# zgcr/SimpleAICV_pytorch_training_examples

Measured on NVIDIA H100. Metric: images/sec (ResNet-50 224x224 training step, whole job), higher is better.
Workload: dtype bf16

## Files before the change

### include/saicv_b200.h

```cpp
#ifndef SAICV_B200_H_
#define SAICV_B200_H_
#include <stdint.h>

#ifdef __cplusplus
extern "C" {
#endif

#define SAICV_EPI_BIAS 1
#define SAICV_EPI_RELU 2
#define SAICV_EPI_GELU 4
#define SAICV_EPI_DIRECT 8
#define SAICV_EPI_RESID 16
#define SAICV_EPI_ADD_BF16 32
#define SAICV_EPI_MUL_DRELU 512

int saicv_version(void);
const char* saicv_last_error(void);
int saicv_sm_count(void);
long long saicv_launch_count(void);

int saicv_linear_fwd(const void* x, const void* w, const float* bias, const float* resid,
                     const float* row_scale, int rows_per_scale, float* stats_partial, void* y,
                     int M, int N, int K, int flags, int out_f32, void* stream);
int saicv_gemm_stats_rows(long long out_rows, int out_cols);
int saicv_linear_dgrad(const void* dy, const void* w, const float* resid, const void* gelu_pre,
                       void* dx, int M, int N, int K, int flags, int out_f32, void* stream);
int saicv_linear_wgrad(const void* dy, const void* x, float* dw_partial, int M, int N, int K,
                       int splits, void* stream);
int saicv_wgrad_splits(int out_rows, int out_cols, long long reduce_len);

typedef struct {
  int n, h, w, c;
  int k, r, s;
  int stride, pad;
} saicv_conv_shape;
int saicv_conv_fprop(const void* x, const void* w, float* stats_partial, void* y,
                     const saicv_conv_shape* cs, int flags, void* stream);
int saicv_conv_dgrad(const void* dy, const void* w, const void* add, const uint32_t* mask_bits, void* dx,
                     const saicv_conv_shape* cs, void* stream);
int saicv_conv_wgrad(const void* dy, const void* x, float* dw_partial, const saicv_conv_shape* cs,
                     int splits, void* stream);

int saicv_prep_conv_weight(const float* w, void* w_bf16, int k, int c, int r, int s, int kpad,
                           int order, int kp, int cp, void* stream);
int saicv_finish_conv_wgrad(const float* partial, float* grad, int splits, int k, int c, int r,
                            int s, int kpad, int accumulate, int order, int kp, int cp, void* stream);
int saicv_reduce_partials(const float* partial, float* out, int splits, long long n,
                          int accumulate, void* stream);
int saicv_cast_bf16(const float* src, void* dst, long long n, void* stream);
int saicv_nchw_to_nhwc_bf16(const float* x, void* y, int n, int c, int h, int w, void* stream);
int saicv_stem_kpad(int c, int r, int s);
int saicv_stem_im2col(const float* x, void* cols, int n, int c, int h, int w, int r, int s,
                      int stride, int pad, int kpad, void* stream);
int saicv_zero_upsample2(const void* dy, void* u, int n, int p, int q, int h, int w, int c,
                         void* stream);
int saicv_add_strided2(void* dx, const void* dd, int n, int p, int q, int h, int w, int c,
                       void* stream);

#define SAICV_BN_PARTIAL_ROWS 264
int saicv_bn_stats(const void* y, float* partials, long long rows, int c, void* stream);
int saicv_bn_finalize(const float* partials, int partial_rows, const float* gamma, const float* beta,
                      float* running_mean, float* running_var, float* scale_shift, float* saved,
                      long long rows, int c, float eps, float momentum, void* stream);
int saicv_bn_apply(const void* y, const float* scale_shift, const void* res,
                   const float* res_scale_shift, void* out, uint32_t* mask_bits, long long rows, int c,
                   int act, void* stream);
int saicv_bn_bwd_reduce(const void* dout, const void* out, const uint32_t* bits, const void* y,
                        const float* saved, const float* scale_shift, float* partials, float* sums,
                        long long rows, int c, int act, void* stream);
int saicv_bn_bwd_apply(const void* dout, const void* out, const uint32_t* bits, const void* y,
                       const float* saved, const float* gamma, const float* scale_shift, float* sums,
                       void* dy, void* dres, float* dgamma, float* dbeta, long long rows, int c, int act,
                       int accumulate, void* stream);
int saicv_bn_bwd_reduce2(const void* g, const uint32_t* bits, const void* y_a, const void* y_b,
                         const float* saved_a, const float* saved_b, float* partials, float* sums,
                         long long rows, int c, void* stream);
int saicv_bn_bwd_apply2(const void* g, const uint32_t* bits, const void* y_a, const void* y_b,
                        const float* saved_a, const float* saved_b, const float* gamma_a,
                        const float* gamma_b, const float* sums, void* dy_a, void* dy_b,
                        float* dgamma_a, float* dbeta_a, float* dgamma_b, float* dbeta_b,
                        long long rows, int c, int accumulate_a, int accumulate_b, void* stream);
int saicv_add_bf16(void* a, const void* b, long long n, void* stream);

int saicv_maxpool3x3s2_fwd(const void* x, void* y, uint8_t* argmax, int n, int h, int w, int c,
                           void* stream);
int saicv_maxpool3x3s2_bwd(const void* dy, const uint8_t* argmax, void* dx, int n, int h, int w,
                           int c, void* stream);
int saicv_maxpool_fwd(const void* x, void* y, uint8_t* argmax, int n, int h, int w, int c, int k,
                      int stride, int pad, int pad_hi, int oob_zero, void* stream);
int saicv_maxpool_bwd(const void* dy, const uint8_t* argmax, void* dx, int n, int h, int w, int c,
                      int k, int stride, int pad, int pad_hi, void* stream);
int saicv_avgpool_fwd(const void* x, void* y, int n, int hw, int c, void* stream);
int saicv_avgpool_bwd(const void* dy, void* dx, int n, int hw, int c, void* stream);
int saicv_colsum(const void* x, float* partials, float* out, long long rows, int c, int accumulate,
                 int is_f32, void* stream);

int saicv_layernorm_fwd(const float* x, const float* gamma, const float* beta, void* y,
                        float* stats, long long rows, int c, float eps, void* stream);
int saicv_layernorm_bwd(const void* dy, const float* x, const float* gamma, const float* stats,
                        const float* dres, float* dx, void* dx_bf16, const float* bf16_row_scale,
                        int rows_per_scale, float* partials ,
                        float* dgamma, float* dbeta, long long rows, int c, int accumulate, void* stream);
int saicv_gelu_fwd(const void* u, void* h, long long n, void* stream);
int saicv_gelu_bwd(const void* dh, const void* u, void* du, long long n, void* stream);
int saicv_vit_assemble_tokens(const float* patch, const float* cls, const float* pos, float* x,
                              int b, int np, int c, void* stream);
int saicv_vit_assemble_tokens_bwd(const float* dx, float* dpos, float* dcls, void* dpatch, int b,
                                  int np, int c, int accumulate, void* stream);
int saicv_token_pool_fwd(const float* x, float* pooled, int b, int l, int c, int mean_pool,
                         void* stream);
int saicv_token_pool_bwd(const float* dpooled, float* dx, void* dx_bf16, const float* bf16_row_scale,
                         int b, int l, int c, int mean_pool, void* stream);
int saicv_dwconv_fwd(const void* x, const float* w, const float* bias, void* y, int n, int h, int wd,
                     int c, int k, int dil, int relu, int flip, void* stream);
int saicv_dwconv_dgrad_masked(const void* dy, const float* w, const void* mask, void* dx, int n, int h,
                              int wd, int c, int k, void* stream);
int saicv_avgpool_stream_fwd(const void* x, int x_f32, void* y, int n, int hw, int c, void* stream);
int saicv_avgpool_stream_bwd(const void* dy, void* dx, int dx_f32, int n, int hw, int c, void* stream);
int saicv_dwconv_wgrad_blocks(long long npix);
int saicv_dwconv_wgrad(const void* dy, const void* x, float* partial, float* dw, int n, int h, int wd,
                       int c, int k, int dil, int accumulate, void* stream);
int saicv_mul_bf16(const void* a, const void* b, void* out, long long n, void* stream);
int saicv_gate_bwd(const void* dg, const void* c1, const void* dlk, const void* p1, void* out,
                   long long n, void* stream);
int saicv_ls_residual_fwd(const void* x, int x_f32, const void* branch, const void* shortcut,
                          const float* ls, const float* row_scale, int rows_per_scale, float* out,
                          long long rows, int c, void* stream);
int saicv_ls_residual_bwd(const float* dxn, const void* branch, const void* shortcut, const float* ls,
                          const float* row_scale, int rows_per_scale, void* dy, float* partial,
                          float* dls, long long rows, int c, int accumulate, void* stream);
int saicv_bn_generic_partial_rows(long long rows, int c);
int saicv_bn_stats_generic(const void* x, int x_f32, float* partial, long long rows, int c, void* stream);
int saicv_bn_apply_generic(const void* x, int x_f32, const float* scale_shift, void* out, int out_f32,
                           long long rows, int c, void* stream);
int saicv_bn_bwd_generic(const void* x, int x_f32, const void* g, int g_f32, const float* saved,
                         const float* gamma, const float* dres, float* partial, float* sums, void* dx,
                         int dx_f32, float* dgamma, float* dbeta, long long rows, int c, int accumulate,
                         void* stream);
int saicv_im2col_nhwc(const void* x, void* cols, int n, int h, int w, int c, int k, int stride, int pad,
                      void* stream);
int saicv_col2im_nhwc(const void* dcols, void* dx, int n, int h, int w, int c, int k, int stride, int pad,
                      void* stream);

int saicv_window_partition(const void* x, void* windows, int b, int h, int w, int c, int ws, void* stream);
int saicv_window_unpartition(const void* windows, void* x, int b, int h, int w, int c, int ws, void* stream);
int saicv_add_pos_embed(float* x, const float* pos, int b, long long per_batch, void* stream);
int saicv_relpos_pack_q(const void* qkv, void* qc, int bw, int heads, int hd, int l, void* stream);
int saicv_relpos_table(const float* rel_pos_h, const float* rel_pos_w, void* rtab, int sh, int sw, int nip, int hd,
                       void* stream);
int saicv_relpos_gather(const void* qkv, const void* t, void* qe, void* ke, int bw, int heads, int hd, int sh, int sw,
                        int dqk, int nip, float scale, void* stream);
int saicv_relpos_shift(const void* dqe, void* ef, int bw, int heads, int hd, int sh, int sw, int dqk, int nip,
                       void* stream);
int saicv_relpos_dq_combine(const void* dqe, const float* dqx, void* dqkv, int bw, int heads, int hd, int l, int dqk,
                            float scale, void* stream);

typedef struct {
  const void* q; const void* k; const void* v;
  void* out;
  float* lse;
  long long q_strides[3], k_strides[3], v_strides[3], o_strides[3];
  const unsigned int* key_mask_bits;
  int mask_words;
  int b, h, lq, lk, dqk, dv;
  float scale;
  float dropout_p;
  unsigned long long dropout_seed;
  const unsigned long long* dropout_seed_base;
} saicv_attn_args;
int saicv_attn_fwd(const saicv_attn_args* a, void* stream);
typedef struct {
  saicv_attn_args fwd;
  const void* dout;
  float* delta;
  void* dq; void* dk; void* dv;
  long long dq_strides[3], dk_strides[3], dv_strides[3];
  int dk_cols;
} saicv_attn_bwd_args;
int saicv_attn_bwd(const saicv_attn_bwd_args* a, void* stream);
int saicv_attention_fwd(const void* qkv, void* out, float* lse, int b, int l, int h, int d,
                        float scale, void* stream);
int saicv_attention_bwd(const void* qkv, const void* out, const void* dout, const float* lse,
                        float* delta, void* dqkv, int b, int l, int h, int d, float scale, void* stream);

int saicv_postln_fwd(const float* z, const float* gamma, const float* beta, float eps, float* y, void* yb,
                     const float* pos, long long pos_rows, void* ypb, float* stats, long long rows, int c,
                     void* stream);
int saicv_postln_bwd(const float* dy, const float* z, const float* gamma, const float* stats, const float* dres,
                     float* dz, void* dzb, float* partials, float* dgamma, float* dbeta, long long rows, int c,
                     int accumulate, void* stream);
int saicv_add_pos_cast(const float* x, const float* pos, long long pos_rows, void* xb, void* xpb, long long rows,
                       int c, void* stream);
int saicv_dropout(const void* in, int in_f32, const float* resid, const float* row_scale, long long elems_per_scale,
                  void* out, int out_f32, long long n, float p, unsigned long long seed,
                  const unsigned long long* seed_base, void* stream);
int saicv_heads_pack(const void* src, int ld, int col0, const float* extra, float extra_const, void* dst, int b,
                     int l, int h, int hd, int dp, float scale, void* stream);
int saicv_heads_unpack(const void* src, void* dst, int ld, int col0, int b, int l, int h, int hd, int dp, float scale,
                       void* stream);

int saicv_sam_loss_partial_floats(int b, int m, long long n);
int saicv_sam_loss_sums(const void* logits, int logits_bf16, const float* targets, float* partials, float* sums, int b,
                        int m, long long n, float alpha, float gamma, float mask_threshold, void* stream);
int saicv_sam_loss_bwd(const void* logits, int logits_bf16, const float* targets, const float* coef, void* dlogits,
                       int dl_bf16, int b, int m, long long n, float alpha, float gamma, void* stream);

#define SAICV_OPT_CHUNK 8192
#define SAICV_OPT_RING 8
typedef struct {
  float* p;
  const float* g;
  float* s1;
  float* s2;
  void* shadow;
  long long numel;
  int group;
  int rs;
  int c, cp, kpad;
  int pad_;
} saicv_opt_tensor;
int saicv_opt_chunk(void);
int saicv_multi_tensor_sgd(const void* tensors, const int* chunk_tensor, const int* chunk_index, int n_chunks,
                           const float* hyper, int n_groups, int* step, const float* clip, void* stream);
int saicv_multi_tensor_adamw(const void* tensors, const int* chunk_tensor, const int* chunk_index, int n_chunks,
                             const float* hyper, int n_groups, int* step, const float* clip, void* stream);
int saicv_multi_tensor_clip_coef(const void* tensors, const int* chunk_tensor, const int* chunk_index, int n_chunks,
                                 float max_norm, float* partial, float* clip, void* stream);

int saicv_u8_nhwc_to_nchw_norm(const void* in, float* out, int n, int h, int w, const float* mean3, const float* std3,
                               void* stream);

int saicv_token_gather_fwd(const float* src, long long src_rows, const int* idx, const float* fill, const float* pos,
                           const int* pos_idx, float* out, int b, int r, int c, void* stream);
int saicv_token_fill_slabs(long long rows);
int saicv_token_gather_bwd(const float* dout, const int* idx, void* dsrc, int dsrc_bf16, long long src_rows,
                           float* fill_partial, int b, int r, int c, void* stream);

#ifdef __cplusplus
}
#endif
#endif
```

### simpleaicv_pytorch_training_examples_b200/_lib.py

```python
import ctypes
import os

_HERE = os.path.dirname(os.path.abspath(__file__))
LIB_PATH = os.path.join(_HERE, 'libsaicv_b200.so')
BN_PARTIAL_ROWS = 264

c_void_p = ctypes.c_void_p
c_int = ctypes.c_int
c_ll = ctypes.c_longlong
c_float = ctypes.c_float


class ConvShape(ctypes.Structure):
    _fields_ = [('n', c_int), ('h', c_int), ('w', c_int), ('c', c_int),
                ('k', c_int), ('r', c_int), ('s', c_int), ('stride', c_int),
                ('pad', c_int)]


class AttnArgs(ctypes.Structure):
    _fields_ = [('q', c_void_p), ('k', c_void_p), ('v', c_void_p), ('out', c_void_p), ('lse', c_void_p),
                ('q_strides', c_ll * 3), ('k_strides', c_ll * 3), ('v_strides', c_ll * 3), ('o_strides', c_ll * 3),
                ('key_mask_bits', c_void_p), ('mask_words', c_int),
                ('b', c_int), ('h', c_int), ('lq', c_int), ('lk', c_int), ('dqk', c_int), ('dv', c_int),
                ('scale', c_float), ('dropout_p', c_float), ('dropout_seed', ctypes.c_ulonglong),
                ('dropout_seed_base', c_void_p)]


class AttnBwdArgs(ctypes.Structure):
    _fields_ = [('fwd', AttnArgs), ('dout', c_void_p), ('delta', c_void_p),
                ('dq', c_void_p), ('dk', c_void_p), ('dv', c_void_p),
                ('dq_strides', c_ll * 3), ('dk_strides', c_ll * 3), ('dv_strides', c_ll * 3), ('dk_cols', c_int)]


SIGNATURES = {
    'saicv_version': [],
    'saicv_sm_count': [],
    'saicv_linear_fwd': [c_void_p, c_void_p, c_void_p, c_void_p, c_void_p, c_int, c_void_p, c_void_p, c_int, c_int, c_int, c_int, c_int, c_void_p],
    'saicv_gemm_stats_rows': [c_ll, c_int],
    'saicv_linear_dgrad': [c_void_p, c_void_p, c_void_p, c_void_p, c_void_p, c_int, c_int, c_int, c_int, c_int, c_void_p],
    'saicv_linear_wgrad': [c_void_p, c_void_p, c_void_p, c_int, c_int, c_int, c_int, c_void_p],
    'saicv_wgrad_splits': [c_int, c_int, c_ll],
    'saicv_conv_fprop': [c_void_p, c_void_p, c_void_p, c_void_p, ctypes.POINTER(ConvShape), c_int, c_void_p],
    'saicv_conv_dgrad': [c_void_p, c_void_p, c_void_p, c_void_p, c_void_p, ctypes.POINTER(ConvShape), c_void_p],
    'saicv_conv_wgrad': [c_void_p, c_void_p, c_void_p, ctypes.POINTER(ConvShape), c_int, c_void_p],
    'saicv_prep_conv_weight': [c_void_p, c_void_p, c_int, c_int, c_int, c_int, c_int, c_int, c_int, c_int, c_void_p],
    'saicv_finish_conv_wgrad': [c_void_p, c_void_p, c_int, c_int, c_int, c_int, c_int, c_int, c_int, c_int, c_int, c_int, c_void_p],
    'saicv_reduce_partials': [c_void_p, c_void_p, c_int, c_ll, c_int, c_void_p],
    'saicv_cast_bf16': [c_void_p, c_void_p, c_ll, c_void_p],
    'saicv_nchw_to_nhwc_bf16': [c_void_p, c_void_p, c_int, c_int, c_int, c_int, c_void_p],
    'saicv_stem_kpad': [c_int, c_int, c_int],
    'saicv_stem_im2col': [c_void_p, c_void_p, c_int, c_int, c_int, c_int, c_int, c_int, c_int, c_int, c_int, c_void_p],
    'saicv_zero_upsample2': [c_void_p, c_void_p, c_int, c_int, c_int, c_int, c_int, c_int, c_void_p],
    'saicv_add_strided2': [c_void_p, c_void_p, c_int, c_int, c_int, c_int, c_int, c_int, c_void_p],
    'saicv_bn_stats': [c_void_p, c_void_p, c_ll, c_int, c_void_p],
    'saicv_bn_finalize': [c_void_p, c_int, c_void_p, c_void_p, c_void_p, c_void_p, c_void_p, c_void_p, c_ll, c_int, c_float, c_float, c_void_p],
    'saicv_bn_apply': [c_void_p, c_void_p, c_void_p, c_void_p, c_void_p, c_void_p, c_ll, c_int, c_int, c_void_p],
    'saicv_bn_bwd_reduce': [c_void_p, c_void_p, c_void_p, c_void_p, c_void_p, c_void_p, c_void_p, c_void_p, c_ll, c_int, c_int, c_void_p],
    'saicv_bn_bwd_apply': [c_void_p, c_void_p, c_void_p, c_void_p, c_void_p, c_void_p, c_void_p, c_void_p, c_void_p, c_void_p, c_void_p, c_void_p, c_ll, c_int, c_int, c_int, c_void_p],
    'saicv_bn_bwd_reduce2': [c_void_p, c_void_p, c_void_p, c_void_p, c_void_p, c_void_p, c_void_p, c_void_p, c_ll, c_int, c_void_p],
    'saicv_bn_bwd_apply2': [c_void_p] * 15 + [c_ll, c_int, c_int, c_int, c_void_p],
    'saicv_add_bf16': [c_void_p, c_void_p, c_ll, c_void_p],
    'saicv_maxpool3x3s2_fwd': [c_void_p, c_void_p, c_void_p, c_int, c_int, c_int, c_int, c_void_p],
    'saicv_maxpool3x3s2_bwd': [c_void_p, c_void_p, c_void_p, c_int, c_int, c_int, c_int, c_void_p],
    'saicv_maxpool_fwd': [c_void_p, c_void_p, c_void_p, c_int, c_int, c_int, c_int, c_int, c_int, c_int, c_int, c_int, c_void_p],
    'saicv_maxpool_bwd': [c_void_p, c_void_p, c_void_p, c_int, c_int, c_int, c_int, c_int, c_int, c_int, c_int, c_void_p],
    'saicv_avgpool_fwd': [c_void_p, c_void_p, c_int, c_int, c_int, c_void_p],
    'saicv_avgpool_bwd': [c_void_p, c_void_p, c_int, c_int, c_int, c_void_p],
    'saicv_colsum': [c_void_p, c_void_p, c_void_p, c_ll, c_int, c_int, c_int, c_void_p],
    'saicv_layernorm_fwd': [c_void_p, c_void_p, c_void_p, c_void_p, c_void_p, c_ll, c_int, c_float, c_void_p],
    'saicv_layernorm_bwd': [c_void_p, c_void_p, c_void_p, c_void_p, c_void_p, c_void_p, c_void_p, c_void_p, c_int, c_void_p, c_void_p, c_void_p, c_ll, c_int, c_int, c_void_p],
    'saicv_gelu_fwd': [c_void_p, c_void_p, c_ll, c_void_p],
    'saicv_gelu_bwd': [c_void_p, c_void_p, c_void_p, c_ll, c_void_p],
    'saicv_vit_assemble_tokens': [c_void_p, c_void_p, c_void_p, c_void_p, c_int, c_int, c_int, c_void_p],
    'saicv_vit_assemble_tokens_bwd': [c_void_p, c_void_p, c_void_p, c_void_p, c_int, c_int, c_int, c_int, c_void_p],
    'saicv_token_pool_fwd': [c_void_p, c_void_p, c_int, c_int, c_int, c_int, c_void_p],
    'saicv_token_pool_bwd': [c_void_p, c_void_p, c_void_p, c_void_p, c_int, c_int, c_int, c_int, c_void_p],
    'saicv_attention_fwd': [c_void_p, c_void_p, c_void_p, c_int, c_int, c_int, c_int, c_float, c_void_p],
    'saicv_attention_bwd': [c_void_p, c_void_p, c_void_p, c_void_p, c_void_p, c_void_p, c_int, c_int, c_int, c_int, c_float, c_void_p],
    'saicv_attn_fwd': [ctypes.POINTER(AttnArgs), c_void_p],
    'saicv_attn_bwd': [ctypes.POINTER(AttnBwdArgs), c_void_p],
    'saicv_window_partition': [c_void_p, c_void_p, c_int, c_int, c_int, c_int, c_int, c_void_p],
    'saicv_window_unpartition': [c_void_p, c_void_p, c_int, c_int, c_int, c_int, c_int, c_void_p],
    'saicv_add_pos_embed': [c_void_p, c_void_p, c_int, c_ll, c_void_p],
    'saicv_relpos_pack_q': [c_void_p, c_void_p, c_int, c_int, c_int, c_int, c_void_p],
    'saicv_relpos_table': [c_void_p, c_void_p, c_void_p, c_int, c_int, c_int, c_int, c_void_p],
    'saicv_relpos_gather': [c_void_p, c_void_p, c_void_p, c_void_p, c_int, c_int, c_int, c_int, c_int, c_int, c_int, c_float, c_void_p],
    'saicv_relpos_shift': [c_void_p, c_void_p, c_int, c_int, c_int, c_int, c_int, c_int, c_int, c_void_p],
    'saicv_relpos_dq_combine': [c_void_p, c_void_p, c_void_p, c_int, c_int, c_int, c_int, c_int, c_float, c_void_p],
    'saicv_sam_loss_partial_floats': [c_int, c_int, c_ll],
    'saicv_sam_loss_sums': [c_void_p, c_int, c_void_p, c_void_p, c_void_p, c_int, c_int, c_ll, c_float, c_float, c_float, c_void_p],
    'saicv_sam_loss_bwd': [c_void_p, c_int, c_void_p, c_void_p, c_void_p, c_int, c_int, c_int, c_ll, c_float, c_float, c_void_p],
    'saicv_u8_nhwc_to_nchw_norm': [c_void_p, c_void_p, c_int, c_int, c_int, ctypes.POINTER(c_float), ctypes.POINTER(c_float), c_void_p],
    'saicv_token_gather_fwd': [c_void_p, c_ll, c_void_p, c_void_p, c_void_p, c_void_p, c_void_p, c_int, c_int, c_int, c_void_p],
    'saicv_token_fill_slabs': [c_ll],
    'saicv_token_gather_bwd': [c_void_p, c_void_p, c_void_p, c_int, c_ll, c_void_p, c_int, c_int, c_int, c_void_p],
    'saicv_opt_chunk': [],
    'saicv_multi_tensor_sgd': [c_void_p, c_void_p, c_void_p, c_int, c_void_p, c_int, c_void_p, c_void_p, c_void_p],
    'saicv_multi_tensor_adamw': [c_void_p, c_void_p, c_void_p, c_int, c_void_p, c_int, c_void_p, c_void_p, c_void_p],
    'saicv_multi_tensor_clip_coef': [c_void_p, c_void_p, c_void_p, c_int, c_float, c_void_p, c_void_p, c_void_p],
    'saicv_postln_fwd': [c_void_p, c_void_p, c_void_p, c_float, c_void_p, c_void_p, c_void_p, c_ll, c_void_p, c_void_p, c_ll, c_int, c_void_p],
    'saicv_postln_bwd': [c_void_p, c_void_p, c_void_p, c_void_p, c_void_p, c_void_p, c_void_p, c_void_p, c_void_p, c_void_p, c_ll, c_int, c_int, c_void_p],
    'saicv_add_pos_cast': [c_void_p, c_void_p, c_ll, c_void_p, c_void_p, c_ll, c_int, c_void_p],
    'saicv_dropout': [c_void_p, c_int, c_void_p, c_void_p, c_ll, c_void_p, c_int, c_ll, c_float, ctypes.c_ulonglong, c_void_p, c_void_p],
    'saicv_heads_pack': [c_void_p, c_int, c_int, c_void_p, c_float, c_void_p, c_int, c_int, c_int, c_int, c_int, c_float, c_void_p],
    'saicv_heads_unpack': [c_void_p, c_void_p, c_int, c_int, c_int, c_int, c_int, c_int, c_int, c_float, c_void_p],
    'saicv_dwconv_fwd': [c_void_p, c_void_p, c_void_p, c_void_p, c_int, c_int, c_int, c_int, c_int, c_int, c_int, c_int, c_void_p],
    'saicv_dwconv_dgrad_masked': [c_void_p, c_void_p, c_void_p, c_void_p, c_int, c_int, c_int, c_int, c_int, c_void_p],
    'saicv_avgpool_stream_fwd': [c_void_p, c_int, c_void_p, c_int, c_int, c_int, c_void_p],
    'saicv_avgpool_stream_bwd': [c_void_p, c_void_p, c_int, c_int, c_int, c_int, c_void_p],
    'saicv_dwconv_wgrad_blocks': [c_ll],
    'saicv_dwconv_wgrad': [c_void_p, c_void_p, c_void_p, c_void_p, c_int, c_int, c_int, c_int, c_int, c_int, c_int, c_void_p],
    'saicv_mul_bf16': [c_void_p, c_void_p, c_void_p, c_ll, c_void_p],
    'saicv_gate_bwd': [c_void_p, c_void_p, c_void_p, c_void_p, c_void_p, c_ll, c_void_p],
    'saicv_ls_residual_fwd': [c_void_p, c_int, c_void_p, c_void_p, c_void_p, c_void_p, c_int, c_void_p, c_ll, c_int, c_void_p],
    'saicv_ls_residual_bwd': [c_void_p, c_void_p, c_void_p, c_void_p, c_void_p, c_int, c_void_p, c_void_p, c_void_p, c_ll, c_int, c_int, c_void_p],
    'saicv_bn_generic_partial_rows': [c_ll, c_int],
    'saicv_bn_stats_generic': [c_void_p, c_int, c_void_p, c_ll, c_int, c_void_p],
    'saicv_bn_apply_generic': [c_void_p, c_int, c_void_p, c_void_p, c_int, c_ll, c_int, c_void_p],
    'saicv_bn_bwd_generic': [c_void_p, c_int, c_void_p, c_int, c_void_p, c_void_p, c_void_p, c_void_p, c_void_p, c_void_p, c_int, c_void_p, c_void_p, c_ll, c_int, c_int, c_void_p],
    'saicv_im2col_nhwc': [c_void_p, c_void_p, c_int, c_int, c_int, c_int, c_int, c_int, c_int, c_void_p],
    'saicv_col2im_nhwc': [c_void_p, c_void_p, c_int, c_int, c_int, c_int, c_int, c_int, c_int, c_void_p],
}

_lib = None


def load():
    global _lib
    if _lib is not None:
        return _lib
    if not os.path.exists(LIB_PATH):
        raise RuntimeError(
            f'{LIB_PATH} not found: build it with `python -c "import __graft_entry__ as g; g.build()"` '
            '(there is no CPU or library fallback for the hot path)')
    lib = ctypes.CDLL(LIB_PATH)
    lib.saicv_last_error.restype = ctypes.c_char_p
    lib.saicv_last_error.argtypes = []
    lib.saicv_launch_count.restype = c_ll
    lib.saicv_launch_count.argtypes = []
    for name, argtypes in SIGNATURES.items():
        fn = getattr(lib, name)
        fn.argtypes = argtypes
        fn.restype = c_int
    _lib = lib
    return lib


def launch_count():
    return int(load().saicv_launch_count())


def call(name, *args):
    lib = load()
    rc = getattr(lib, name)(*args)
    if rc != 0:
        raise RuntimeError(f'{name} failed ({rc}): {lib.saicv_last_error().decode()}')
    return rc
```

### simpleaicv_pytorch_training_examples_b200/csrc/capi_elementwise.cu

```cuda
#include <cuda_bf16.h>
#include <cuda_runtime.h>

#include <atomic>
#include <cstdarg>
#include <cstdio>

#include "../../include/saicv_b200.h"
#include "host_util.h"
#include "vec8.cuh"

namespace saicv {

static thread_local char g_err[512] = "";
int set_error(const char* fmt, ...) {
  va_list ap;
  va_start(ap, fmt);
  vsnprintf(g_err, sizeof(g_err), fmt, ap);
  va_end(ap);
  return 1;
}
static std::atomic<long long> g_launches{0};
void count_launch(int n) { g_launches.fetch_add(n, std::memory_order_relaxed); }
int check_launch(const char* what) {
  cudaError_t e = cudaGetLastError();
// ... 323 lines not shown
  const float inv_n = 1.0f / (float)rows;
  const float mean = s0 * inv_n;
  float var = s1 * inv_n - mean * mean;
  var = fmaxf(var, 0.f);
  const float rstd = rsqrtf(var + eps);
  const float sc = gamma[c] * rstd;
  ss[c] = sc;
  ss[C + c] = beta[c] - mean * sc;
  saved[c] = mean;
  saved[C + c] = rstd;
  if (rmean) {
    const float unbiased = rows > 1 ? var * ((float)rows / (float)(rows - 1)) : var;
    rmean[c] = (1.f - momentum) * rmean[c] + momentum * mean;
    rvar[c] = (1.f - momentum) * rvar[c] + momentum * unbiased;
  }
}

template <bool HAS_RES, bool RES_BN>
__global__ void __launch_bounds__(kThreads, 2)
bn_apply_kernel(const void* __restrict__ y, const float* __restrict__ ss, const void* __restrict__ res,
                const float* __restrict__ rss, void* __restrict__ out, uint8_t* __restrict__ mask, long long rows, int C,
                SlabGeom gm, int act) {
  const int vpr = gm.vpr;
  const int tx = threadIdx.x % gm.tx_count;
  const int ty = threadIdx.x / gm.tx_count;
  if (tx >= vpr) return;
  float sc[8], sh[8], rsc[8], rsh[8];
#pragma unroll
  for (int i = 0; i < 8; ++i) {
    sc[i] = ss[tx * 8 + i];
    sh[i] = ss[C + tx * 8 + i];
    rsc[i] = RES_BN ? rss[tx * 8 + i] : 1.f;
    rsh[i] = RES_BN ? rss[C + tx * 8 + i] : 0.f;
  }
  const long long r0 = (long long)blockIdx.x * gm.rows_per_block;
  long long r1 = r0 + gm.rows_per_block;
  if (r1 > rows) r1 = rows;
  for (long long r = r0 + ty; r < r1; r += (long long)gm.ty_count * UNROLL) {
    V8 vy[UNROLL], vr[UNROLL];
    bool ok[UNROLL];
#pragma unroll
    for (int u = 0; u < UNROLL; ++u) {
      const long long rr = r + (long long)u * gm.ty_count;
      ok[u] = rr < r1;
      if (ok[u]) {
        vy[u] = ldg8(y, rr * vpr + tx);
        if (HAS_RES) vr[u] = ldg8(res, rr * vpr + tx);
      }
    }
#pragma unroll
    for (int u = 0; u < UNROLL; ++u) {
      if (!ok[u]) continue;
      float f[8];
      unpack8(vy[u], f);
#pragma unroll
      for (int i = 0; i < 8; ++i) f[i] = f[i] * sc[i] + sh[i];
      const bool res_after = (act & 8) != 0;
      if (res_after) {
#pragma unroll
        for (int i = 0; i < 8; ++i) f[i] = act_apply(f[i], act & 7);
      }
      if (HAS_RES) {
        float rv[8];
        unpack8(vr[u], rv);
#pragma unroll
        for (int i = 0; i < 8; ++i) f[i] += RES_BN ? rv[i] * rsc[i] + rsh[i] : rv[i];
      }
      if (!res_after) {
#pragma unroll
        for (int i = 0; i < 8; ++i) f[i] = act_apply(f[i], act);
      }
      const long long vi = (r + (long long)u * gm.ty_count) * vpr + tx;
      const V8 o = pack8(f);
      stg8(out, vi, o);
      if (mask) {
        float fo[8];
        unpack8(o, fo);
        uint32_t m = 0;
#pragma unroll
        for (int i = 0; i < 8; ++i) m |= (fo[i] > 0.f ? 1u : 0u) << i;
        mask[vi] = (uint8_t)m;
      }
    }
  }
}

__device__ __forceinline__ void bwd_apply_coefs(const float* __restrict__ saved, const float* __restrict__ gamma,
                                                const float* __restrict__ sums, int tx, int C, float inv_rows,
                                                float (&A)[8], float (&B)[8], float (&K)[8]) {
#pragma unroll
  for (int i = 0; i < 8; ++i) {
    const int c = tx * 8 + i;
    const float mean = saved[c], rstd = saved[C + c];
    const float k1 = gamma[c] * rstd;
    const float k2 = sums[c] * inv_rows, k3 = sums[C + c] * inv_rows;
    A[i] = k1;
    B[i] = -k1 * k3 * rstd;
    K[i] = -k1 * k2 + k1 * k3 * rstd * mean;
  }
}

template <bool HAS_OUT, bool HAS_DRES>
__global__ void __launch_bounds__(kThreads, 2)
bn_bwd_apply_kernel(const void* __restrict__ dout, const void* __restrict__ out, const uint8_t* __restrict__ bits,
                    const void* __restrict__ y, const float* __restrict__ saved, const float* __restrict__ gamma,
                    const float* __restrict__ sums, const float* __restrict__ ss, void* __restrict__ dy,
                    void* __restrict__ dres, long long rows, int C, SlabGeom gm, int act, float inv_rows) {
  const int vpr = gm.vpr;
  const int tx = threadIdx.x % gm.tx_count;
  const int ty = threadIdx.x / gm.tx_count;
  if (tx >= vpr) return;
  float A[8], B[8], K[8], sc[8], sh[8];
  const bool use_bits = !HAS_OUT && act != 0 && bits != nullptr;
  const bool recompute_mask = !HAS_OUT && act != 0 && bits == nullptr;
  bwd_apply_coefs(saved, gamma, sums, tx, C, inv_rows, A, B, K);
#pragma unroll
  for (int i = 0; i < 8; ++i) {
    sc[i] = recompute_mask ? ss[tx * 8 + i] : 0.f;
    sh[i] = recompute_mask ? ss[C + tx * 8 + i] : 0.f;
  }
  const long long r0 = (long long)blockIdx.x * gm.rows_per_block;
  long long r1 = r0 + gm.rows_per_block;
  if (r1 > rows) r1 = rows;
  for (long long r = r0 + ty; r < r1; r += (long long)gm.ty_count * UNROLL) {
    V8 vg[UNROLL], vo[UNROLL], vy[UNROLL];
    uint32_t mb[UNROLL];
    bool ok[UNROLL];
#pragma unroll
    for (int u = 0; u < UNROLL; ++u) {
      const long long rr = r + (long long)u * gm.ty_count;
      ok[u] = rr < r1;
      if (ok[u]) {
        const long long vi = rr * vpr + tx;
        vg[u] = ldg8(dout, vi);
        vy[u] = ldg8(y, vi);
        if (HAS_OUT) vo[u] = ldg8(out, vi);
        else if (use_bits) mb[u] = __ldg(bits + vi);
      }
    }
#pragma unroll
    for (int u = 0; u < UNROLL; ++u) {
      if (!ok[u]) continue;
      const long long vi = (r + (long long)u * gm.ty_count) * vpr + tx;
      float g[8], fy[8];
      unpack8(vg[u], g);
      unpack8(vy[u], fy);
      if (HAS_OUT) {
        float fo[8];
        unpack8(vo[u], fo);
#pragma unroll
        for (int i = 0; i < 8; ++i) g[i] *= act_grad(fo[i], act);
      } else if (use_bits) {
#pragma unroll
        for (int i = 0; i < 8; ++i) g[i] *= mask_bit(mb[u], i);
      } else if (act != 0) {
#pragma unroll
        for (int i = 0; i < 8; ++i) g[i] *= act_grad(fy[i] * sc[i] + sh[i], act);
      }
      if (HAS_DRES) stg8(dres, vi, pack8(g));
      float d[8];
#pragma unroll
      for (int i = 0; i < 8; ++i) d[i] = A[i] * g[i] + B[i] * fy[i] + K[i];
      stg8(dy, vi, pack8(d));
    }
  }
}

__global__ void __launch_bounds__(kThreads, 2)
bn_bwd_apply2_kernel(const void* __restrict__ g, const uint8_t* __restrict__ bits, const void* __restrict__ ya,
                     const void* __restrict__ yb, const float* __restrict__ saved_a, const float* __restrict__ saved_b,
                     const float* __restrict__ gamma_a, const float* __restrict__ gamma_b, const float* __restrict__ sums,
                     void* __restrict__ dya, void* __restrict__ dyb, long long rows, int C, SlabGeom gm, float inv_rows) {
  const int vpr = gm.vpr;
  const int tx = threadIdx.x % gm.tx_count;
  const int ty = threadIdx.x / gm.tx_count;
  if (tx >= vpr) return;
  float Aa[8], Ba[8], Ka[8], Ab[8], Bb[8], Kb[8];
  bwd_apply_coefs(saved_a, gamma_a, sums, tx, C, inv_rows, Aa, Ba, Ka);
  bwd_apply_coefs(saved_b, gamma_b, sums + 2 * C, tx, C, inv_rows, Ab, Bb, Kb);
  const long long r0 = (long long)blockIdx.x * gm.rows_per_block;
  long long r1 = r0 + gm.rows_per_block;
  if (r1 > rows) r1 = rows;
  for (long long r = r0 + ty; r < r1; r += (long long)gm.ty_count * UNROLL) {
    V8 vg[UNROLL], va[UNROLL], vb[UNROLL];
    uint32_t mk[UNROLL];
    bool ok[UNROLL];
#pragma unroll
    for (int u = 0; u < UNROLL; ++u) {
      const long long rr = r + (long long)u * gm.ty_count;
      ok[u] = rr < r1;
      if (ok[u]) {
        const long long vi = rr * vpr + tx;
        vg[u] = ldg8(g, vi);
        va[u] = ldg8(ya, vi);
        vb[u] = ldg8(yb, vi);
        if (bits) mk[u] = __ldg(bits + vi);
      }
    }
#pragma unroll
    for (int u = 0; u < UNROLL; ++u) {
      if (!ok[u]) continue;
      const long long vi = (r + (long long)u * gm.ty_count) * vpr + tx;
      float fg[8], fa[8], fb[8], d[8];
      unpack8(vg[u], fg);
      unpack8(va[u], fa);
      unpack8(vb[u], fb);
      if (bits) {
#pragma unroll
        for (int i = 0; i < 8; ++i) fg[i] *= mask_bit(mk[u], i);
      }
#pragma unroll
      for (int i = 0; i < 8; ++i) d[i] = Aa[i] * fg[i] + Ba[i] * fa[i] + Ka[i];
      stg8(dya, vi, pack8(d));
#pragma unroll
      for (int i = 0; i < 8; ++i) d[i] = Ab[i] * fg[i] + Bb[i] * fb[i] + Kb[i];
      stg8(dyb, vi, pack8(d));
    }
  }
}

__global__ void bn_param_grad_kernel(const float* __restrict__ sums, float* __restrict__ dgamma,
                                     float* __restrict__ dbeta, int C, int accumulate) {
  const int c = blockIdx.x * blockDim.x + threadIdx.x;
  if (c >= C) return;
  if (accumulate) {
    dbeta[c] += sums[c];
    dgamma[c] += sums[C + c];
  } else {
    dbeta[c] = sums[c];
    dgamma[c] = sums[C + c];
  }
}

__global__ void add_bf16_kernel(void* __restrict__ a, const void* __restrict__ b, long long nvec) {
  for (long long vi = (long long)blockIdx.x * blockDim.x + threadIdx.x; vi < nvec;
       vi += (long long)gridDim.x * blockDim.x) {
    float fa[8], fb[8];
    unpack8(ldg8(a, vi), fa);
    unpack8(ldg8(b, vi), fb);
#pragma unroll
    for (int i = 0; i < 8; ++i) fa[i] += fb[i];
    stg8(a, vi, pack8(fa));
  }
}

__global__ void cast_bf16_kernel(const float* __restrict__ src, __nv_bfloat16* __restrict__ dst, long long n) {
  for (long long i = (long long)blockIdx.x * blockDim.x + threadIdx.x; i < n;
       i += (long long)gridDim.x * blockDim.x)
    dst[i] = __float2bfloat16_rn(src[i]);
}
__global__ void cast_bf16_vec_kernel(const float4* __restrict__ src, uint4* __restrict__ dst, long long n8) {
  for (long long i = (long long)blockIdx.x * blockDim.x + threadIdx.x; i < n8; i += (long long)gridDim.x * blockDim.x) {
    const float4 a = __ldg(src + 2 * i), b = __ldg(src + 2 * i + 1);
    const float f[8] = {a.x, a.y, a.z, a.w, b.x, b.y, b.z, b.w};
    dst[i] = pack8(f).q;
  }
}

__global__ void reduce_partials_kernel(const float* __restrict__ partial, float* __restrict__ out, int splits,
                                       long long n, int accumulate) {
  for (long long i = (long long)blockIdx.x * blockDim.x + threadIdx.x; i < n;
       i += (long long)gridDim.x * blockDim.x) {
    float s = accumulate ? out[i] : 0.f;
    for (int k = 0; k < splits; ++k) s += partial[(long long)k * n + i];
    out[i] = s;
  }
}
__global__ void reduce_partials_vec_kernel(const float4* __restrict__ partial, float4* __restrict__ out, int splits, long long n4,
                                           int accumulate) {
  for (long long i = (long long)blockIdx.x * blockDim.x + threadIdx.x; i < n4; i += (long long)gridDim.x * blockDim.x) {
    float4 s = accumulate ? out[i] : make_float4(0.f, 0.f, 0.f, 0.f);
#pragma unroll 4
    for (int k = 0; k < splits; ++k) {
      const float4 v = __ldg(partial + (long long)k * n4 + i);
      s.x += v.x; s.y += v.y; s.z += v.z; s.w += v.w;
    }
    out[i] = s;
  }
}

__global__ void prep_conv_weight_kernel(const float* __restrict__ w, __nv_bfloat16* __restrict__ o, int K, int C,
                                        int R, int S, int kpad, int order, int Kp, int Cp) {
  const long long total = (long long)Kp * kpad;
  for (long long i = (long long)blockIdx.x * blockDim.x + threadIdx.x; i < total;
       i += (long long)gridDim.x * blockDim.x) {
    const int k = (int)(i / kpad), j = (int)(i % kpad);
    float v = 0.f;
    if (k < K) {
      if (order == 1) {
        const int S8 = (S + 7) & ~7;
        const int cr = j / S8, sx = j % S8;
        if (cr < C * R && sx < S) v = w[(long long)k * C * R * S + (long long)cr * S + sx];
      } else if (j < R * S * Cp) {
        const int tap = j / Cp, c = j % Cp;
        if (c < C) v = w[((long long)k * C + c) * (R * S) + tap];
      }
    }
    o[i] = __float2bfloat16_rn(v);
  }
}

__global__ void finish_conv_wgrad_kernel(const float* __restrict__ partial, float* __restrict__ grad, int splits,
                                         int K, int C, int R, int S, int kpad, int accumulate, int order, int Kp,
                                         int Cp) {
  const long long total = (long long)K * C * R * S;
  for (long long i = (long long)blockIdx.x * blockDim.x + threadIdx.x; i < total;
       i += (long long)gridDim.x * blockDim.x) {
    const int tap = (int)(i % (R * S));
    const long long kc = i / (R * S);
    const int c = (int)(kc % C), k = (int)(kc / C);
    const int S8 = (S + 7) & ~7;
    const long long src = order == 1 ? (long long)k * kpad + (long long)(c * R + tap / S) * S8 + tap % S
                                     : (long long)k * kpad + (long long)tap * Cp + c;
    float s = accumulate ? grad[i] : 0.f;
    for (int sp = 0; sp < splits; ++sp) s += partial[(long long)sp * Kp * kpad + src];
    grad[i] = s;
  }
}

__global__ void nchw_to_nhwc_kernel(const float* __restrict__ x, __nv_bfloat16* __restrict__ y, int N, int C, int H,
                                    int W) {
  const long long total = (long long)N * H * W;
  for (long long i = (long long)blockIdx.x * blockDim.x + threadIdx.x; i < total;
       i += (long long)gridDim.x * blockDim.x) {
    const long long hw = i % ((long long)H * W);
    const long long n = i / ((long long)H * W);
    for (int c = 0; c < C; ++c) y[i * C + c] = __float2bfloat16_rn(x[(n * C + c) * (long long)H * W + hw]);
  }
}

__global__ void __launch_bounds__(kThreads)
stem_im2col_kernel(const float* __restrict__ x, void* __restrict__ cols, int N, int C, int H, int W, int R, int S,
                   int stride, int pad, int P, int Q, int kpad, int T) {
  extern __shared__ float sm[];
  const int Wt = (T - 1) * stride + S;
  float* patch = sm;
  const int qtiles = (Q + T - 1) / T;
  const int qt = blockIdx.x % qtiles;
  const int p = (blockIdx.x / qtiles) % P;
  const int n = blockIdx.x / (qtiles * P);
  const int q0 = qt * T;
  const int h0 = p * stride - pad, w0 = q0 * stride - pad;
  for (int i = threadIdx.x; i < C * R * Wt; i += blockDim.x) {
    const int wi = i % Wt, cr = i / Wt;
    const int r = cr % R, c = cr / R;
    const int h = h0 + r, w = w0 + wi;
    float v = 0.f;
    if (h >= 0 && h < H && w >= 0 && w < W) v = __ldg(x + (((long long)n * C + c) * H + h) * W + w);
    patch[i] = v;
  }
  __syncthreads();
  const int vpr = kpad >> 3, S8 = (S + 7) & ~7, vps = S8 >> 3;
  const int npix = min(T, Q - q0);
  const long long row0 = ((long long)n * P + p) * Q + q0;
  for (int v = threadIdx.x; v < npix * vpr; v += blockDim.x) {
    const int pix = v / vpr, kv = v - pix * vpr;
    const int cr = kv / vps, s0 = (kv - cr * vps) * 8;
    float f[8];
    if (cr < C * R) {
      const float* src = patch + cr * Wt + pix * stride + s0;
#pragma unroll
      for (int e = 0; e < 8; ++e) f[e] = (s0 + e < S) ? src[e] : 0.f;
    } else {
#pragma unroll
      for (int e = 0; e < 8; ++e) f[e] = 0.f;
    }
    stg8(cols, (row0 + pix) * vpr + kv, pack8(f));
  }
}

__global__ void zero_upsample2_kernel(const void* __restrict__ dy, void* __restrict__ u, int N, int P, int Q, int H,
                                      int W, int C) {
  const int vpr = C >> 3;
  const long long total = (long long)N * H * W * vpr;
  for (long long i = (long long)blockIdx.x * blockDim.x + threadIdx.x; i < total;
       i += (long long)gridDim.x * blockDim.x) {
    const int v = (int)(i % vpr);
    const long long pix = i / vpr;
    const int w = (int)(pix % W);
    const int h = (int)((pix / W) % H);
    const long long n = pix / ((long long)W * H);
    V8 val;
    val.q = make_uint4(0u, 0u, 0u, 0u);
    if (!(h & 1) && !(w & 1) && (h >> 1) < P && (w >> 1) < Q)
      val = ldg8(dy, ((n * P + (h >> 1)) * Q + (w >> 1)) * vpr + v);
    stg8(u, i, val);
  }
}

__global__ void add_strided2_kernel(void* __restrict__ dx, const void* __restrict__ dd, int N, int P, int Q, int H,
                                    int W, int C) {
  const int vpr = C >> 3;
  const long long total = (long long)N * P * Q * vpr;
  for (long long i = (long long)blockIdx.x * blockDim.x + threadIdx.x; i < total;
       i += (long long)gridDim.x * blockDim.x) {
    const int v = (int)(i % vpr);
    const long long pix = i / vpr;
    const int q = (int)(pix % Q);
    const int p = (int)((pix / Q) % P);
    const long long n = pix / ((long long)Q * P);
    const long long di = ((n * H + 2 * p) * W + 2 * q) * vpr + v;
    float a[8], b[8];
    unpack8(ldg8(dx, di), a);
    unpack8(ldg8(dd, i), b);
#pragma unroll
    for (int k = 0; k < 8; ++k) a[k] += b[k];
    stg8(dx, di, pack8(a));
  }
}

template <int KT>
__global__ void maxpool_fwd_kernel(const void* __restrict__ x, void* __restrict__ y, uint8_t* __restrict__ amax,
                                   int N, int H, int W, int C, int P, int Q, int Krt, int stride, int pad, int oob_zero) {
  const int K = KT > 0 ? KT : Krt;
  const int vpr = C >> 3;
  const long long total = (long long)N * P * Q * vpr;
  for (long long i = (long long)blockIdx.x * blockDim.x + threadIdx.x; i < total;
       i += (long long)gridDim.x * blockDim.x) {
    const int v = (int)(i % vpr);
    const long long pix = i / vpr;
    const int q = (int)(pix % Q);
    const int p = (int)((pix / Q) % P);
    const long long n = pix / ((long long)Q * P);
    float best[8];
    int arg[8];
#pragma unroll
    for (int k = 0; k < 8; ++k) { best[k] = -INFINITY; arg[k] = 0; }
    bool first = true;
    if (KT > 0) {
      V8 win[KT > 0 ? KT * KT : 1];
      bool ok[KT > 0 ? KT * KT : 1];
#pragma unroll
      for (int r = 0; r < KT; ++r)
#pragma unroll
        for (int s = 0; s < KT; ++s) {
          const int h = stride * p - pad + r, w = stride * q - pad + s;
          ok[r * KT + s] = h >= 0 && h < H && w >= 0 && w < W;
          win[r * KT + s].zero();
          if (ok[r * KT + s]) win[r * KT + s] = ldg8(x, ((n * H + h) * W + w) * vpr + v);
        }
#pragma unroll
      for (int t = 0; t < KT * KT; ++t) {
        if (!ok[t] && !oob_zero) continue;
        float f[8];
        unpack8(win[t], f);
        const int code = ok[t] ? t : 255;
#pragma unroll
        for (int k = 0; k < 8; ++k)
          if (first || f[k] > best[k]) { best[k] = f[k]; arg[k] = code; }
        first = false;
      }
    } else {
      for (int r = 0; r < K; ++r) {
        const int h = stride * p - pad + r;
        for (int s = 0; s < K; ++s) {
          const int w = stride * q - pad + s;
          const bool inside = h >= 0 && h < H && w >= 0 && w < W;
          if (!inside && !oob_zero) continue;
          float f[8];
          if (inside) {
            unpack8(ldg8(x, ((n * H + h) * W + w) * vpr + v), f);
          } else {
#pragma unroll
            for (int k = 0; k < 8; ++k) f[k] = 0.f;
          }
          const int code = inside ? r * K + s : 255;
#pragma unroll
          for (int k = 0; k < 8; ++k)
            if (first || f[k] > best[k]) { best[k] = f[k]; arg[k] = code; }
          first = false;
        }
      }
    }
    stg8(y, i, pack8(best));
    uint64_t packed = 0;
#pragma unroll
    for (int k = 0; k < 8; ++k) packed |= (uint64_t)(arg[k] & 0xff) << (8 * k);
    reinterpret_cast<uint64_t*>(amax)[i] = packed;
  }
}

template <bool FAST>
__global__ void maxpool_bwd_kernel(const void* __restrict__ dy, const uint8_t* __restrict__ amax,
                                   void* __restrict__ dx, int N, int H, int W, int C, int P, int Q, int K, int stride,
                                   int pad) {
  const int vpr = C >> 3;
  const long long total = (long long)N * H * W * vpr;
  for (long long i = (long long)blockIdx.x * blockDim.x + threadIdx.x; i < total;
       i += (long long)gridDim.x * blockDim.x) {
    const int v = (int)(i % vpr);
    const long long pix = i / vpr;
    const int w = (int)(pix % W);
    const int h = (int)((pix / W) % H);
    const long long n = pix / ((long long)W * H);
    float acc[8];
#pragma unroll
    for (int k = 0; k < 8; ++k) acc[k] = 0.f;
    const int hp = h + pad, wp = w + pad;
    const int p_hi = min(hp / stride, P - 1), q_hi = min(wp / stride, Q - 1);
    const int p_lo = max((hp - K + stride) / stride, 0), q_lo = max((wp - K + stride) / stride, 0);
    if (FAST) {
      uint64_t am[4];
      V8 gv[4];
      int code[4];
#pragma unroll
      for (int t = 0; t < 4; ++t) {
        const int p = hp / stride - (t >> 1), q = wp / stride - (t & 1);
        const int r = hp - stride * p, s2 = wp - stride * q;
        const bool ok = p >= 0 && p < P && q >= 0 && q < Q && r < K && s2 < K;
        code[t] = ok ? r * K + s2 : -1;
        am[t] = 0;
        gv[t].zero();
        if (ok) {
          const long long oi = ((n * P + p) * Q + q) * vpr + v;
          am[t] = __ldg(reinterpret_cast<const uint64_t*>(amax) + oi);
          gv[t] = ldg8(dy, oi);
        }
      }
#pragma unroll
      for (int t = 0; t < 4; ++t) {
        float g[8];
        unpack8(gv[t], g);
#pragma unroll
        for (int k = 0; k < 8; ++k)
          if ((int)((am[t] >> (8 * k)) & 0xff) == code[t]) acc[k] += g[k];
      }
      stg8(dx, i, pack8(acc));
      continue;
    }
    for (int p = p_lo; p <= p_hi; ++p) {
      const int r = hp - stride * p;
      if (r < 0 || r >= K) continue;
      for (int q = q_lo; q <= q_hi; ++q) {
        const int s = wp - stride * q;
        if (s < 0 || s >= K) continue;
        const long long oi = ((n * P + p) * Q + q) * vpr + v;
        const uint64_t packed = reinterpret_cast<const uint64_t*>(amax)[oi];
        float g[8];
        unpack8(ldg8(dy, oi), g);
#pragma unroll
        for (int k = 0; k < 8; ++k)
          if ((int)((packed >> (8 * k)) & 0xff) == r * K + s) acc[k] += g[k];
      }
    }
    stg8(dx, i, pack8(acc));
  }
}

__global__ void avgpool_fwd_kernel(const void* __restrict__ x, void* __restrict__ y, int N, int HW, int C) {
  const int vpr = C >> 3;
  const long long total = (long long)N * vpr;
  const float inv = 1.f / (float)HW;
  for (long long i = (long long)blockIdx.x * blockDim.x + threadIdx.x; i < total;
       i += (long long)gridDim.x * blockDim.x) {
    const int v = (int)(i % vpr);
    const long long n = i / vpr;
    float acc[8];
#pragma unroll
    for (int k = 0; k < 8; ++k) acc[k] = 0.f;
    for (int t = 0; t < HW; ++t) {
      float f[8];
      unpack8(ldg8(x, (n * HW + t) * vpr + v), f);
#pragma unroll
      for (int k = 0; k < 8; ++k) acc[k] += f[k];
    }
#pragma unroll
    for (int k = 0; k < 8; ++k) acc[k] *= inv;
    stg8(y, i, pack8(acc));
  }
}

__global__ void avgpool_bwd_kernel(const void* __restrict__ dy, void* __restrict__ dx, int N, int HW, int C) {
  const int vpr = C >> 3;
  const long long total = (long long)N * HW * vpr;
  const float inv = 1.f / (float)HW;
  for (long long i = (long long)blockIdx.x * blockDim.x + threadIdx.x; i < total;
       i += (long long)gridDim.x * blockDim.x) {
    const int v = (int)(i % vpr);
    const long long n = i / ((long long)HW * vpr);
    float f[8];
    unpack8(ldg8(dy, n * vpr + v), f);
#pragma unroll
    for (int k = 0; k < 8; ++k) f[k] *= inv;
    stg8(dx, i, pack8(f));
  }
}

}
}

using namespace saicv;

#define ST ((cudaStream_t)stream)

extern "C" {

int saicv_version(void) { return 100; }
long long saicv_launch_count(void) { return saicv::launch_count(); }
const char* saicv_last_error(void) { return saicv::last_error(); }

int saicv_bn_stats(const void* y, float* partials, long long rows, int c, void* stream) {
  int nblk;
  return launch_colreduce<0>(y, nullptr, nullptr, nullptr, nullptr, partials, rows, c, 0, &nblk, ST);
}

int saicv_bn_finalize(const float* partials, int partial_rows_, const float* gamma, const float* beta,
                      float* running_mean, float* running_var, float* scale_shift, float* saved, long long rows,
                      int c, float eps, float momentum, void* stream) {
  const int nrows = partial_rows_ > 0 ? partial_rows_ : partial_rows(rows, c);
  bn_finalize_kernel<<<(c + 7) / 8, 256, 0, ST>>>(partials, nrows, gamma, beta, running_mean,
                                                    running_var, scale_shift, saved, rows, c, eps, momentum);
  return check_launch("bn_finalize_kernel");
}

int saicv_bn_apply(const void* y, const float* scale_shift, const void* res, const float* res_scale_shift,
                   void* out, uint32_t* mask_bits, long long rows, int c, int act, void* stream) {
  if (mask_bits && (c % 32 || (act & 7) != 1))
    return set_error("saicv_bn_apply: mask_bits needs c %% 32 == 0 and a ReLU (c=%d act=%d)", c, act);
  SlabGeom g;
  int blocks;
  if (!slab_geom(rows, c, UNROLL, &g, &blocks)) return 1;
  uint8_t* mask = reinterpret_cast<uint8_t*>(mask_bits);
  if (res == nullptr)
    bn_apply_kernel<false, false><<<blocks, kThreads, 0, ST>>>(y, scale_shift, res, res_scale_shift, out, mask, rows, c, g, act);
  else if (res_scale_shift == nullptr)
    bn_apply_kernel<true, false><<<blocks, kThreads, 0, ST>>>(y, scale_shift, res, res_scale_shift, out, mask, rows, c, g, act);
  else
    bn_apply_kernel<true, true><<<blocks, kThreads, 0, ST>>>(y, scale_shift, res, res_scale_shift, out, mask, rows, c, g, act);
  return check_launch("bn_apply_kernel");
}

static int check_mask_source(const char* fn, const void* out, const uint32_t* bits, const float* scale_shift, int c,
                             int act) {
  if (act != 0 && out == nullptr && bits == nullptr && scale_shift == nullptr)
    return set_error("%s: need the activated output, mask bits or scale_shift to form the activation mask", fn);
  if ((act & 7) == 3 && out != nullptr) return set_error("%s: SiLU needs the recompute path (out == NULL, scale_shift given)", fn);
  if (bits != nullptr && (act != 1 || c % 32)) return set_error("%s: mask bits need act == 1 (ReLU) and c %% 32 == 0 (c=%d)", fn, c);
  return 0;
}

int saicv_bn_bwd_reduce(const void* dout, const void* out, const uint32_t* bits, const void* y, const float* saved,
                        const float* scale_shift, float* partials, float* sums, long long rows, int c, int act,
                        void* stream) {
  if (int e = check_mask_source("saicv_bn_bwd_reduce", out, bits, scale_shift, c, act)) return e;
  int nblk;
  if (int e = launch_colreduce<1>(dout, out, y, saved, scale_shift, partials, rows, c, act, &nblk, ST, bits)) return e;
  return fold(partials, sums, nblk, 2 * c, 0, ST);
}

int saicv_bn_bwd_apply(const void* dout, const void* out, const uint32_t* bits, const void* y, const float* saved,
                       const float* gamma, const float* scale_shift, float* sums, void* dy, void* dres, float* dgamma,
                       float* dbeta, long long rows, int c, int act, int accumulate, void* stream) {
  if (int e = check_mask_source("saicv_bn_bwd_apply", out, bits, scale_shift, c, act)) return e;
  SlabGeom g;
  int blocks;
  if (!slab_geom(rows, c, UNROLL, &g, &blocks)) return 1;
  const float inv_rows = 1.0f / (float)rows;
  const uint8_t* mask = reinterpret_cast<const uint8_t*>(bits);
#define BWD_APPLY(HO, HD) \
  bn_bwd_apply_kernel<HO, HD><<<blocks, kThreads, 0, ST>>>(dout, out, mask, y, saved, gamma, sums, scale_shift, dy, dres, rows, c, g, act, inv_rows)
  if (out != nullptr && act != 0) {
    if (dres) BWD_APPLY(true, true); else BWD_APPLY(true, false);
  } else {
    if (dres) BWD_APPLY(false, true); else BWD_APPLY(false, false);
  }
#undef BWD_APPLY
  if (int e = check_launch("bn_bwd_apply_kernel")) return e;
  bn_param_grad_kernel<<<(c + 127) / 128, 128, 0, ST>>>(sums, dgamma, dbeta, c, accumulate);
  return check_launch("bn_param_grad_kernel");
}

int saicv_bn_bwd_reduce2(const void* g, const uint32_t* bits, const void* y_a, const void* y_b, const float* saved_a,
                         const float* saved_b, float* partials, float* sums, long long rows, int c, void* stream) {
  if (bits != nullptr && c % 32) return set_error("saicv_bn_bwd_reduce2: mask bits need c %% 32 == 0 (c=%d)", c);
  SlabGeom gm;
  int nblk;
  if (!slab_geom(rows, c, 4, &gm, &nblk, kMaxPartials)) return 1;
  colreduce2_kernel<<<nblk, kThreads, 0, ST>>>(g, reinterpret_cast<const uint8_t*>(bits), y_a, y_b, saved_a, saved_b,
                                               partials, rows, c, gm);
  if (int e = check_launch("colreduce2_kernel")) return e;
  return fold(partials, sums, nblk, 4 * c, 0, ST);
}

int saicv_bn_bwd_apply2(const void* g, const uint32_t* bits, const void* y_a, const void* y_b, const float* saved_a,
                        const float* saved_b, const float* gamma_a, const float* gamma_b, const float* sums, void* dy_a,
                        void* dy_b, float* dgamma_a, float* dbeta_a, float* dgamma_b, float* dbeta_b, long long rows,
                        int c, int accumulate_a, int accumulate_b, void* stream) {
  if (bits != nullptr && c % 32) return set_error("saicv_bn_bwd_apply2: mask bits need c %% 32 == 0 (c=%d)", c);
  SlabGeom gm;
  int blocks;
  if (!slab_geom(rows, c, UNROLL, &gm, &blocks)) return 1;
  bn_bwd_apply2_kernel<<<blocks, kThreads, 0, ST>>>(g, reinterpret_cast<const uint8_t*>(bits), y_a, y_b, saved_a,
                                                    saved_b, gamma_a, gamma_b, sums, dy_a, dy_b, rows, c, gm,
                                                    1.0f / (float)rows);
  if (int e = check_launch("bn_bwd_apply2_kernel")) return e;
  bn_param_grad_kernel<<<(c + 127) / 128, 128, 0, ST>>>(sums, dgamma_a, dbeta_a, c, accumulate_a);
  if (int e = check_launch("bn_param_grad_kernel")) return e;
  bn_param_grad_kernel<<<(c + 127) / 128, 128, 0, ST>>>(sums + 2 * c, dgamma_b, dbeta_b, c, accumulate_b);
  return check_launch("bn_param_grad_kernel");
}

int saicv_add_bf16(void* a, const void* b, long long n, void* stream) {
  if (n % 8) return set_error("saicv_add_bf16: n %% 8 != 0");
  add_bf16_kernel<<<grid_for(n / 8), kThreads, 0, ST>>>(a, b, n / 8);
  return check_launch("add_bf16_kernel");
}

int saicv_cast_bf16(const float* src, void* dst, long long n, void* stream) {
  if (n % 8 == 0 && ((uintptr_t)src & 15) == 0 && ((uintptr_t)dst & 15) == 0) {
    cast_bf16_vec_kernel<<<grid_for(n / 8), kThreads, 0, ST>>>(reinterpret_cast<const float4*>(src), reinterpret_cast<uint4*>(dst), n / 8);
    return check_launch("cast_bf16_vec_kernel");
  }
  cast_bf16_kernel<<<grid_for(n), kThreads, 0, ST>>>(src, reinterpret_cast<__nv_bfloat16*>(dst), n);
  return check_launch("cast_bf16_kernel");
}

int saicv_reduce_partials(const float* partial, float* out, int splits, long long n, int accumulate,
                          void* stream) {
  if (n % 4 == 0 && ((uintptr_t)partial & 15) == 0 && ((uintptr_t)out & 15) == 0) {
    reduce_partials_vec_kernel<<<grid_for(n / 4), kThreads, 0, ST>>>(reinterpret_cast<const float4*>(partial), reinterpret_cast<float4*>(out),
                                                                    splits, n / 4, accumulate);
    return check_launch("reduce_partials_vec_kernel");
  }
  reduce_partials_kernel<<<grid_for(n), kThreads, 0, ST>>>(partial, out, splits, n, accumulate);
  return check_launch("reduce_partials_kernel");
}

int saicv_prep_conv_weight(const float* w, void* w_bf16, int k, int c, int r, int s, int kpad, int order,
                           int kp, int cp, void* stream) {
  if (kp <= 0) kp = k;
  if (cp <= 0) cp = c;
  if (kpad % 8 || kpad < r * s * (order == 1 ? c : cp) || kp < k || cp < c)
    return set_error("saicv_prep_conv_weight: bad padding (kpad %d kp %d cp %d)", kpad, kp, cp);
  prep_conv_weight_kernel<<<grid_for((long long)kp * kpad), kThreads, 0, ST>>>(
      w, reinterpret_cast<__nv_bfloat16*>(w_bf16), k, c, r, s, kpad, order, kp, cp);
  return check_launch("prep_conv_weight_kernel");
}

int saicv_finish_conv_wgrad(const float* partial, float* grad, int splits, int k, int c, int r, int s, int kpad,
                            int accumulate, int order, int kp, int cp, void* stream) {
  if (kp <= 0) kp = k;
  if (cp <= 0) cp = c;
  finish_conv_wgrad_kernel<<<grid_for((long long)k * c * r * s), kThreads, 0, ST>>>(partial, grad, splits, k, c, r,
                                                                                     s, kpad, accumulate, order, kp, cp);
  return check_launch("finish_conv_wgrad_kernel");
}

int saicv_nchw_to_nhwc_bf16(const float* x, void* y, int n, int c, int h, int w, void* stream) {
  nchw_to_nhwc_kernel<<<grid_for((long long)n * h * w), kThreads, 0, ST>>>(x, reinterpret_cast<__nv_bfloat16*>(y),
                                                                           n, c, h, w);
  return check_launch("nchw_to_nhwc_kernel");
}

int saicv_stem_kpad(int c, int r, int s) { return (c * r * ((s + 7) / 8 * 8) + 63) / 64 * 64; }

int saicv_stem_im2col(const float* x, void* cols, int n, int c, int h, int w, int r, int s, int stride, int pad,
                      int kpad, void* stream) {
  if (kpad % 8 || kpad < r * c * ((s + 7) / 8 * 8))
    return set_error("saicv_stem_im2col: kpad %d must be a multiple of 8 >= c*r*roundup(s, 8) = %d (saicv_stem_kpad)", kpad, r * c * ((s + 7) / 8 * 8));
  const int P = (h + 2 * pad - r) / stride + 1, Q = (w + 2 * pad - s) / stride + 1;
  int T = 32;
  while (T > 1 && ((size_t)c * r * ((T - 1) * stride + s) * 4) > 40 * 1024) T >>= 1;
  const size_t smem = (size_t)c * r * ((T - 1) * stride + s) * 4;
  if (smem > 48 * 1024) return set_error("saicv_stem_im2col: patch of %zu bytes does not fit in shared memory", smem);
  const long long blocks = (long long)n * P * ((Q + T - 1) / T);
  stem_im2col_kernel<<<(unsigned)blocks, kThreads, smem, ST>>>(x, cols, n, c, h, w, r, s, stride, pad, P, Q, kpad, T);
  return check_launch("stem_im2col_kernel");
}

int saicv_zero_upsample2(const void* dy, void* u, int n, int p, int q, int h, int w, int c, void* stream) {
  if (c % 8) return set_error("saicv_zero_upsample2: C %% 8 != 0");
  zero_upsample2_kernel<<<grid_for((long long)n * h * w * (c / 8)), kThreads, 0, ST>>>(dy, u, n, p, q, h, w, c);
  return check_launch("zero_upsample2_kernel");
}

int saicv_add_strided2(void* dx, const void* dd, int n, int p, int q, int h, int w, int c, void* stream) {
  if (c % 8) return set_error("saicv_add_strided2: C %% 8 != 0");
  add_strided2_kernel<<<grid_for((long long)n * p * q * (c / 8)), kThreads, 0, ST>>>(dx, dd, n, p, q, h, w, c);
  return check_launch("add_strided2_kernel");
}

int saicv_maxpool_fwd(const void* x, void* y, uint8_t* argmax, int n, int h, int w, int c, int k, int stride, int pad,
                      int pad_hi, int oob_zero, void* stream) {
  if (c % 8) return set_error("saicv_maxpool_fwd: C %% 8 != 0");
  if (k < 1 || k > 15 || stride < 1) return set_error("saicv_maxpool_fwd: unsupported window %d / stride %d", k, stride);
  const int P = (h + pad + pad_hi - k) / stride + 1, Q = (w + pad + pad_hi - k) / stride + 1;
  const int grid = grid_for((long long)n * P * Q * (c / 8));
  if (k == 3) maxpool_fwd_kernel<3><<<grid, kThreads, 0, ST>>>(x, y, argmax, n, h, w, c, P, Q, k, stride, pad, oob_zero);
  else if (k == 2) maxpool_fwd_kernel<2><<<grid, kThreads, 0, ST>>>(x, y, argmax, n, h, w, c, P, Q, k, stride, pad, oob_zero);
  else maxpool_fwd_kernel<0><<<grid, kThreads, 0, ST>>>(x, y, argmax, n, h, w, c, P, Q, k, stride, pad, oob_zero);
  return check_launch("maxpool_fwd_kernel");
}

int saicv_maxpool_bwd(const void* dy, const uint8_t* argmax, void* dx, int n, int h, int w, int c, int k, int stride,
                      int pad, int pad_hi, void* stream) {
  if (c % 8) return set_error("saicv_maxpool_bwd: C %% 8 != 0");
  const int P = (h + pad + pad_hi - k) / stride + 1, Q = (w + pad + pad_hi - k) / stride + 1;
  const int grid = grid_for((long long)n * h * w * (c / 8));
  if (k <= 2 * stride && k >= stride) maxpool_bwd_kernel<true><<<grid, kThreads, 0, ST>>>(dy, argmax, dx, n, h, w, c, P, Q, k, stride, pad);
  else maxpool_bwd_kernel<false><<<grid, kThreads, 0, ST>>>(dy, argmax, dx, n, h, w, c, P, Q, k, stride, pad);
  return check_launch("maxpool_bwd_kernel");
}

int saicv_maxpool3x3s2_fwd(const void* x, void* y, uint8_t* argmax, int n, int h, int w, int c, void* stream) {
  return saicv_maxpool_fwd(x, y, argmax, n, h, w, c, 3, 2, 1, 1, 0, stream);
}

int saicv_maxpool3x3s2_bwd(const void* dy, const uint8_t* argmax, void* dx, int n, int h, int w, int c,
                           void* stream) {
  return saicv_maxpool_bwd(dy, argmax, dx, n, h, w, c, 3, 2, 1, 1, stream);
}

int saicv_avgpool_fwd(const void* x, void* y, int n, int hw, int c, void* stream) {
  if (c % 8) return set_error("saicv_avgpool_fwd: C %% 8 != 0");
  avgpool_fwd_kernel<<<grid_for((long long)n * (c / 8), 128), 128, 0, ST>>>(x, y, n, hw, c);
  return check_launch("avgpool_fwd_kernel");
}

int saicv_avgpool_bwd(const void* dy, void* dx, int n, int hw, int c, void* stream) {
  if (c % 8) return set_error("saicv_avgpool_bwd: C %% 8 != 0");
  avgpool_bwd_kernel<<<grid_for((long long)n * hw * (c / 8)), kThreads, 0, ST>>>(dy, dx, n, hw, c);
  return check_launch("avgpool_bwd_kernel");
}

int saicv_colsum(const void* x, float* partials, float* out, long long rows, int c, int accumulate, int is_f32,
                 void* stream) {
  if (is_f32) {
    colsum_f32_kernel<<<(c + 127) / 128, 128, 0, ST>>>(reinterpret_cast<const float*>(x), out, rows, c, accumulate);
    return check_launch("colsum_f32_kernel");
  }
  if (c % 8) return set_error("saicv_colsum: C %% 8 != 0");
  for (int c0 = 0; c0 < c; c0 += 2048) {
    const int cw = c - c0 < 2048 ? c - c0 : 2048;
    SlabGeom g;
    int nblk;
    if (!slab_geom(rows, cw, 8, &g, &nblk, kMaxPartials)) return 1;
    g.ldv = c / 8;
    colreduce_kernel<2, 8><<<nblk, kThreads, 0, ST>>>(reinterpret_cast<const __nv_bfloat16*>(x) + c0, nullptr, nullptr,
                                                   nullptr, nullptr, nullptr, partials, rows, cw, g, 0);
    if (int e = check_launch("colreduce_kernel")) return e;
    if (int e = fold(partials, out + c0, nblk, cw, accumulate, ST)) return e;
  }
  return 0;
}

}
```

### simpleaicv_pytorch_training_examples_b200/csrc/capi_gemm.cu

```cuda
#include <cudaTypedefs.h>

#include <cstdarg>
#include <cstdio>
#include <cstdlib>
#include <cstring>
#include <mutex>

#include "../../include/saicv_b200.h"
#include "gemm_sm90.cuh"
#include "host_util.h"

using namespace saicv;

namespace {

PFN_cuTensorMapEncodeTiled_v12000 g_encode_tiled = nullptr;
PFN_cuTensorMapEncodeIm2col_v12000 g_encode_im2col = nullptr;
int g_sm_count = 0;
int g_driver_version = 0;
std::once_flag g_once;
bool g_init_ok = false;

void init_driver() {
  cudaDriverEntryPointQueryResult qres;
  void* fn = nullptr;
  if (cudaGetDriverEntryPoint("cuTensorMapEncodeTiled", &fn, cudaEnableDefault, &qres) != cudaSuccess ||
      qres != cudaDriverEntryPointSuccess || fn == nullptr) {
    set_error("cuTensorMapEncodeTiled not available (no CUDA driver?)");
    return;
  }
  g_encode_tiled = reinterpret_cast<PFN_cuTensorMapEncodeTiled_v12000>(fn);
  fn = nullptr;
  if (cudaGetDriverEntryPoint("cuTensorMapEncodeIm2col", &fn, cudaEnableDefault, &qres) != cudaSuccess ||
      qres != cudaDriverEntryPointSuccess || fn == nullptr) {
    set_error("cuTensorMapEncodeIm2col not available");
    return;
  }
  g_encode_im2col = reinterpret_cast<PFN_cuTensorMapEncodeIm2col_v12000>(fn);
  int dev = 0;
  if (cudaGetDevice(&dev) != cudaSuccess) { set_error("cudaGetDevice failed"); return; }
  cudaDeviceProp prop;
  if (cudaGetDeviceProperties(&prop, dev) != cudaSuccess) { set_error("cudaGetDeviceProperties failed"); return; }
  if (prop.major != 9) {
    set_error("libsaicv_b200 requires an sm_90 (H100) device, found sm_%d%d", prop.major, prop.minor);
    return;
  }
  g_sm_count = prop.multiProcessorCount;
  cudaDriverGetVersion(&g_driver_version);
  g_init_ok = true;
}

bool ensure_init() {
  std::call_once(g_once, init_driver);
  return g_init_ok;
}

bool encode_2d(CUtensorMap* m, const void* ptr, CUtensorMapDataType dt, int esz, uint64_t cols,
               uint64_t rows, uint64_t row_stride_elems, uint32_t box_cols, uint32_t box_rows) {
  cuuint64_t dims[2] = {cols, rows};
  cuuint64_t strides[1] = {row_stride_elems * (uint64_t)esz};
  cuuint32_t box[2] = {box_cols, box_rows};
  cuuint32_t estr[2] = {1, 1};
  CUresult r = g_encode_tiled(m, dt, 2, const_cast<void*>(ptr), dims, strides, box, estr,
                              CU_TENSOR_MAP_INTERLEAVE_NONE, CU_TENSOR_MAP_SWIZZLE_128B,
                              CU_TENSOR_MAP_L2_PROMOTION_L2_256B, CU_TENSOR_MAP_FLOAT_OOB_FILL_NONE);
  if (r != CUDA_SUCCESS) {
    set_error("cuTensorMapEncodeTiled(2d) failed: %d (cols=%llu rows=%llu stride=%llu box=%u,%u ptr=%p)",
              (int)r, (unsigned long long)cols, (unsigned long long)rows,
              (unsigned long long)row_stride_elems, box_cols, box_rows, ptr);
    return false;
  }
  return true;
}

bool encode_out(CUtensorMap* m, const void* ptr, bool f32, uint64_t cols, uint64_t rows,
                uint64_t ldd, uint64_t splits, uint64_t split_stride) {
  const int esz = f32 ? 4 : 2;
  cuuint64_t dims[3] = {cols, rows, splits};
  cuuint64_t strides[2] = {ldd * esz, (splits > 1 ? split_stride : ldd * rows) * esz};
  cuuint32_t box[3] = {f32 ? 32u : 64u, 128u, 1u};
  cuuint32_t estr[3] = {1, 1, 1};
  CUresult r = g_encode_tiled(m, f32 ? CU_TENSOR_MAP_DATA_TYPE_FLOAT32 : CU_TENSOR_MAP_DATA_TYPE_BFLOAT16, 3,
                              const_cast<void*>(ptr), dims, strides, box, estr,
                              CU_TENSOR_MAP_INTERLEAVE_NONE, CU_TENSOR_MAP_SWIZZLE_128B,
                              CU_TENSOR_MAP_L2_PROMOTION_L2_256B, CU_TENSOR_MAP_FLOAT_OOB_FILL_NONE);
  if (r != CUDA_SUCCESS) {
    set_error("cuTensorMapEncodeTiled(out) failed: %d (cols=%llu rows=%llu ldd=%llu splits=%llu)", (int)r,
              (unsigned long long)cols, (unsigned long long)rows, (unsigned long long)ldd,
              (unsigned long long)splits);
    return false;
  }
  return true;
}

bool encode_im2col(CUtensorMap* m, const void* ptr, int n, int h, int w, int c, int lc_h, int lc_w,
                   int uc_h, int uc_w, int stride, uint32_t pixels_per_col) {
  cuuint64_t dims[4] = {(uint64_t)c, (uint64_t)w, (uint64_t)h, (uint64_t)n};
  cuuint64_t strides[3] = {(uint64_t)c * 2, (uint64_t)w * c * 2, (uint64_t)h * w * c * 2};
  int lower[2] = {lc_w, lc_h};
  int upper[2] = {uc_w, uc_h};
  cuuint32_t estr[4] = {1, (cuuint32_t)stride, (cuuint32_t)stride, 1};
  CUresult r = g_encode_im2col(m, CU_TENSOR_MAP_DATA_TYPE_BFLOAT16, 4, const_cast<void*>(ptr), dims, strides,
                               lower, upper, 64, pixels_per_col, estr, CU_TENSOR_MAP_INTERLEAVE_NONE,
                               CU_TENSOR_MAP_SWIZZLE_128B, CU_TENSOR_MAP_L2_PROMOTION_L2_256B,
                               CU_TENSOR_MAP_FLOAT_OOB_FILL_NONE);
  if (r != CUDA_SUCCESS) {
    set_error("cuTensorMapEncodeIm2col failed: %d (n=%d h=%d w=%d c=%d lc=%d,%d uc=%d,%d stride=%d ppc=%u)",
              (int)r, n, h, w, c, lc_h, lc_w, uc_h, uc_w, stride, pixels_per_col);
    return false;
  }
  if (g_driver_version <= 13010 && (uint64_t)n * h * w * c * 2 < 131072)
    reinterpret_cast<uint64_t*>(m)[1] &= ~(1ull << 21);
  return true;
}

bool aligned16(const void* p) { return (reinterpret_cast<uintptr_t>(p) & 15) == 0; }

void tune_override(int* bn, int* stages, int* nb) {
  const char* e = getenv("SAICV_GEMM_TUNE");
  if (!e || !*e) return;
  int a = 0, b = 0, c = 0;
  sscanf(e, "%d:%d:%d", &a, &b, &c);
  if (bn && (a == 64 || a == 128)) *bn = a;
  if (stages && b > 0) *stages = b;
  if (nb && c > 0) *nb = c;
}

template <int BN>
void pick_smem_split(const GemmParams& p, int stat_bytes, int* stages_out, int* nb_out) {
  using Cfg = GemmCfg<BN>;
  const int budget = kSmemBudget - stat_bytes;
  const bool has_aux = p.aux_tma != 0;
  const int kb = p.kb_per_split;
  const int min_stages = has_aux ? (kb <= 4 ? 2 : (kb <= 16 && p.out_f32) ? 3 : 4) : (kb >= 4 ? 4 : 3);
  int nb = has_aux ? 3 : 2;
  while (nb > 1 && (budget - 2 * nb * kStoreBufBytes) / Cfg::kStageBytes < min_stages) --nb;
  int stages = (budget - 2 * nb * kStoreBufBytes) / Cfg::kStageBytes;
  tune_override(nullptr, &stages, &nb);
  if (nb > kMaxStoreBufs) nb = kMaxStoreBufs;
  const int fit = (budget - 2 * nb * kStoreBufBytes) / Cfg::kStageBytes;
  if (stages > fit) stages = fit;
  if (stages > Cfg::kStages) stages = Cfg::kStages;
  *stages_out = stages;
  *nb_out = nb;
}

template <int BN, int VAR>
int launch(const CUtensorMap& a, const CUtensorMap& b, const CUtensorMap& d, const CUtensorMap& r, const GemmParams& p,
           cudaStream_t st) {
  using Cfg = GemmCfg<BN>;
  static bool attr_set = false;
  if (!attr_set) {
    cudaError_t e = cudaFuncSetAttribute(gemm_sm90_kernel<BN, VAR>, cudaFuncAttributeMaxDynamicSharedMemorySize,
                                         Cfg::kSmemBytes);
    if (e != cudaSuccess) return set_error("cudaFuncSetAttribute(smem=%d): %s", Cfg::kSmemBytes, cudaGetErrorString(e));
    attr_set = true;
  }
  const int num_m = (p.M + BM - 1) / BM, num_n = (p.N + BN - 1) / BN;
  const long long total = (long long)num_m * num_n * p.splits;
  const int grid = (int)(total < g_sm_count ? total : g_sm_count);
  const int stat_bytes = (p.epi_flags & EPI_STATS) ? ((8 * p.N + 15) & ~15) : 0;
  int stages = 0, nb = 1;
  pick_smem_split<BN>(p, stat_bytes, &stages, &nb);
  if (stages < 2) return set_error("gemm_sm90_kernel<%d>: %d bytes of statistics do not fit in shared memory", BN, stat_bytes);
  const_cast<GemmParams&>(p).num_stages = stages;
  const_cast<GemmParams&>(p).store_bufs = nb;
  gemm_sm90_kernel<BN, VAR><<<grid, GemmVariant<VAR>::kThreads, Cfg::kSmemBytes, st>>>(a, b, d, r, p);
  cudaError_t e = cudaGetLastError();
  if (e != cudaSuccess) return set_error("gemm_sm90_kernel<%d> launch: %s", BN, cudaGetErrorString(e));
  count_launch(1);
  return 0;
}

int pick_bn(int N) {
  const int cand[2] = {128, 64};
  int best = 128;
  long long best_cost = -1;
  for (int i = 0; i < 2; ++i) {
    const long long cost = (long long)((N + cand[i] - 1) / cand[i]) * cand[i];
    if (best_cost < 0 || cost < best_cost) { best_cost = cost; best = cand[i]; }
  }
  tune_override(&best, nullptr, nullptr);
  return best;
}

int dispatch(int bn, const CUtensorMap& a, const CUtensorMap& b, const CUtensorMap& d, GemmParams& p,
             cudaStream_t st, const void* aux = nullptr, bool aux_f32 = false) {
  CUtensorMap r = d;
  p.aux_tma = 0;
  const bool both = (p.epi_flags & EPI_RESID) && (p.epi_flags & (EPI_RESID_BF16 | EPI_MUL_DGELU | EPI_MUL_DRELU));
  if (aux && !both && !(p.epi_flags & EPI_DIRECT) && p.splits == 1 && aux_f32 == (p.out_f32 != 0) && aligned16(aux) &&
      !getenv("SAICV_GEMM_NO_AUX_TMA")) {
    if (!encode_out(&r, aux, aux_f32, p.N, p.M, p.ldd, 1, 0)) return 2;
    p.aux_tma = 1;
  }
  int var = VAR_FULL;
  if (!getenv("SAICV_GEMM_FULL_VARIANT")) {
    if (p.aux_tma && !(p.epi_flags & ~GemmVariant<VAR_AUX>::kMask)) var = VAR_AUX;
    else if (!p.aux_tma && !p.out_f32 && !(p.epi_flags & ~GemmVariant<VAR_PLAIN_BF16>::kMask))
      var = ((p.epi_flags & EPI_STATS) && !getenv("SAICV_GEMM_INLINE_STATS")) ? VAR_STATS_BF16 : VAR_PLAIN_BF16;
    else if (!p.aux_tma && p.out_f32 && !(p.epi_flags & ~GemmVariant<VAR_PLAIN_F32>::kMask)) var = VAR_PLAIN_F32;
  }
  if ((p.epi_flags & EPI_MASK_BITS) && var != VAR_AUX)
    return set_error("EPI_MASK_BITS needs the TMA aux-operand epilogue (VAR_AUX): bf16 `add` operand, one split, no overrides");
#define SAICV_LAUNCH_BN(BN_)                                                         \
  switch (var) {                                                                     \
    case VAR_PLAIN_BF16: return launch<BN_, VAR_PLAIN_BF16>(a, b, d, r, p, st);      \
    case VAR_STATS_BF16: return launch<BN_, VAR_STATS_BF16>(a, b, d, r, p, st);      \
    case VAR_PLAIN_F32: return launch<BN_, VAR_PLAIN_F32>(a, b, d, r, p, st);        \
    case VAR_AUX: return launch<BN_, VAR_AUX>(a, b, d, r, p, st);                    \
    default: return launch<BN_, VAR_FULL>(a, b, d, r, p, st);                        \
  }
  switch (bn) {
    case 64: SAICV_LAUNCH_BN(64)
    default: SAICV_LAUNCH_BN(128)
  }
#undef SAICV_LAUNCH_BN
}

}

extern "C" {

int saicv_sm_count(void) { return ensure_init() ? g_sm_count : 0; }

int saicv_gemm_stats_rows(long long out_rows, int out_cols) {
  const int bn = pick_bn(out_cols);
  const long long tiles = ((out_rows + BM - 1) / BM) * ((out_cols + bn - 1) / bn);
  const int sms = ensure_init() ? g_sm_count : 132;
  return (int)(tiles < sms ? tiles : sms);
}

int saicv_wgrad_splits(int out_rows, int out_cols, long long reduce_len) {
  const int bn = pick_bn(out_cols);
  const long long tiles = (long long)((out_rows + BM - 1) / BM) * ((out_cols + bn - 1) / bn);
  const long long num_kb = (reduce_len + BK - 1) / BK;
  const int sms = g_sm_count > 0 ? g_sm_count : 132;
  long long want = (2LL * sms + tiles - 1) / tiles;
  long long max_by_k = num_kb / 8 > 0 ? num_kb / 8 : 1;
  long long s = want < max_by_k ? want : max_by_k;
  if (s < 1) s = 1;
  if (s > 64) s = 64;
  long long per = (num_kb + s - 1) / s;
  s = (num_kb + per - 1) / per;
  return (int)s;
}

int saicv_linear_fwd(const void* x, const void* w, const float* bias, const float* resid,
                     const float* row_scale, int rows_per_scale, float* stats_partial, void* y, int M, int N,
                     int K, int flags, int out_f32, void* stream) {
  if (!ensure_init()) return 1;
  if (!aligned16(x) || !aligned16(w) || !aligned16(y) || (K % 8) || (N % (out_f32 ? 4 : 8)))
    return set_error("saicv_linear_fwd: unaligned operand (M=%d N=%d K=%d)", M, N, K);
  const int bn = pick_bn(N);
  CUtensorMap ta, tb, td;
  if (!encode_2d(&ta, x, CU_TENSOR_MAP_DATA_TYPE_BFLOAT16, 2, K, M, K, 64, 128)) return 2;
  if (!encode_2d(&tb, w, CU_TENSOR_MAP_DATA_TYPE_BFLOAT16, 2, K, N, K, 64, bn)) return 2;
  if (!encode_out(&td, y, out_f32, N, M, N, 1, 0)) return 2;
  GemmParams p{};
  p.M = M; p.N = N; p.num_kb = (K + BK - 1) / BK; p.kb_per_split = p.num_kb; p.splits = 1;
  p.a_mode = A_K2D; p.b_mode = B_K2D;
  p.g.P = p.g.Q = 1; p.g.cchunks = 1; p.g.S = 1; p.g.R = 1;
  p.epi_flags = (flags & (EPI_RELU | EPI_GELU | EPI_DIRECT)) | (bias ? EPI_BIAS : 0) | (resid ? EPI_RESID : 0) |
                (row_scale ? EPI_ROW_SCALE : 0);
  if (row_scale && rows_per_scale <= 0) return set_error("saicv_linear_fwd: rows_per_scale must be > 0");
  p.row_scale = row_scale; p.rows_per_scale = rows_per_scale;
  if (stats_partial) {
    if (bias || resid || out_f32 || (flags & EPI_DIRECT))
      return set_error("saicv_linear_fwd: stats_partial needs a plain bf16 output through the TMA-store epilogue (no bias / residual)");
    p.epi_flags |= EPI_STATS; p.stats_partial = stats_partial;
  }
  p.out_f32 = out_f32; p.bias = bias; p.resid = resid; p.out = y; p.ldd = N; p.split_stride = 0;
  return dispatch(bn, ta, tb, td, p, (cudaStream_t)stream, resid, true);
}

int saicv_linear_dgrad(const void* dy, const void* w, const float* resid, const void* gelu_pre, void* dx,
                       int M, int N, int K, int flags, int out_f32, void* stream) {
  if (!ensure_init()) return 1;
  if (!aligned16(dy) || !aligned16(w) || !aligned16(dx) || (K % 8) || (N % 8))
    return set_error("saicv_linear_dgrad: unaligned operand (M=%d N=%d K=%d)", M, N, K);
  const int bn = pick_bn(K);
  CUtensorMap ta, tb, td;
  if (!encode_2d(&ta, dy, CU_TENSOR_MAP_DATA_TYPE_BFLOAT16, 2, N, M, N, 64, 128)) return 2;
  if (!encode_2d(&tb, w, CU_TENSOR_MAP_DATA_TYPE_BFLOAT16, 2, K, N, K, 64, 64)) return 2;
  if (!encode_out(&td, dx, out_f32, K, M, K, 1, 0)) return 2;
  GemmParams p{};
  p.M = M; p.N = K; p.num_kb = (N + BK - 1) / BK; p.kb_per_split = p.num_kb; p.splits = 1;
  p.a_mode = A_K2D; p.b_mode = B_MN2D;
  p.g.P = p.g.Q = 1; p.g.cchunks = 1; p.g.S = 1; p.g.R = 1;
  const int aux_mode = !gelu_pre ? 0 : (flags & EPI_MUL_DRELU) ? EPI_MUL_DRELU : (flags & EPI_RESID_BF16) ? EPI_RESID_BF16 : EPI_MUL_DGELU;
  p.epi_flags = (flags & EPI_DIRECT) | (resid ? EPI_RESID : 0) | aux_mode;
  if (gelu_pre && !aligned16(gelu_pre)) return set_error("saicv_linear_dgrad: unaligned aux operand");
  p.out_f32 = out_f32; p.resid = resid; p.resid_bf16 = gelu_pre; p.out = dx; p.ldd = K;
  return dispatch(bn, ta, tb, td, p, (cudaStream_t)stream, resid ? (const void*)resid : gelu_pre, resid != nullptr);
}

int saicv_linear_wgrad(const void* dy, const void* x, float* dw_partial, int M, int N, int K,
                       int splits, void* stream) {
  if (!ensure_init()) return 1;
  if (!aligned16(dy) || !aligned16(x) || !aligned16(dw_partial) || (K % 8) || (N % 8))
    return set_error("saicv_linear_wgrad: unaligned operand (M=%d N=%d K=%d)", M, N, K);
  const int bn = pick_bn(K);
  CUtensorMap ta, tb, td;
  if (!encode_2d(&ta, dy, CU_TENSOR_MAP_DATA_TYPE_BFLOAT16, 2, N, M, N, 64, 64)) return 2;
  if (!encode_2d(&tb, x, CU_TENSOR_MAP_DATA_TYPE_BFLOAT16, 2, K, M, K, 64, 64)) return 2;
  if (!encode_out(&td, dw_partial, true, K, N, K, splits, (uint64_t)N * K)) return 2;
  GemmParams p{};
  p.M = N; p.N = K; p.num_kb = (M + BK - 1) / BK;
  p.kb_per_split = (p.num_kb + splits - 1) / splits;
  p.splits = (p.num_kb + p.kb_per_split - 1) / p.kb_per_split;
  if (p.splits != splits) return set_error("saicv_linear_wgrad: splits=%d leaves an empty split (use saicv_wgrad_splits)", splits);
  p.a_mode = A_MN2D; p.b_mode = B_MN2D;
  p.g.P = p.g.Q = 1; p.g.cchunks = 1; p.g.S = 1; p.g.R = 1;
  p.epi_flags = 0; p.out_f32 = 1; p.out = dw_partial; p.ldd = K; p.split_stride = (long long)N * K;
  return dispatch(bn, ta, tb, td, p, (cudaStream_t)stream);
}

static int conv_out(int in, int pad, int r, int stride) { return (in + 2 * pad - r) / stride + 1; }

int saicv_conv_fprop(const void* x, const void* w, float* stats_partial, void* y, const saicv_conv_shape* cs,
                     int flags, void* stream) {
  if (!ensure_init()) return 1;
  if (cs->c % 64 || cs->k % 8 || !aligned16(x) || !aligned16(w) || !aligned16(y))
    return set_error("saicv_conv_fprop: needs c%%64==0, k%%8==0 and 16B-aligned pointers (c=%d k=%d)", cs->c, cs->k);
  const int P = conv_out(cs->h, cs->pad, cs->r, cs->stride), Q = conv_out(cs->w, cs->pad, cs->s, cs->stride);
  const long long M = (long long)cs->n * P * Q;
  const int Kred = cs->r * cs->s * cs->c;
  const int bn = pick_bn(cs->k);
  CUtensorMap ta, tb, td;
  if (!encode_im2col(&ta, x, cs->n, cs->h, cs->w, cs->c, -cs->pad, -cs->pad, cs->pad - (cs->r - 1),
                     cs->pad - (cs->s - 1), cs->stride, 128))
    return 2;
  if (!encode_2d(&tb, w, CU_TENSOR_MAP_DATA_TYPE_BFLOAT16, 2, Kred, cs->k, Kred, 64, bn)) return 2;
  if (!encode_out(&td, y, false, cs->k, M, cs->k, 1, 0)) return 2;
  GemmParams p{};
  p.M = (int)M; p.N = cs->k; p.num_kb = Kred / BK; p.kb_per_split = p.num_kb; p.splits = 1;
  p.a_mode = A_IM2COL; p.b_mode = B_K2D; p.b_cin = cs->c;
  p.g.P = P; p.g.Q = Q; p.g.stride = cs->stride; p.g.lc_h = -cs->pad; p.g.lc_w = -cs->pad;
  p.g.R = cs->r; p.g.S = cs->s; p.g.cchunks = cs->c / 64; p.g.n_img = cs->n;
  p.epi_flags = flags & (EPI_RELU | EPI_DIRECT); p.out_f32 = 0; p.out = y; p.ldd = cs->k;
  if (stats_partial) {
    if (flags & EPI_DIRECT) return set_error("saicv_conv_fprop: stats_partial is not available with SAICV_EPI_DIRECT");
    p.epi_flags |= EPI_STATS; p.stats_partial = stats_partial;
  }
  return dispatch(bn, ta, tb, td, p, (cudaStream_t)stream);
}

int saicv_conv_dgrad(const void* dy, const void* w, const void* add, const uint32_t* mask_bits, void* dx,
                     const saicv_conv_shape* cs, void* stream) {
  if (!ensure_init()) return 1;
  if (cs->c % 64 || cs->k % 64 || !aligned16(dy) || !aligned16(w) || !aligned16(dx))
    return set_error("saicv_conv_dgrad: needs c%%64==0 and k%%64==0 (c=%d k=%d)", cs->c, cs->k);
  if (cs->stride != 1) return set_error("saicv_conv_dgrad: stride must be 1 (zero-upsample dy for strided convs)");
  const long long M = (long long)cs->n * cs->h * cs->w;
  const int Kw = cs->r * cs->s * cs->c;
  const int bn = pick_bn(cs->c);
  const int lc_h = cs->pad - (cs->r - 1), lc_w = cs->pad - (cs->s - 1);
  CUtensorMap ta, tb, td;
  if (!encode_im2col(&ta, dy, cs->n, cs->h, cs->w, cs->k, lc_h, lc_w, lc_h, lc_w, 1, 128)) return 2;
  if (!encode_2d(&tb, w, CU_TENSOR_MAP_DATA_TYPE_BFLOAT16, 2, Kw, cs->k, Kw, 64, 64)) return 2;
  if (!encode_out(&td, dx, false, cs->c, M, cs->c, 1, 0)) return 2;
  GemmParams p{};
  p.M = (int)M; p.N = cs->c; p.num_kb = cs->r * cs->s * (cs->k / 64); p.kb_per_split = p.num_kb; p.splits = 1;
  p.a_mode = A_IM2COL; p.b_mode = B_MN2D; p.flip_taps = 1; p.b_cin = cs->c;
  p.g.P = cs->h; p.g.Q = cs->w; p.g.stride = 1; p.g.lc_h = lc_h; p.g.lc_w = lc_w;
  p.g.R = cs->r; p.g.S = cs->s; p.g.cchunks = cs->k / 64; p.g.n_img = cs->n;
  p.epi_flags = (add ? EPI_RESID_BF16 : 0) | (mask_bits ? EPI_MASK_BITS : 0);
  p.resid_bf16 = add; p.mask_bits = mask_bits; p.out_f32 = 0; p.out = dx; p.ldd = cs->c;
  if (add && !aligned16(add)) return set_error("saicv_conv_dgrad: unaligned `add`");
  if (mask_bits && !add) return set_error("saicv_conv_dgrad: mask_bits is applied in the epilogue of the fused `add` only");
  return dispatch(bn, ta, tb, td, p, (cudaStream_t)stream, add, false);
}

int saicv_conv_wgrad(const void* dy, const void* x, float* dw_partial, const saicv_conv_shape* cs,
                     int splits, void* stream) {
  if (!ensure_init()) return 1;
  if (cs->c % 64 || cs->k % 8 || !aligned16(dy) || !aligned16(x) || !aligned16(dw_partial))
    return set_error("saicv_conv_wgrad: needs c%%64==0, k%%8==0 (c=%d k=%d)", cs->c, cs->k);
  const int P = conv_out(cs->h, cs->pad, cs->r, cs->stride), Q = conv_out(cs->w, cs->pad, cs->s, cs->stride);
  const long long Mpix = (long long)cs->n * P * Q;
  const int Ncols = cs->r * cs->s * cs->c;
  const int bn = pick_bn(Ncols);
  CUtensorMap ta, tb, td;
  if (!encode_2d(&ta, dy, CU_TENSOR_MAP_DATA_TYPE_BFLOAT16, 2, cs->k, Mpix, cs->k, 64, 64)) return 2;
  if (!encode_im2col(&tb, x, cs->n, cs->h, cs->w, cs->c, -cs->pad, -cs->pad, cs->pad - (cs->r - 1),
                     cs->pad - (cs->s - 1), cs->stride, 64))
    return 2;
  if (!encode_out(&td, dw_partial, true, Ncols, cs->k, Ncols, splits, (uint64_t)cs->k * Ncols)) return 2;
  GemmParams p{};
  p.M = cs->k; p.N = Ncols; p.num_kb = (int)((Mpix + BK - 1) / BK);
  p.kb_per_split = (p.num_kb + splits - 1) / splits;
  p.splits = (p.num_kb + p.kb_per_split - 1) / p.kb_per_split;
  if (p.splits != splits) return set_error("saicv_conv_wgrad: splits=%d leaves an empty split (use saicv_wgrad_splits)", splits);
  p.a_mode = A_MN2D; p.b_mode = B_IM2COL;
  p.g.P = P; p.g.Q = Q; p.g.stride = cs->stride; p.g.lc_h = -cs->pad; p.g.lc_w = -cs->pad;
  p.g.R = cs->r; p.g.S = cs->s; p.g.cchunks = cs->c / 64; p.g.n_img = cs->n;
  p.epi_flags = 0; p.out_f32 = 1; p.out = dw_partial; p.ldd = Ncols; p.split_stride = (long long)cs->k * Ncols;
  return dispatch(bn, ta, tb, td, p, (cudaStream_t)stream);
}

}
```

### simpleaicv_pytorch_training_examples_b200/csrc/gemm_sm90.cuh

```cuda
#pragma once
#include "gelu_math.cuh"
#include "ptx.cuh"

namespace saicv {

enum : int { A_K2D = 0, A_IM2COL = 1, A_MN2D = 2 };
enum : int { B_K2D = 0, B_MN2D = 2, B_IM2COL = 3 };
enum : int { EPI_BIAS = 1, EPI_RELU = 2, EPI_GELU = 4, EPI_DIRECT = 8, EPI_RESID = 16, EPI_RESID_BF16 = 32,
              EPI_MUL_DGELU = 64, EPI_ROW_SCALE = 128, EPI_STATS = 256, EPI_MUL_DRELU = 512, EPI_MASK_BITS = 1024 };

constexpr int BM = 128;
constexpr int BK = 64;
constexpr int kGemmThreads = 384;
constexpr int kStoreBufBytes = 16384;
constexpr int kMaxStoreBufs = 3;
constexpr int kSmemTotal = 232448;
constexpr int kXposeStride = 33;
constexpr int kXposeBytes = 8 * 32 * kXposeStride * 4;
constexpr int kSmemBudget = kSmemTotal - 1024  - 512  - kXposeBytes;

template <int BN>
struct GemmCfg {
  static constexpr int kStageBytes = BM * BK * 2 + BN * BK * 2;
  static constexpr int kStagesRaw = (kSmemBudget - 2 * kStoreBufBytes) / kStageBytes;
  static constexpr int kStages = kStagesRaw > 8 ? 8 : kStagesRaw;
  static constexpr int kSmemBytes = kSmemTotal;
  static_assert(BN == 64 || BN == 128, "a consumer warpgroup owns 64 columns: BN is 64 (one warpgroup) or 128 (two)");
  static constexpr int kConsumerWGs = BN / 64;
};

struct ConvGeom {
  int P, Q;
  int stride;
  int lc_h, lc_w;
  int R, S;
  int cchunks;
  int n_img;
};

struct GemmParams {
  int M, N;
  int num_kb;
  int kb_per_split;
  int splits;
  int a_mode, b_mode;
  int flip_taps;
  int b_cin;
  ConvGeom g;
  int epi_flags;
  int out_f32;
  const float* bias;
  const float* resid;
  const void* resid_bf16;
  const float* row_scale;
  int rows_per_scale;
  void* out;
  long long ldd;
  long long split_stride;
  int num_stages;
  int store_bufs;
  int aux_tma;
  float* stats_partial;
  const uint32_t* mask_bits;
};

enum : int { VAR_FULL = 0, VAR_PLAIN_BF16 = 1, VAR_PLAIN_F32 = 2, VAR_AUX = 3, VAR_STATS_BF16 = 4 };
template <int VAR>
struct GemmVariant {
  static constexpr int kMask = VAR == VAR_FULL ? (0x7fffffff & ~EPI_MASK_BITS)
                               : (VAR == VAR_PLAIN_BF16 || VAR == VAR_STATS_BF16) ? (EPI_BIAS | EPI_RELU | EPI_STATS)
                               : VAR == VAR_PLAIN_F32 ? EPI_BIAS
                               : (EPI_BIAS | EPI_ROW_SCALE | EPI_RESID | EPI_RESID_BF16 | EPI_MUL_DGELU | EPI_MUL_DRELU |
                                  EPI_MASK_BITS);
  static constexpr int kOut = (VAR == VAR_PLAIN_BF16 || VAR == VAR_STATS_BF16) ? 1 : VAR == VAR_PLAIN_F32 ? 2 : 0;
  static constexpr int kAux = VAR == VAR_FULL ? 0 : VAR == VAR_AUX ? 2 : 1;
  static constexpr bool kStatsWarps = VAR == VAR_STATS_BF16;
  static constexpr int kThreads = kStatsWarps ? kGemmThreads + 128 : kGemmThreads;
};

template <int BN, int TA, int TB>
__device__ __forceinline__ void gemm_mainloop(float (&acc)[2][32], const uint8_t* sA, const uint8_t* sB, uint64_t* full_bar,
                                              uint64_t* empty_bar, int nstages, int& stage, uint32_t& phase, int kb0, int kb1,
                                              uint32_t b_off, int lane) {
  constexpr int kABytes = BM * BK * 2, kBBytes = BN * BK * 2;
  constexpr uint32_t a_lbo = TA ? 8192u : 16u, b_lbo = TB ? 8192u : 16u;
  constexpr uint32_t a_kstep = TA ? 2048u : 32u, b_kstep = TB ? 2048u : 32u;
  int prev = -1;
  for (int kb = kb0; kb < kb1; ++kb) {
    mbar_wait(&full_bar[stage], phase);
    const uint32_t a_addr = smem_u32(sA + stage * kABytes);
    const uint32_t b_addr = smem_u32(sB + stage * kBBytes) + b_off;
    wgmma_fence_regs(acc[0]);
    wgmma_fence_regs(acc[1]);
    wgmma_fence();
#pragma unroll
    for (int k = 0; k < BK / 16; ++k) {
      const uint64_t db = make_smem_desc(b_addr + k * b_kstep, b_lbo, 1024);
      const int acc_in = (kb > kb0 || k > 0) ? 1 : 0;
      wgmma_m64n64<TA, TB>(acc[0], make_smem_desc(a_addr + k * a_kstep, a_lbo, 1024), db, acc_in);
      wgmma_m64n64<TA, TB>(acc[1], make_smem_desc(a_addr + 8192 + k * a_kstep, a_lbo, 1024), db, acc_in);
    }
    wgmma_commit();
    wgmma_wait<1>();
    wgmma_fence_regs(acc[0]);
    wgmma_fence_regs(acc[1]);
    if (prev >= 0) {
      __syncwarp();
      if (lane == 0) mbar_arrive(&empty_bar[prev]);
    }
    prev = stage;
    if (++stage == nstages) { stage = 0; phase ^= 1; }
  }
  wgmma_wait<0>();
  wgmma_fence_regs(acc[0]);
  wgmma_fence_regs(acc[1]);
  if (prev >= 0) {
    __syncwarp();
    if (lane == 0) mbar_arrive(&empty_bar[prev]);
  }
}

template <int BN, int VAR>
__global__ void __launch_bounds__(GemmVariant<VAR>::kThreads, 1)
gemm_sm90_kernel(const __grid_constant__ CUtensorMap tmA, const __grid_constant__ CUtensorMap tmB,
                  const __grid_constant__ CUtensorMap tmD, const __grid_constant__ CUtensorMap tmR,
                  const GemmParams p) {
  using Cfg = GemmCfg<BN>;
  constexpr int kStages = Cfg::kStages;
  constexpr int kABytes = BM * BK * 2;
  constexpr int kBBytes = BN * BK * 2;

  extern __shared__ uint8_t smem_raw[];
  uint8_t* smem = reinterpret_cast<uint8_t*>((reinterpret_cast<uintptr_t>(smem_raw) + 1023) &
                                             ~static_cast<uintptr_t>(1023));
  using V = GemmVariant<VAR>;
  const int flags = p.epi_flags & V::kMask;
  const bool out_f32 = V::kOut == 0 ? (p.out_f32 != 0) : (V::kOut == 2);
  const int nstages = p.num_stages;
  const bool do_stats = (flags & EPI_STATS) != 0;
  uint8_t* sA = smem;
  uint8_t* sB = smem + nstages * kABytes;
  uint8_t* sD = smem + nstages * Cfg::kStageBytes;
  const int NB = p.store_bufs;
  float* sStat = reinterpret_cast<float*>(sD + 2 * NB * kStoreBufBytes);
  uint64_t* full_bar = reinterpret_cast<uint64_t*>(sD + 2 * NB * kStoreBufBytes + (do_stats ? ((8 * p.N + 15) & ~15) : 0));
  uint64_t* empty_bar = full_bar + kStages;
  uint64_t* aux_bar = empty_bar + kStages;
  uint64_t* staged_bar = aux_bar + 2 * kMaxStoreBufs;
  uint64_t* sdone_bar = staged_bar + 2 * kMaxStoreBufs;
  float* sXpose = reinterpret_cast<float*>(smem + kSmemTotal - 1024 - kXposeBytes);

  const int warp = threadIdx.x >> 5;
  const int lane = threadIdx.x & 31;

  if (warp == 0 && lane == 0) {
    tma_prefetch_desc(&tmA);
    tma_prefetch_desc(&tmB);
    tma_prefetch_desc(&tmD);
    if (V::kAux != 1 && p.aux_tma) tma_prefetch_desc(&tmR);
  }
  if (warp == 1 && lane == 0) {
    for (int i = 0; i < kStages; ++i) {
      mbar_init(&full_bar[i], 1);
      mbar_init(&empty_bar[i], 4 * Cfg::kConsumerWGs);
    }
    for (int i = 0; i < 2 * kMaxStoreBufs; ++i) {
      mbar_init(&aux_bar[i], 1);
      mbar_init(&staged_bar[i], 1);
      mbar_init(&sdone_bar[i], 4);
    }
    fence_barrier_init();
  }
  __syncthreads();

  const int num_m = (p.M + BM - 1) / BM;
  const int num_n = (p.N + BN - 1) / BN;
  const int total = num_m * num_n * p.splits;

  if (warp == 0) {
    if (lane == 0) {
      int stage = 0;
      uint32_t phase = 0;
      const int PQ = p.g.P * p.g.Q;
      for (int w = blockIdx.x; w < total; w += gridDim.x) {
        const int n_blk = w % num_n;
        const int t = w / num_n;
        const int m_blk = t % num_m;
        const int split = t / num_m;
        const int m0 = m_blk * BM, n0 = n_blk * BN;
        const int kb0 = split * p.kb_per_split;
        const int kb1 = min(p.num_kb, kb0 + p.kb_per_split);
        int a_n = 0, a_h = 0, a_w = 0;
        if (p.a_mode == A_IM2COL) {
          a_n = m0 / PQ;
          const int rem = m0 - a_n * PQ;
          const int pp = rem / p.g.Q;
          a_h = pp * p.g.stride + p.g.lc_h;
          a_w = (rem - pp * p.g.Q) * p.g.stride + p.g.lc_w;
        }
        for (int kb = kb0; kb < kb1; ++kb) {
          mbar_wait(&empty_bar[stage], phase ^ 1);
          uint64_t* bar = &full_bar[stage];
          mbar_expect_tx(bar, kABytes + kBBytes);
          uint8_t* a_dst = sA + stage * kABytes;
          uint8_t* b_dst = sB + stage * kBBytes;
          int tap = 0, cc = kb, r = 0, s = 0;
          if (p.a_mode == A_IM2COL) {
            tap = kb / p.g.cchunks;
            cc = kb - tap * p.g.cchunks;
            r = tap / p.g.S;
            s = tap - r * p.g.S;
          }
          if (p.a_mode == A_K2D) {
            tma_load_2d(&tmA, bar, a_dst, kb * BK, m0);
          } else if (p.a_mode == A_IM2COL) {
            tma_load_im2col_4d(&tmA, bar, a_dst, cc * 64, a_w, a_h, a_n, (uint16_t)s, (uint16_t)r);
          } else {
            tma_load_2d(&tmA, bar, a_dst, m0, kb * BK);
            tma_load_2d(&tmA, bar, a_dst + 8192, m0 + 64, kb * BK);
          }
          if (p.b_mode == B_K2D) {
            tma_load_2d(&tmB, bar, b_dst, kb * BK, n0);
          } else if (p.b_mode == B_MN2D) {
            int col_base = 0, row = kb * BK;
            if (p.a_mode == A_IM2COL) {
              const int tapb = p.flip_taps ? (p.g.R * p.g.S - 1 - tap) : tap;
              col_base = tapb * p.b_cin;
              row = cc * 64;
            }
#pragma unroll
            for (int j = 0; j < BN / 64; ++j)
              tma_load_2d(&tmB, bar, b_dst + j * 8192, col_base + n0 + j * 64, row);
          } else {
            const int pix = kb * BK;
            const int bn_ = pix / PQ;
            const int rem = pix - bn_ * PQ;
            const int pp = rem / p.g.Q;
            const int bh = pp * p.g.stride + p.g.lc_h;
            const int bw = (rem - pp * p.g.Q) * p.g.stride + p.g.lc_w;
#pragma unroll
            for (int j = 0; j < BN / 64; ++j) {
              const int cb = n0 / 64 + j;
              const int tapj = cb / p.g.cchunks;
              const int ccj = cb - tapj * p.g.cchunks;
              const int rj = tapj / p.g.S;
              const int sj = tapj - rj * p.g.S;
              const bool valid = tapj < p.g.R * p.g.S;
              tma_load_im2col_4d(&tmB, bar, b_dst + j * 8192, ccj * 64, bw, bh,
                                 valid ? bn_ : p.g.n_img, (uint16_t)(valid ? sj : 0),
                                 (uint16_t)(valid ? rj : 0));
            }
          }
          if (++stage == nstages) { stage = 0; phase ^= 1; }
        }
      }
    }
    __syncwarp();
  } else if (warp >= 4 && warp < 12) {
    const int e = warp - 4;
    const int q = e & 3;
    const int half = e >> 2;
    const int gtid = threadIdx.x - 128 - half * 128;
    const int row_in_tile = (lane < 16 ? 0 : 48) + q * 16 + lane;
    const int rsw = row_in_tile & 7;
    const uint32_t bar_id = 1 + half;
    uint8_t* const sbase = sD + half * NB * kStoreBufBytes;
    uint64_t* const abar = aux_bar + half * kMaxStoreBufs;
    float* const xp = sXpose + e * 32 * kXposeStride;
    const bool direct = (flags & EPI_DIRECT) != 0;
    const bool aux_tma = V::kAux == 0 ? (p.aux_tma != 0) : (V::kAux == 2);
    constexpr int NCH = BN / 32;
    const int c_begin = half ? 2 : 0;
    const int c_end = half ? NCH : 2;
    const bool a_mn = (p.a_mode == A_MN2D), b_mn = (p.b_mode != B_K2D);
    int stage = 0;
    uint32_t phase = 0;
    const int spt = out_f32 ? (c_end - c_begin) : ((c_end - c_begin) >> 1);
    int bufi = 0;
    uint32_t aux_phase = 0;
    long long pf_w = blockIdx.x;
    int pf_j = 0, pf_b = 0;
    auto request_aux = [&]() {
      if (pf_w < total) {
        const int n_blk2 = (int)(pf_w % num_n);
        const int m_blk2 = (int)((pf_w / num_n) % num_m);
        const int col = n_blk2 * BN + (out_f32 ? (c_begin + pf_j) * 32 : ((c_begin >> 1) + pf_j) * 64);
        mbar_expect_tx(&abar[pf_b], kStoreBufBytes);
        tma_load_3d(&tmR, &abar[pf_b], sbase + pf_b * kStoreBufBytes, col, m_blk2 * BM, 0);
      }
      if (++pf_j == spt) { pf_j = 0; pf_w += gridDim.x; }
      if (++pf_b == NB) pf_b = 0;
    };
    if (aux_tma && gtid == 0 && spt > 0) {
      const int la = NB > 1 ? NB - 1 : 1;
      for (int i = 0; i < la; ++i) request_aux();
    }
    constexpr int kStatBarThreads = V::kStatsWarps ? 384 : 256;
    uint32_t sd_phase = 0;
    if (do_stats) {
      for (int j = threadIdx.x - 128; j < 2 * p.N; j += 256) sStat[j] = 0.f;
      named_bar_sync(3, kStatBarThreads);
    }
    for (int w = blockIdx.x; w < total; w += gridDim.x) {
      const int n_blk = w % num_n;
      const int t = w / num_n;
      const int m_blk = t % num_m;
      const int split = t / num_m;
      const int m0 = m_blk * BM, n0 = n_blk * BN;
      const long long row = m0 + row_in_tile;
      if (c_begin >= c_end) continue;
      float acc[2][32];
      {
        const int kb0 = split * p.kb_per_split;
        const int kb1 = min(p.num_kb, kb0 + p.kb_per_split);
        const uint32_t b_off = half * 8192u;
        if (a_mn) gemm_mainloop<BN, 1, 1>(acc, sA, sB, full_bar, empty_bar, nstages, stage, phase, kb0, kb1, b_off, lane);
        else if (b_mn) gemm_mainloop<BN, 0, 1>(acc, sA, sB, full_bar, empty_bar, nstages, stage, phase, kb0, kb1, b_off, lane);
        else gemm_mainloop<BN, 0, 0>(acc, sA, sB, full_bar, empty_bar, nstages, stage, phase, kb0, kb1, b_off, lane);
      }
#pragma unroll
      for (int ci = 0; ci < 2; ++ci) {
        const int c = c_begin + ci;
        const int col0 = n0 + c * 32;
        const int part = out_f32 ? 0 : ((c - c_begin) & 1);
        const bool s_begin = out_f32 || part == 0;
        const bool s_end = out_f32 || part == 1;
        uint8_t* const sbuf = sbase + bufi * kStoreBufBytes;
        uint8_t* const buf = sbuf + row_in_tile * 128;
        float bv = 0.f;
        if ((flags & EPI_BIAS) && col0 + lane < p.N) bv = __ldg(p.bias + col0 + lane);
        float4 rf[8];
        uint4 rb[4];
        const bool has_rf = (flags & EPI_RESID) && row < p.M;
        const bool has_rb = (flags & (EPI_RESID_BF16 | EPI_MUL_DGELU | EPI_MUL_DRELU)) && row < p.M;
        float rscale = 1.f;
        if ((flags & EPI_ROW_SCALE) && row < p.M) rscale = __ldg(p.row_scale + row / p.rows_per_scale);
        uint32_t mbits = 0u;
        if ((flags & EPI_MASK_BITS) && row < p.M && col0 < p.N) mbits = __ldg(p.mask_bits + row * (p.N >> 5) + (col0 >> 5));
        if (!aux_tma) {
          if (has_rf) {
            const float4* rp = reinterpret_cast<const float4*>(p.resid + row * p.ldd + col0);
#pragma unroll
            for (int j = 0; j < 8; ++j) rf[j] = (col0 + 4 * j < p.N) ? __ldg(rp + j) : make_float4(0.f, 0.f, 0.f, 0.f);
          }
          if (has_rb) {
            const uint4* rp = reinterpret_cast<const uint4*>(
                reinterpret_cast<const __nv_bfloat16*>(p.resid_bf16) + row * p.ldd + col0);
#pragma unroll
            for (int j = 0; j < 4; ++j) rb[j] = (col0 + 8 * j < p.N) ? __ldg(rp + j) : make_uint4(0, 0, 0, 0);
          }
        }
        __syncwarp();
#pragma unroll
        for (int blk = 0; blk < 2; ++blk) {
#pragma unroll
          for (int jj = 0; jj < 4; ++jj) {
            const int j = ci * 4 + jj;
            float* const dst = xp + (blk * 16 + (lane >> 2)) * kXposeStride + jj * 8 + 2 * (lane & 3);
            dst[0] = acc[blk][4 * j];
            dst[1] = acc[blk][4 * j + 1];
            dst[8 * kXposeStride] = acc[blk][4 * j + 2];
            dst[8 * kXposeStride + 1] = acc[blk][4 * j + 3];
          }
        }
        __syncwarp();
        float f[32];
#pragma unroll
        for (int j = 0; j < 32; ++j) f[j] = xp[lane * kXposeStride + j];
        if (aux_tma) {
          if (s_begin) mbar_wait(&abar[bufi], (aux_phase >> bufi) & 1u);
          if (out_f32) {
#pragma unroll
            for (int j = 0; j < 8; ++j) rf[j] = *reinterpret_cast<const float4*>(buf + ((j ^ rsw) << 4));
          } else {
#pragma unroll
            for (int j = 0; j < 4; ++j) rb[j] = *reinterpret_cast<const uint4*>(buf + (((part * 4 + j) ^ rsw) << 4));
          }
        }
        if (flags & EPI_BIAS) {
#pragma unroll
          for (int j = 0; j < 32; ++j) f[j] += __shfl_sync(0xffffffffu, bv, j);
        }
        if (flags & EPI_GELU) {
#pragma unroll
          for (int j = 0; j < 32; ++j) f[j] = gelu_erf(f[j]);
        }
        if (flags & EPI_RELU) {
#pragma unroll
          for (int j = 0; j < 32; ++j) f[j] = fmaxf(f[j], 0.f);
        }
        if (flags & EPI_ROW_SCALE) {
#pragma unroll
          for (int j = 0; j < 32; ++j) f[j] *= rscale;
        }
        if (flags & EPI_RESID) {
          if (aux_tma || has_rf) {
#pragma unroll
            for (int j = 0; j < 8; ++j) {
              f[4 * j] += rf[j].x; f[4 * j + 1] += rf[j].y; f[4 * j + 2] += rf[j].z; f[4 * j + 3] += rf[j].w;
            }
          }
        }
        if (flags & (EPI_RESID_BF16 | EPI_MUL_DGELU | EPI_MUL_DRELU)) {
          if (aux_tma || has_rb) {
#pragma unroll
            for (int j = 0; j < 4; ++j) {
              const uint32_t wv[4] = {rb[j].x, rb[j].y, rb[j].z, rb[j].w};
#pragma unroll
              for (int u = 0; u < 4; ++u) {
                const float2 ab = __bfloat1622float2(*reinterpret_cast<const __nv_bfloat162*>(&wv[u]));
                if (flags & EPI_MUL_DGELU) {
                  f[8 * j + 2 * u] *= gelu_erf_grad(ab.x);
                  f[8 * j + 2 * u + 1] *= gelu_erf_grad(ab.y);
                } else if (flags & EPI_MUL_DRELU) {
                  f[8 * j + 2 * u] = ab.x > 0.f ? f[8 * j + 2 * u] : 0.f;
                  f[8 * j + 2 * u + 1] = ab.y > 0.f ? f[8 * j + 2 * u + 1] : 0.f;
                } else {
                  f[8 * j + 2 * u] += ab.x;
                  f[8 * j + 2 * u + 1] += ab.y;
                }
              }
            }
          }
        }
        if (flags & EPI_MASK_BITS) {
#pragma unroll
          for (int j = 0; j < 32; ++j) f[j] *= ((mbits >> j) & 1u) ? 1.f : 0.f;
        }
        if (direct) {
          if (row < p.M) {
            if (out_f32) {
              float* o = reinterpret_cast<float*>(p.out) + split * p.split_stride + row * p.ldd + col0;
#pragma unroll
              for (int j = 0; j < 32; j += 4)
                if (col0 + j < p.N)
                  *reinterpret_cast<float4*>(o + j) = make_float4(f[j], f[j + 1], f[j + 2], f[j + 3]);
            } else {
              __nv_bfloat16* o = reinterpret_cast<__nv_bfloat16*>(p.out) + split * p.split_stride +
                                 row * p.ldd + col0;
#pragma unroll
              for (int j = 0; j < 32; j += 8)
                if (col0 + j < p.N)
                  *reinterpret_cast<uint4*>(o + j) =
                      make_uint4(pack_bf16x2(f[j], f[j + 1]), pack_bf16x2(f[j + 2], f[j + 3]),
                                 pack_bf16x2(f[j + 4], f[j + 5]), pack_bf16x2(f[j + 6], f[j + 7]));
            }
          }
        } else {
          if (s_begin && !aux_tma) {
            if (gtid == 0) {
              tma_store_wait_read_n(NB - 1);
              if (V::kStatsWarps && do_stats) {
                mbar_wait(&sdone_bar[half * kMaxStoreBufs + bufi], ((sd_phase >> bufi) & 1u) ^ 1u);
                sd_phase ^= (1u << bufi);
              }
            }
            named_bar_sync(bar_id, 128);
          }
          if (out_f32) {
#pragma unroll
            for (int j = 0; j < 8; ++j)
              *reinterpret_cast<float4*>(buf + ((j ^ rsw) << 4)) =
                  make_float4(f[4 * j], f[4 * j + 1], f[4 * j + 2], f[4 * j + 3]);
          } else {
#pragma unroll
            for (int j = 0; j < 4; ++j)
              *reinterpret_cast<uint4*>(buf + (((part * 4 + j) ^ rsw) << 4)) =
                  make_uint4(pack_bf16x2(f[8 * j], f[8 * j + 1]), pack_bf16x2(f[8 * j + 2], f[8 * j + 3]),
                             pack_bf16x2(f[8 * j + 4], f[8 * j + 5]), pack_bf16x2(f[8 * j + 6], f[8 * j + 7]));
          }
          if (s_end) {
            fence_proxy_async_smem();
            named_bar_sync(bar_id, 128);
            const int scol = out_f32 ? col0 : col0 - 32;
            if (gtid == 0) {
              if (scol < p.N) {
                asm volatile(
                    "cp.async.bulk.tensor.3d.global.shared::cta.bulk_group [%0, {%2, %3, %4}], [%1];" ::"l"(
                        reinterpret_cast<uint64_t>(&tmD)),
                    "r"(smem_u32(sbuf)), "r"(scol), "r"(m0), "r"(split)
                    : "memory");
              }
              tma_store_commit();
              if (aux_tma) {
                tma_store_wait_read_n(NB > 1 ? 1 : 0);
                request_aux();
              }
            }
            if (V::kStatsWarps && do_stats) {
              if (gtid == 0) mbar_arrive(&staged_bar[half * kMaxStoreBufs + bufi]);
            } else if (do_stats) {
              const int wq = gtid >> 5;
              const int piece = lane & 3;
              const int chunk = wq * 2 + (piece >> 1);
              const int r0 = lane >> 2;
              const uint8_t* const sp = sbuf + r0 * 128 + ((chunk ^ r0) << 4) + (piece & 1) * 8;
              float sx[4] = {0.f, 0.f, 0.f, 0.f}, sq[4] = {0.f, 0.f, 0.f, 0.f};
#pragma unroll
              for (int i = 0; i < 16; ++i) {
                const uint2 w2 = *reinterpret_cast<const uint2*>(sp + i * 1024);
                const float a0 = __uint_as_float(w2.x << 16), a1 = __uint_as_float(w2.x & 0xffff0000u);
                const float b0 = __uint_as_float(w2.y << 16), b1 = __uint_as_float(w2.y & 0xffff0000u);
                sx[0] += a0; sq[0] = fmaf(a0, a0, sq[0]);
                sx[1] += a1; sq[1] = fmaf(a1, a1, sq[1]);
                sx[2] += b0; sq[2] = fmaf(b0, b0, sq[2]);
                sx[3] += b1; sq[3] = fmaf(b1, b1, sq[3]);
              }
#pragma unroll
              for (int o = 4; o < 32; o <<= 1) {
#pragma unroll
                for (int j = 0; j < 4; ++j) {
                  sx[j] += __shfl_xor_sync(0xffffffffu, sx[j], o);
                  sq[j] += __shfl_xor_sync(0xffffffffu, sq[j], o);
                }
              }
              const int gcol = scol + wq * 16 + piece * 4;
              if (lane < 4 && gcol < p.N) {
#pragma unroll
                for (int j = 0; j < 4; ++j) {
                  sStat[gcol + j] += sx[j];
                  sStat[p.N + gcol + j] += sq[j];
                }
              }
            }
            aux_phase ^= (1u << bufi);
            if (++bufi == NB) bufi = 0;
          }
        }
      }
    }
    if (gtid == 0) tma_store_wait<0>();
    if (do_stats) {
      named_bar_sync(3, kStatBarThreads);
      float* dst = p.stats_partial + (long long)blockIdx.x * 2 * p.N;
      for (int j = threadIdx.x - 128; j < 2 * p.N; j += 256) dst[j] = sStat[j];
    }
  } else if (V::kStatsWarps && warp >= 12) {
    if (do_stats) {
      const int wq = warp - 12;
      const int piece = lane & 3;
      const int chunk = wq * 2 + (piece >> 1);
      const int r0 = lane >> 2;
      const int soff = r0 * 128 + ((chunk ^ r0) << 4) + (piece & 1) * 8;
      constexpr int NCH = BN / 32;
      constexpr int split_at = 2 * ((BN / 64 + 1) / 2);
      constexpr int spt_h[2] = {split_at / 2, (NCH - split_at) / 2};
      int sb[2] = {0, 0};
      uint32_t st_phase[2] = {0u, 0u};
      named_bar_sync(3, 384);
      for (int w = blockIdx.x; w < total; w += gridDim.x) {
        const int n0 = (w % num_n) * BN;
#pragma unroll 1
        for (int j = 0; j < spt_h[0]; ++j) {
#pragma unroll 1
          for (int h = 0; h < 2; ++h) {
            if (j >= spt_h[h]) continue;
            const int b = sb[h];
            mbar_wait(&staged_bar[h * kMaxStoreBufs + b], (st_phase[h] >> b) & 1u);
            const uint8_t* const sp = sD + (h * NB + b) * kStoreBufBytes + soff;
            float sx[4] = {0.f, 0.f, 0.f, 0.f}, sq[4] = {0.f, 0.f, 0.f, 0.f};
#pragma unroll
            for (int i = 0; i < 16; ++i) {
              const uint2 w2 = *reinterpret_cast<const uint2*>(sp + i * 1024);
              const float a0 = __uint_as_float(w2.x << 16), a1 = __uint_as_float(w2.x & 0xffff0000u);
              const float b0 = __uint_as_float(w2.y << 16), b1 = __uint_as_float(w2.y & 0xffff0000u);
              sx[0] += a0; sq[0] = fmaf(a0, a0, sq[0]);
              sx[1] += a1; sq[1] = fmaf(a1, a1, sq[1]);
              sx[2] += b0; sq[2] = fmaf(b0, b0, sq[2]);
              sx[3] += b1; sq[3] = fmaf(b1, b1, sq[3]);
            }
            __syncwarp();
            if (lane == 0) mbar_arrive(&sdone_bar[h * kMaxStoreBufs + b]);
#pragma unroll
            for (int o = 4; o < 32; o <<= 1) {
#pragma unroll
              for (int k = 0; k < 4; ++k) {
                sx[k] += __shfl_xor_sync(0xffffffffu, sx[k], o);
                sq[k] += __shfl_xor_sync(0xffffffffu, sq[k], o);
              }
            }
            const int gcol = n0 + ((h ? split_at : 0) / 2 + j) * 64 + wq * 16 + piece * 4;
            if (lane < 4 && gcol < p.N) {
#pragma unroll
              for (int k = 0; k < 4; ++k) {
                sStat[gcol + k] += sx[k];
                sStat[p.N + gcol + k] += sq[k];
              }
            }
            st_phase[h] ^= (1u << b);
            sb[h] = (b + 1 == NB) ? 0 : b + 1;
          }
        }
      }
      named_bar_sync(3, 384);
    }
  }
}

}
```

### simpleaicv_pytorch_training_examples_b200/engine/convnet.py

```python
import torch

from .. import ops
from .operands import CONV, STEM, Linear, Operand, rows_wgrad

ACT_NONE, ACT_RELU, ACT_LEAKY, ACT_SILU = 0, 1, 2, 3
FUSE_BN_STATS = True


def _round_up(v, m):
    return (v + m - 1) // m * m


class GradSink:

    def __init__(self):
        self.views = {}
        self.on_ready = None
        self.on_backward_end = None

    def buffer_for(self, param):
        v = self.views.get(id(param))
        if v is None:
            v = torch.empty_like(param, dtype=torch.float32)
            self.views[id(param)] = v
        return v

    def begin(self, param):
        buf = self.buffer_for(param)
        if param.grad is None:
            return buf, False
        if param.grad.data_ptr() != buf.data_ptr():
            buf.copy_(param.grad)
        return buf, True

    def done(self, param, buf):
        param.grad = buf
        if self.on_ready is not None:
            self.on_ready(param)


_NBT_BATCH = None


def _flush_nbt():
    global _NBT_BATCH
    pending, _NBT_BATCH = _NBT_BATCH, None
    if pending:
        torch._foreach_add_(pending, 1)


class ConvBN:

    def __init__(self, block, act, res_after_act=False):
        self.conv = block.layer[0]
        self.bn = block.layer[1]
        self.act = act
        self.res_after_act = res_after_act
        k, c, r, s = self.conv.weight.shape
        self.k, self.c, self.r, self.s = k, c, r, s
        self.stride = self.conv.stride[0]
        self.pad = self.conv.padding[0]
        assert self.conv.groups == 1 and self.conv.bias is None and r == s
        assert self.conv.stride[0] == self.conv.stride[1] and self.conv.padding[0] == self.conv.padding[1]
        self.is_stem = (c % 8) != 0
        self.kp = _round_up(k, 64)
        self.cp = c if self.is_stem else _round_up(c, 64)
        self.padded = self.kp != k
        self.op = Operand(self.conv.weight, STEM if self.is_stem else CONV, kp=self.kp, cp=self.cp)
        self.kpad = self.op.kpad
        self.sums = None

    @property
    def w_bf16(self):
        return self.op.w

    def prep(self):
        bn = self.bn
        dev = self.op.refresh().device
        if self.sums is None or self.sums.device != dev:
            self.sums = torch.zeros(2, self.kp, device=dev)
            if self.padded:
                self.gamma_p = torch.ones(self.kp, device=dev)
                self.beta_p = torch.zeros(self.kp, device=dev)
                self.rm_p = torch.zeros(self.kp, device=dev)
                self.rv_p = torch.ones(self.kp, device=dev)
                self.dg_p = torch.empty(self.kp, device=dev)
                self.db_p = torch.empty(self.kp, device=dev)
        if self.padded:
            self.gamma_p[:self.k].copy_(bn.weight.detach())
            self.beta_p[:self.k].copy_(bn.bias.detach())

    def _gamma(self):
        return self.gamma_p if self.padded else self.bn.weight.detach()

    def _beta(self):
        return self.beta_p if self.padded else self.bn.bias.detach()

    def out_hw(self, h, w):
        return (ops.conv_out_size(h, self.pad, self.r, self.stride),
                ops.conv_out_size(w, self.pad, self.s, self.stride))

    def conv_fwd(self, a_in, tape, want_stats=False):
        if self.is_stem:
            n, _, h, w = a_in.shape
        else:
            n, h, w, cin = a_in.shape
            assert cin == self.cp, f'expected {self.cp} (padded) input channels, got {cin}'
        P, Q = self.out_hw(h, w)
        rows = n * P * Q
        stats = ops.partial_ws(a_in.device, 2 * self.kp) if want_stats else None
        tape['stats'] = (stats, ops.gemm_stats_rows(rows, self.kp)) if want_stats else None
        if self.is_stem:
            cols = ops.stem_im2col(a_in, self.r, self.s, self.stride, self.pad, self.kpad)
            y = ops.linear_fwd(cols, self.op.w, stats=stats).view(n, P, Q, self.kp)
            tape['cols'] = cols
        else:
            cs = ops.make_conv_shape(n, h, w, self.cp, self.kp, self.r, self.s, self.stride, self.pad)
            y = ops.conv_fprop(a_in, self.op.w, cs, stats=stats)
            tape['a_in'] = a_in
            tape['cs'] = cs
        tape['in_hw'] = (h, w)
        tape['y'] = y
        return y

    def bn_prepare(self, y, training, tape):
        bn = self.bn
        rows = y.numel() // self.kp
        track = bn.track_running_stats
        ss = tape['ss'] = torch.empty(2, self.kp, device=y.device)
        saved = tape['saved'] = torch.empty(2, self.kp, device=y.device)
        if training or not track:
            momentum = bn.momentum if bn.momentum is not None else 0.1
            fused = tape.get('stats') if tape is not None else None
            if fused is not None:
                partials, prow = fused
            else:
                partials, prow = ops.bn_stats(y), 0
            if self.padded and track:
                self.rm_p[:self.k].copy_(bn.running_mean)
                self.rv_p[:self.k].copy_(bn.running_var)
            rm = (self.rm_p if self.padded else bn.running_mean) if track else None
            rv = (self.rv_p if self.padded else bn.running_var) if track else None
            ops.bn_finalize(partials, self._gamma(), self._beta(), rm, rv, ss, saved, rows, bn.eps, momentum,
                            partial_rows=prow)
            if self.padded and track:
                bn.running_mean.copy_(self.rm_p[:self.k])
                bn.running_var.copy_(self.rv_p[:self.k])
            if track and bn.num_batches_tracked is not None:
                if _NBT_BATCH is not None:
                    _NBT_BATCH.append(bn.num_batches_tracked)
                else:
                    bn.num_batches_tracked.add_(1)
        else:
            scale = bn.weight.detach() * torch.rsqrt(bn.running_var + bn.eps)
            ss.zero_()
            ss[0, :self.k].copy_(scale)
            ss[1, :self.k].copy_(bn.bias.detach() - bn.running_mean * scale)

    def forward(self, a_in, tape, training, res=None, res_ss=None, want_mask=False):
        y = self.conv_fwd(a_in, tape, want_stats=training and FUSE_BN_STATS)
        self.bn_prepare(y, training, tape)
        out = torch.empty_like(y)
        act = self.act | (8 if (self.res_after_act and res is not None) else 0)
        bits = tape['bits'] = ops.mask_bits_like(y) if want_mask else None
        ops.bn_apply(y, tape['ss'], out, act, res=res, res_scale_shift=res_ss, mask_bits=bits)
        tape['out'] = out
        return out

    def _grad_targets(self, sink):
        gbuf, gacc = sink.begin(self.bn.weight)
        bbuf, bacc = sink.begin(self.bn.bias)
        assert gacc == bacc
        if self.padded:
            return (self.gamma_p, self.dg_p, self.db_p, False), (gbuf, bbuf, gacc)
        return (self.bn.weight.detach(), gbuf, bbuf, gacc), (gbuf, bbuf, gacc)

    def _grad_done(self, sink, bufs):
        gbuf, bbuf, acc = bufs
        if self.padded:
            if acc:
                gbuf.add_(self.dg_p[:self.k])
                bbuf.add_(self.db_p[:self.k])
            else:
                gbuf.copy_(self.dg_p[:self.k])
                bbuf.copy_(self.db_p[:self.k])
        sink.done(self.bn.weight, gbuf)
        sink.done(self.bn.bias, bbuf)

    def bn_bwd(self, dout, tape, sink, bits=None, want_dres=False, act=None):
        act = self.act if act is None else act
        y = tape['y']
        ss = tape['ss'] if (act != ACT_NONE and bits is None) else None
        saved = tape['saved']
        ops.bn_bwd_reduce(dout, None, y, saved, self.sums, act, scale_shift=ss, bits=bits)
        dy = torch.empty_like(y)
        dres = torch.empty_like(y) if want_dres else None
        (gamma, dg, db, acc), bufs = self._grad_targets(sink)
        ops.bn_bwd_apply(dout, None, y, saved, gamma, self.sums, dy, dres, dg, db, act, accumulate=acc,
                         scale_shift=ss, bits=bits)
        self._grad_done(sink, bufs)
        return dy, dres

    def bn_bwd_pair(self, other, g, tape, other_tape, sink, bits):
        y, yo = tape['y'], other_tape['y']
        sums = torch.empty(4, self.kp, device=y.device)
        ops.bn_bwd_reduce2(g, bits, y, yo, tape['saved'], other_tape['saved'], sums)
        dy, dyo = torch.empty_like(y), torch.empty_like(yo)
        (ga, dga, dba, acca), bufs_a = self._grad_targets(sink)
        (gb, dgb, dbb, accb), bufs_b = other._grad_targets(sink)
        ops.bn_bwd_apply2(g, bits, y, yo, tape['saved'], other_tape['saved'], ga, gb, sums, dy, dyo, dga, dba, dgb, dbb,
                          accumulate_a=acca, accumulate_b=accb)
        self._grad_done(sink, bufs_a)
        other._grad_done(sink, bufs_b)
        return dy, dyo

    def conv_bwd(self, dy, tape, sink, need_dx=True, add=None, mask_bits=None):
        w = self.conv.weight
        wbuf, wacc = sink.begin(w)
        n, P, Q, _ = dy.shape
        h, wd = tape['in_hw']
        if self.is_stem:
            part = ops.linear_wgrad(dy.view(-1, self.kp), tape['cols'])
            ops.finish_conv_wgrad(part, wbuf, self.kpad, accumulate=wacc, order=ops.ORDER_CRS, kp=self.kp)
            sink.done(w, wbuf)
            assert not need_dx, 'the stem has no data gradient'
            return None
        cs = tape['cs']
        part = ops.conv_wgrad(dy, tape['a_in'], cs)
        ops.finish_conv_wgrad(part, wbuf, self.kpad, accumulate=wacc, kp=self.kp, cp=self.cp)
        sink.done(w, wbuf)
        if not need_dx:
            return None
        if self.stride == 1:
            return ops.conv_dgrad(dy, self.op.w, cs, add=add, mask_bits=mask_bits)
        assert self.stride == 2
        if self.r == 1:
            assert add is None and mask_bits is None
            return 'strided', ops.linear_dgrad(dy.view(-1, self.kp), self.op.w).view(n, P, Q, self.cp)
        u = ops.zero_upsample2(dy, h, wd)
        cs1 = ops.make_conv_shape(n, h, wd, self.cp, self.kp, self.r, self.s, 1, self.pad)
        return ops.conv_dgrad(u, self.op.w, cs1, add=add, mask_bits=mask_bits)


class ResidualBlockRT:

    def __init__(self, block):
        names = ['conv1', 'conv2'] + (['conv3'] if hasattr(block, 'conv3') else [])
        self.units = []
        for nm in names:
            self.units.append(ConvBN(getattr(block, nm), ACT_RELU))
        self.down = ConvBN(block.downsample_conv, ACT_NONE) if block.downsample else None

    def all_units(self):
        return self.units + ([self.down] if self.down is not None else [])

    def forward(self, a_in, tape, training):
        tapes = tape.setdefault('u', [dict() for _ in self.units])
        x = a_in
        for u, t in zip(self.units[:-1], tapes[:-1]):
            x = u.forward(x, t, training)
        last, tl = self.units[-1], tapes[-1]
        if self.down is not None:
            td = tape.setdefault('d', dict())
            yd = self.down.conv_fwd(a_in, td, want_stats=training and FUSE_BN_STATS)
            self.down.bn_prepare(yd, training, td)
            out = last.forward(x, tl, training, res=yd, res_ss=td['ss'], want_mask=training)
        else:
            out = last.forward(x, tl, training, res=a_in, want_mask=training)
        return out

    @staticmethod
    def out_mask(tape):
        tapes = tape.get('u')
        return tapes[-1].get('bits') if tapes else None

    def backward(self, dout, tape, sink):
        return self.backward_chain(dout, tape, sink)[0]

    def backward_chain(self, dout, tape, sink, dout_masked=False, in_mask=None):
        tapes = tape['u']
        last, tl = self.units[-1], tapes[-1]
        bits = None if dout_masked else tl['bits']
        strided = None
        if self.down is None:
            dy, g = last.bn_bwd(dout, tl, sink, bits=bits, want_dres=not dout_masked,
                                act=ACT_NONE if dout_masked else None)
            shortcut = dout if dout_masked else g
        else:
            td = tape['d']
            dy, dyd = last.bn_bwd_pair(self.down, dout, tl, td, sink, bits)
            shortcut = self.down.conv_bwd(dyd, td, sink)
            if isinstance(shortcut, tuple):
                strided, shortcut = shortcut[1], None
        first_unit = self.units[0]
        fuse = shortcut is not None and not (first_unit.stride == 2 and first_unit.r == 1)
        mask = in_mask if fuse else None
        n_main = len(self.units) - 1
        dx = last.conv_bwd(dy, tl, sink, add=shortcut if (fuse and n_main == 0) else None,
                           mask_bits=mask if n_main == 0 else None)
        for i, (u, t) in enumerate(zip(reversed(self.units[:-1]), reversed(tapes[:-1]))):
            dy, _ = u.bn_bwd(dx, t, sink)
            dx = u.conv_bwd(dy, t, sink, add=shortcut if (fuse and i == n_main - 1) else None,
                            mask_bits=mask if i == n_main - 1 else None)
        if shortcut is not None and not fuse:
            ops.add_bf16(dx, shortcut)
        if strided is not None:
            ops.add_strided2(dx, strided)
        return dx, mask is not None


def blocks_backward(blocks, tapes, da, sink):
    masked = False
    for i in reversed(range(len(blocks))):
        b, t = blocks[i], tapes[i]
        if 'ckpt_in' in t:
            b.forward(t.pop('ckpt_in'), t, True)
        if isinstance(b, ResidualBlockRT):
            prev = blocks[i - 1] if i > 0 else None
            in_mask = prev.out_mask(tapes[i - 1]) if isinstance(prev, ResidualBlockRT) else None
            da, masked = b.backward_chain(da, t, sink, dout_masked=masked, in_mask=in_mask)
        else:
            assert not masked
            da = b.backward(da, t, sink)
        t.clear()
    return da


class PlainUnitRT:

    def __init__(self, block, act):
        self.unit = ConvBN(block, act)

    def all_units(self):
        return [self.unit]

    def forward(self, a_in, tape, training):
        return self.unit.forward(a_in, tape, training)

    def backward(self, dout, tape, sink):
        dy, _ = self.unit.bn_bwd(dout, tape, sink)
        return self.unit.conv_bwd(dy, tape, sink)


class DarkBlockRT:

    def __init__(self, block, act):
        self.u1 = ConvBN(block.conv[0], act)
        self.u2 = ConvBN(block.conv[1], act, res_after_act=True)

    def all_units(self):
        return [self.u1, self.u2]

    def forward(self, a_in, tape, training):
        t1, t2 = tape.setdefault('u', [dict(), dict()])
        return self.u2.forward(self.u1.forward(a_in, t1, training), t2, training, res=a_in)

    def backward(self, dout, tape, sink):
        t1, t2 = tape['u']
        dy, _ = self.u2.bn_bwd(dout, t2, sink)
        dx = self.u2.conv_bwd(dy, t2, sink)
        dy, _ = self.u1.bn_bwd(dx, t1, sink)
        return self.u1.conv_bwd(dy, t1, sink, add=dout)


class MaxPoolRT:

    def __init__(self, k, stride, pad=0, pad_hi=None, oob_zero=False):
        self.k, self.stride, self.pad, self.pad_hi, self.oob_zero = k, stride, pad, pad_hi, oob_zero

    def all_units(self):
        return []

    def forward(self, a_in, tape, training):
        tape['in_hw'] = (a_in.shape[1], a_in.shape[2])
        out, tape['argmax'] = ops.maxpool_fwd(a_in, self.k, self.stride, self.pad, self.pad_hi, self.oob_zero)
        return out

    def backward(self, dout, tape, sink):
        h, w = tape['in_hw']
        return ops.maxpool_bwd(dout, tape['argmax'], h, w, self.k, self.stride, self.pad, self.pad_hi)


class FcHeadRT:

    def __init__(self, fc):
        self.fc = fc
        self.lin = Linear(fc)
        self.op = self.lin.op

    def prep(self):
        self.lin.prep()

    def forward(self, a, tape):
        tape['feat_hw'] = (a.shape[1], a.shape[2])
        pooled = ops.avgpool_fwd(a)
        feat = self.fc.weight.shape[1]
        if pooled.shape[1] != feat:
            pooled = pooled[:, :feat].contiguous()
        return self.fc_forward(pooled, tape)

    def fc_forward(self, pooled, tape):
        tape['pooled'] = pooled
        ncls = self.fc.weight.shape[0]
        logits = self.lin.fwd(pooled, out_f32=True)
        if logits.shape[1] != ncls:
            logits = logits[:, :ncls].contiguous()
        return logits

    def backward(self, dlogits, tape, sink, cpad):
        dpooled = self.fc_backward(dlogits, tape, sink)
        feat = self.fc.weight.shape[1]
        if cpad != feat:
            full = torch.zeros(dpooled.shape[0], cpad, device=dpooled.device, dtype=torch.bfloat16)
            full[:, :feat] = dpooled
            dpooled = full
        h, w = tape['feat_hw']
        return ops.avgpool_bwd(dpooled, h, w)

    def fc_backward(self, dlogits, tape, sink):
        ncls = self.fc.weight.shape[0]
        npad = self.op.w.shape[0]
        dlogits = dlogits.contiguous().float()
        bbuf, bacc = sink.begin(self.fc.bias)
        ops.colsum(dlogits, bbuf, accumulate=bacc)
        sink.done(self.fc.bias, bbuf)
        dl = torch.zeros(dlogits.shape[0], npad, device=dlogits.device, dtype=torch.bfloat16)
        if npad == ncls:
            ops.cast_bf16(dlogits, dl)
        else:
            dl[:, :ncls] = dlogits.to(torch.bfloat16)
        rows_wgrad(dl, tape['pooled'], self.fc.weight, sink)
        return ops.linear_dgrad(dl, self.op.w)


class ConvHeadRT:

    def __init__(self, conv):
        self.conv = conv
        assert conv.kernel_size == (1, 1) and conv.bias is not None
        self.lin = Linear(conv)
        self.op = self.lin.op

    def prep(self):
        self.lin.prep()

    def forward(self, a, tape):
        n, h, w, c = a.shape
        tape['a_in'] = a
        y = self.lin.fwd(a.view(n * h * w, c))
        pooled = ops.avgpool_fwd(y.view(n, h, w, -1))
        return pooled[:, :self.conv.weight.shape[0]].float()

    def backward(self, dlogits, tape, sink, cpad):
        a = tape['a_in']
        n, h, w, c = a.shape
        ncls = self.conv.weight.shape[0]
        npad = self.op.w.shape[0]
        dl = torch.zeros(n, npad, device=a.device, dtype=torch.bfloat16)
        dl[:, :ncls] = dlogits.to(torch.bfloat16)
        dy = ops.avgpool_bwd(dl, h, w).view(n * h * w, npad)
        bias = self.conv.bias
        rows_wgrad(dy, a.view(n * h * w, c), self.conv.weight, sink)
        bbuf, bacc = sink.begin(bias)
        full = torch.empty(npad, device=a.device)
        ops.colsum(dy, full)
        bbuf.copy_(full[:ncls] + bbuf if bacc else full[:ncls])
        sink.done(bias, bbuf)
        return ops.linear_dgrad(dy, self.op.w).view(n, h, w, c)


class ResNetRT:

    def __init__(self, model, has_maxpool, stem=None, blocks=None, head=None, checkpoint=False):
        self.model = model
        self.has_maxpool = has_maxpool
        if stem is None:
            stem = ConvBN(model.conv1, ACT_RELU)
            blocks = []
            for layer in (model.layer1, model.layer2, model.layer3, model.layer4):
                for blk in layer:
                    blocks.append(ResidualBlockRT(blk))
        self.stem = stem
        self.blocks = blocks
        self.head = head if head is not None else FcHeadRT(model.fc)
        self.checkpoint = checkpoint
        self.sink = GradSink()
        self._units = self.units() + [self.head]

    def units(self):
        us = [self.stem]
        for b in self.blocks:
            us += b.all_units()
        return us

    def operands(self):
        return [u.op for u in self._units]

    def prep(self):
        for u in self._units:
            u.prep()

    def stem_forward(self, x, tape, training):
        a = self.stem.forward(x, tape['stem'], training)
        if self.has_maxpool:
            tape['pool_in_hw'] = (a.shape[1], a.shape[2])
            a, tape['argmax'] = ops.maxpool3x3s2_fwd(a)
        return a

    def head_forward(self, a, tape):
        tape['feat_c'] = a.shape[3]
        return self.head.forward(a, tape)

    def forward(self, x, training, keep_tape):
        assert x.is_cuda and x.dtype == torch.float32 and x.dim() == 4
        global _NBT_BATCH
        x = x.contiguous()
        self.prep()
        tape = {'stem': {}, 'blocks': [dict() for _ in self.blocks]}
        _NBT_BATCH = [] if training else None
        try:
            a = self.stem_forward(x, tape, training)
            ckpt = self.checkpoint and keep_tape
            for b, t in zip(self.blocks, tape['blocks']):
                if ckpt:
                    t['ckpt_in'] = a
                    a = b.forward(a, {}, training)
                else:
                    a = b.forward(a, t, training)
            logits = self.head_forward(a, tape)
        finally:
            _flush_nbt()
        return logits, (tape if keep_tape else None)

    def head_backward(self, dlogits, tape):
        return self.head.backward(dlogits, tape, self.sink, tape['feat_c'])

    def stem_backward(self, da, tape):
        if self.has_maxpool:
            ph, pw = tape['pool_in_hw']
            da = ops.maxpool3x3s2_bwd(da, tape['argmax'], ph, pw)
        dy, _ = self.stem.bn_bwd(da, tape['stem'], self.sink)
        self.stem.conv_bwd(dy, tape['stem'], self.sink, need_dx=False)

    def backward(self, dlogits, tape):
# ... 32 lines not shown
```

### simpleaicv_pytorch_training_examples_b200/ops.py

```python
import ctypes

import torch

from . import _lib
from ._lib import ConvShape

EPI_BIAS, EPI_RELU, EPI_GELU, EPI_DIRECT, EPI_RESID, EPI_ADD_BF16, EPI_MUL_DRELU = 1, 2, 4, 8, 16, 32, 512


def _p(t):
    if t is None:
        return None
    assert t.is_cuda and t.is_contiguous(), 'saicv ops need contiguous CUDA tensors'
    return ctypes.c_void_p(t.data_ptr())


def _stream():
    return ctypes.c_void_p(torch.cuda.current_stream().cuda_stream)


def conv_out_size(h, pad, r, stride):
    return (h + 2 * pad - r) // stride + 1


def make_conv_shape(n, h, w, c, k, r, s, stride, pad):
    return ConvShape(n, h, w, c, k, r, s, stride, pad)


def gemm_stats_rows(out_rows, out_cols):
    return _lib.load().saicv_gemm_stats_rows(out_rows, out_cols)


def linear_fwd(x, w, bias=None, resid=None, out=None, flags=0, out_f32=False, row_scale=None, rows_per_scale=0,
               stats=None):
    M, K = x.shape
    N = w.shape[0]
    assert x.dtype == torch.bfloat16 and w.dtype == torch.bfloat16 and w.shape[1] == K
    if out is None:
        out = torch.empty(M, N, device=x.device, dtype=torch.float32 if out_f32 else torch.bfloat16)
    _lib.call('saicv_linear_fwd', _p(x), _p(w), _p(bias), _p(resid), _p(row_scale), rows_per_scale, _p(stats),
              _p(out), M, N, K, flags, int(out_f32), _stream())
    return out


def linear_dgrad(dy, w, resid=None, out=None, flags=0, out_f32=False, gelu_pre=None, relu_out=None, add=None):
    M, N = dy.shape
    K = w.shape[1]
    assert dy.dtype == torch.bfloat16 and w.dtype == torch.bfloat16 and w.shape[0] == N
    assert (gelu_pre is not None) + (relu_out is not None) + (add is not None) <= 1
    if relu_out is not None:
        gelu_pre, flags = relu_out, flags | EPI_MUL_DRELU
    elif add is not None:
        gelu_pre, flags = add, flags | EPI_ADD_BF16
    if out is None:
        out = torch.empty(M, K, device=dy.device, dtype=torch.float32 if out_f32 else torch.bfloat16)
    _lib.call('saicv_linear_dgrad', _p(dy), _p(w), _p(resid), _p(gelu_pre), _p(out), M, N, K, flags,
              int(out_f32), _stream())
    return out


def wgrad_splits(out_rows, out_cols, reduce_len):
    return _lib.load().saicv_wgrad_splits(out_rows, out_cols, reduce_len)


def linear_wgrad(dy, x, partial=None):
    M, N = dy.shape
    K = x.shape[1]
    splits = wgrad_splits(N, K, M)
    if partial is None:
        partial = torch.empty(splits, N, K, device=dy.device, dtype=torch.float32)
    _lib.call('saicv_linear_wgrad', _p(dy), _p(x), _p(partial), M, N, K, splits, _stream())
    return partial


def reduce_partials(partial, out, accumulate=False):
    splits = partial.shape[0]
    n = out.numel()
    _lib.call('saicv_reduce_partials', _p(partial), _p(out), splits, n, int(accumulate), _stream())
    return out


def conv_fprop(x, w, cs, out=None, flags=0, stats=None):
    P = conv_out_size(cs.h, cs.pad, cs.r, cs.stride)
    Q = conv_out_size(cs.w, cs.pad, cs.s, cs.stride)
    if out is None:
        out = torch.empty(cs.n, P, Q, cs.k, device=x.device, dtype=torch.bfloat16)
    _lib.call('saicv_conv_fprop', _p(x), _p(w), _p(stats), _p(out), ctypes.byref(cs), flags, _stream())
    return out


def conv_dgrad(dy, w, cs, out=None, add=None, mask_bits=None):
    if out is None:
        out = torch.empty(cs.n, cs.h, cs.w, cs.c, device=dy.device, dtype=torch.bfloat16)
    _lib.call('saicv_conv_dgrad', _p(dy), _p(w), _p(add), _p(mask_bits), _p(out), ctypes.byref(cs), _stream())
    return out


def conv_wgrad(dy, x, cs, partial=None):
    P = conv_out_size(cs.h, cs.pad, cs.r, cs.stride)
    Q = conv_out_size(cs.w, cs.pad, cs.s, cs.stride)
    ncols = cs.r * cs.s * cs.c
    splits = wgrad_splits(cs.k, ncols, cs.n * P * Q)
    if partial is None:
        partial = torch.empty(splits, cs.k, ncols, device=dy.device, dtype=torch.float32)
    _lib.call('saicv_conv_wgrad', _p(dy), _p(x), _p(partial), ctypes.byref(cs), splits, _stream())
    return partial


ORDER_RSC, ORDER_CRS = 0, 1


def prep_conv_weight(w_f32, out, kpad, order=ORDER_RSC, kp=0, cp=0):
    k, c, r, s = w_f32.shape
    _lib.call('saicv_prep_conv_weight', _p(w_f32), _p(out), k, c, r, s, kpad, order, kp, cp, _stream())
    return out


def finish_conv_wgrad(partial, grad, kpad, accumulate=False, order=ORDER_RSC, kp=0, cp=0):
    k, c, r, s = grad.shape
    _lib.call('saicv_finish_conv_wgrad', _p(partial), _p(grad), partial.shape[0], k, c, r, s, kpad,
              int(accumulate), order, kp, cp, _stream())
    return grad


def cast_bf16(src, out=None):
    if out is None:
        out = torch.empty(src.shape, device=src.device, dtype=torch.bfloat16)
    _lib.call('saicv_cast_bf16', _p(src), _p(out), src.numel(), _stream())
    return out


def u8_normalize(images, mean, std, out=None):
    import ctypes
    assert images.is_cuda and images.dtype == torch.uint8 and images.dim() == 4 and images.shape[3] == 3 and images.is_contiguous()
    n, h, w, _ = images.shape
    if out is None:
        out = torch.empty(n, 3, h, w, device=images.device, dtype=torch.float32)
    m3 = (ctypes.c_float * 3)(*[float(v) for v in mean])
    s3 = (ctypes.c_float * 3)(*[float(v) for v in std])
    _lib.call('saicv_u8_nhwc_to_nchw_norm', _p(images), _p(out), n, h, w, m3, s3, _stream())
    return out


def nchw_to_nhwc_bf16(x, out=None):
    n, c, h, w = x.shape
    if out is None:
        out = torch.empty(n, h, w, c, device=x.device, dtype=torch.bfloat16)
    _lib.call('saicv_nchw_to_nhwc_bf16', _p(x), _p(out), n, c, h, w, _stream())
    return out


def stem_kpad(c, r, s):
    return (c * r * ((s + 7) // 8 * 8) + 63) // 64 * 64


def stem_im2col(x, r, s, stride, pad, kpad, out=None):
    n, c, h, w = x.shape
    P, Q = conv_out_size(h, pad, r, stride), conv_out_size(w, pad, s, stride)
    if out is None:
        out = torch.empty(n * P * Q, kpad, device=x.device, dtype=torch.bfloat16)
    _lib.call('saicv_stem_im2col', _p(x), _p(out), n, c, h, w, r, s, stride, pad, kpad, _stream())
    return out


def zero_upsample2(dy, h, w, out=None):
    n, p, q, c = dy.shape
    if out is None:
        out = torch.empty(n, h, w, c, device=dy.device, dtype=torch.bfloat16)
    _lib.call('saicv_zero_upsample2', _p(dy), _p(out), n, p, q, h, w, c, _stream())
    return out


def add_strided2(dx, dd):
    n, h, w, c = dx.shape
    _, p, q, _ = dd.shape
    _lib.call('saicv_add_strided2', _p(dx), _p(dd), n, p, q, h, w, c, _stream())
    return dx


_WS = {}


def partial_ws(device, ncols):
    key = (device, ncols)
    ws = _WS.get(key)
    if ws is None:
        ws = _WS[key] = torch.empty(_lib.BN_PARTIAL_ROWS * ncols, device=device, dtype=torch.float32)
    return ws


def bn_stats(y, partials=None):
    c = y.shape[-1]
    if partials is None:
        partials = partial_ws(y.device, 2 * c)
    _lib.call('saicv_bn_stats', _p(y), _p(partials), y.numel() // c, c, _stream())
    return partials


def bn_finalize(stats, gamma, beta, rmean, rvar, scale_shift, saved, rows, eps, momentum, partial_rows=0):
    c = gamma.numel()
    _lib.call('saicv_bn_finalize', _p(stats), partial_rows, _p(gamma), _p(beta), _p(rmean), _p(rvar),
              _p(scale_shift), _p(saved), rows, c, eps, momentum, _stream())


def mask_bits_like(y):
    c = y.shape[-1]
    return torch.empty(y.numel() // c, c // 32, device=y.device, dtype=torch.int32)


def bn_apply(y, scale_shift, out, act, res=None, res_scale_shift=None, mask_bits=None):
    c = y.shape[-1]
    _lib.call('saicv_bn_apply', _p(y), _p(scale_shift), _p(res), _p(res_scale_shift), _p(out), _p(mask_bits),
              y.numel() // c, c, act, _stream())
    return out


def bn_bwd_reduce(dout, out, y, saved, sums, act, scale_shift=None, bits=None):
    c = y.shape[-1]
    _lib.call('saicv_bn_bwd_reduce', _p(dout), _p(out), _p(bits), _p(y), _p(saved), _p(scale_shift),
              _p(partial_ws(y.device, 2 * c)), _p(sums), y.numel() // c, c, act, _stream())


def bn_bwd_apply(dout, out, y, saved, gamma, sums, dy, dres, dgamma, dbeta, act, accumulate=False,
                 scale_shift=None, bits=None):
    c = y.shape[-1]
    _lib.call('saicv_bn_bwd_apply', _p(dout), _p(out), _p(bits), _p(y), _p(saved), _p(gamma), _p(scale_shift),
              _p(sums), _p(dy), _p(dres), _p(dgamma), _p(dbeta), y.numel() // c, c, act,
              int(accumulate), _stream())


def bn_bwd_reduce2(g, bits, y_a, y_b, saved_a, saved_b, sums):
    c = y_a.shape[-1]
    _lib.call('saicv_bn_bwd_reduce2', _p(g), _p(bits), _p(y_a), _p(y_b), _p(saved_a), _p(saved_b),
              _p(partial_ws(g.device, 4 * c)), _p(sums), y_a.numel() // c, c, _stream())


def bn_bwd_apply2(g, bits, y_a, y_b, saved_a, saved_b, gamma_a, gamma_b, sums, dy_a, dy_b, dgamma_a, dbeta_a,
                  dgamma_b, dbeta_b, accumulate_a=False, accumulate_b=False):
    c = y_a.shape[-1]
    _lib.call('saicv_bn_bwd_apply2', _p(g), _p(bits), _p(y_a), _p(y_b), _p(saved_a), _p(saved_b), _p(gamma_a),
              _p(gamma_b), _p(sums), _p(dy_a), _p(dy_b), _p(dgamma_a), _p(dbeta_a), _p(dgamma_b), _p(dbeta_b),
              y_a.numel() // c, c, int(accumulate_a), int(accumulate_b), _stream())


def add_bf16(a, b):
    _lib.call('saicv_add_bf16', _p(a), _p(b), a.numel(), _stream())
    return a


def maxpool3x3s2_fwd(x, out=None, argmax=None):
    n, h, w, c = x.shape
    P, Q = conv_out_size(h, 1, 3, 2), conv_out_size(w, 1, 3, 2)
    if out is None:
        out = torch.empty(n, P, Q, c, device=x.device, dtype=torch.bfloat16)
    if argmax is None:
        argmax = torch.empty(n, P, Q, c, device=x.device, dtype=torch.uint8)
    _lib.call('saicv_maxpool3x3s2_fwd', _p(x), _p(out), _p(argmax), n, h, w, c, _stream())
    return out, argmax


def maxpool3x3s2_bwd(dy, argmax, h, w, out=None):
    n, _, _, c = dy.shape
    if out is None:
        out = torch.empty(n, h, w, c, device=dy.device, dtype=torch.bfloat16)
    _lib.call('saicv_maxpool3x3s2_bwd', _p(dy), _p(argmax), _p(out), n, h, w, c, _stream())
    return out


def maxpool_fwd(x, k, stride, pad=0, pad_hi=None, oob_zero=False):
    n, h, w, c = x.shape
    pad_hi = pad if pad_hi is None else pad_hi
    P, Q = (h + pad + pad_hi - k) // stride + 1, (w + pad + pad_hi - k) // stride + 1
    out = torch.empty(n, P, Q, c, device=x.device, dtype=torch.bfloat16)
    argmax = torch.empty(n, P, Q, c, device=x.device, dtype=torch.uint8)
    _lib.call('saicv_maxpool_fwd', _p(x), _p(out), _p(argmax), n, h, w, c, k, stride, pad, pad_hi, int(oob_zero), _stream())
    return out, argmax


def maxpool_bwd(dy, argmax, h, w, k, stride, pad=0, pad_hi=None):
    n, _, _, c = dy.shape
    pad_hi = pad if pad_hi is None else pad_hi
    out = torch.empty(n, h, w, c, device=dy.device, dtype=torch.bfloat16)
    _lib.call('saicv_maxpool_bwd', _p(dy), _p(argmax), _p(out), n, h, w, c, k, stride, pad, pad_hi, _stream())
    return out


def avgpool_fwd(x, out=None):
    n, h, w, c = x.shape
    if out is None:
        out = torch.empty(n, c, device=x.device, dtype=torch.bfloat16)
    _lib.call('saicv_avgpool_fwd', _p(x), _p(out), n, h * w, c, _stream())
    return out


def avgpool_bwd(dy, h, w, out=None):
    n, c = dy.shape
    if out is None:
        out = torch.empty(n, h, w, c, device=dy.device, dtype=torch.bfloat16)
    _lib.call('saicv_avgpool_bwd', _p(dy), _p(out), n, h * w, c, _stream())
    return out


def colsum(x, out, accumulate=False):
    c = x.shape[-1]
    is_f32 = x.dtype == torch.float32
    ws = None if is_f32 else partial_ws(x.device, c)
    _lib.call('saicv_colsum', _p(x), _p(ws), _p(out), x.numel() // c, c, int(accumulate), int(is_f32), _stream())
    return out


def token_gather_fwd(src, idx, fill, pos=None, pos_idx=None, out=None):
    b, s_rows, c = src.shape
    r = idx.shape[1]
    assert src.dtype == torch.float32 and idx.dtype == torch.int32 and idx.shape[0] == b and src.is_contiguous() and idx.is_contiguous()
    if out is None:
        out = torch.empty(b, r, c, device=src.device, dtype=torch.float32)
    _lib.call('saicv_token_gather_fwd', _p(src), s_rows, _p(idx), _p(fill), _p(pos), _p(pos_idx), _p(out), b, r, c, _stream())
    return out


def token_gather_bwd(dout, idx, src_rows, dsrc_dtype=torch.bfloat16, want_fill=True, zero=True):
    b, r, c = dout.shape
    assert dout.dtype == torch.float32 and dout.is_contiguous() and dsrc_dtype in (torch.bfloat16, torch.float32)
    dsrc = (torch.zeros if zero else torch.empty)(b, src_rows, c, device=dout.device, dtype=dsrc_dtype)
    part = dfill = None
    if want_fill:
        nslab = _lib.load().saicv_token_fill_slabs(b * r)
        part = torch.empty(nslab, c, device=dout.device, dtype=torch.float32)
    _lib.call('saicv_token_gather_bwd', _p(dout), _p(idx), _p(dsrc), int(dsrc_dtype == torch.bfloat16), src_rows, _p(part), b, r, c, _stream())
    if want_fill:
        dfill = torch.empty(c, device=dout.device, dtype=torch.float32)
        reduce_partials(part, dfill)
    return dsrc, dfill


def layernorm_fwd(x, gamma, beta, eps, out=None, stats=None):
    rows, c = x.numel() // x.shape[-1], x.shape[-1]
    assert x.dtype == torch.float32
    if out is None:
        out = torch.empty(x.shape, device=x.device, dtype=torch.bfloat16)
    if stats is None:
        stats = torch.empty(2, rows, device=x.device, dtype=torch.float32)
    _lib.call('saicv_layernorm_fwd', _p(x), _p(gamma), _p(beta), _p(out), _p(stats), rows, c, eps, _stream())
    return out, stats


def layernorm_bwd(dy, x, gamma, stats, dgamma, dbeta, dres=None, dx=None, dx_bf16=None, accumulate=False,
                  bf16_row_scale=None, rows_per_scale=0):
    rows, c = x.numel() // x.shape[-1], x.shape[-1]
    assert dy.dtype == torch.bfloat16 and x.dtype == torch.float32
    if dx is None:
        dx = torch.empty(x.shape, device=x.device, dtype=torch.float32)
    _lib.call('saicv_layernorm_bwd', _p(dy), _p(x), _p(gamma), _p(stats), _p(dres), _p(dx), _p(dx_bf16),
              _p(bf16_row_scale), rows_per_scale, _p(partial_ws(x.device, 2 * c)), _p(dgamma), _p(dbeta), rows, c,
              int(accumulate), _stream())
    return dx


def gelu_fwd(u, out=None):
    if out is None:
        out = torch.empty_like(u)
    _lib.call('saicv_gelu_fwd', _p(u), _p(out), u.numel(), _stream())
    return out


def gelu_bwd(dh, u, out=None):
    if out is None:
        out = torch.empty_like(u)
    _lib.call('saicv_gelu_bwd', _p(dh), _p(u), _p(out), u.numel(), _stream())
    return out


def vit_assemble_tokens(patch, cls, pos, b, np_, c, out=None):
    if out is None:
        out = torch.empty(b, np_ + 1, c, device=patch.device, dtype=torch.float32)
    _lib.call('saicv_vit_assemble_tokens', _p(patch), _p(cls), _p(pos), _p(out), b, np_, c, _stream())
    return out


def vit_assemble_tokens_bwd(dx, dpos, dcls, dpatch, accumulate=False):
    b, l, c = dx.shape
    _lib.call('saicv_vit_assemble_tokens_bwd', _p(dx), _p(dpos), _p(dcls), _p(dpatch), b, l - 1, c,
              int(accumulate), _stream())
    return dpatch


def token_pool_fwd(x, mean_pool, out=None):
    b, l, c = x.shape
    if out is None:
        out = torch.empty(b, c, device=x.device, dtype=torch.float32)
    _lib.call('saicv_token_pool_fwd', _p(x), _p(out), b, l, c, int(mean_pool), _stream())
    return out


def token_pool_bwd(dpooled, l, mean_pool, dx=None, dx_bf16=None, bf16_row_scale=None):
    b, c = dpooled.shape
    if dx is None:
        dx = torch.empty(b, l, c, device=dpooled.device, dtype=torch.float32)
    _lib.call('saicv_token_pool_bwd', _p(dpooled), _p(dx), _p(dx_bf16), _p(bf16_row_scale), b, l, c,
              int(mean_pool), _stream())
    return dx


def attention_fwd(qkv, b, l, h, d, scale, out=None, lse=None):
    if out is None:
        out = torch.empty(b * l, h * d, device=qkv.device, dtype=torch.bfloat16)
    if lse is None:
        lse = torch.empty(b, h, l, device=qkv.device, dtype=torch.float32)
    _lib.call('saicv_attention_fwd', _p(qkv), _p(out), _p(lse), b, l, h, d, scale, _stream())
    return out, lse


def attention_bwd(qkv, out, dout, lse, b, l, h, d, scale, dqkv=None):
    if dqkv is None:
        dqkv = torch.empty_like(qkv)
    delta = torch.empty(b, h, l, device=qkv.device, dtype=torch.float32)
    _lib.call('saicv_attention_bwd', _p(qkv), _p(out), _p(dout), _p(lse), _p(delta), _p(dqkv), b, l, h, d, scale, _stream())
    return dqkv


def _bhl_strides(t):
    assert t.dim() == 4 and t.stride(3) == 1 and t.dtype == torch.bfloat16 and t.is_cuda
    return (ctypes.c_longlong * 3)(t.stride(0), t.stride(1), t.stride(2))

# ... 299 lines not shown
```

Baseline: 5561.

## Add phase-decomposed stride-2 conv dgrad and transposed weight-gradient GEMM

```diff
diff --git a/include/saicv_b200.h b/include/saicv_b200.h
--- a/include/saicv_b200.h
+++ b/include/saicv_b200.h
@@ -28,6 +28,7 @@
 int saicv_linear_wgrad(const void* dy, const void* x, float* dw_partial, int M, int N, int K,
                        int splits, void* stream);
 int saicv_wgrad_splits(int out_rows, int out_cols, long long reduce_len);
+int saicv_wgrad_transposed(int out_rows, int out_cols);
 
 typedef struct {
   int n, h, w, c;
@@ -44,7 +45,7 @@
 int saicv_prep_conv_weight(const float* w, void* w_bf16, int k, int c, int r, int s, int kpad,
                            int order, int kp, int cp, void* stream);
 int saicv_finish_conv_wgrad(const float* partial, float* grad, int splits, int k, int c, int r,
-                            int s, int kpad, int accumulate, int order, int kp, int cp, void* stream);
+                            int s, int kpad, int accumulate, int order, int kp, int cp, int transposed, void* stream);
 int saicv_reduce_partials(const float* partial, float* out, int splits, long long n,
                           int accumulate, void* stream);
 int saicv_cast_bf16(const float* src, void* dst, long long n, void* stream);
diff --git a/simpleaicv_pytorch_training_examples_b200/_lib.py b/simpleaicv_pytorch_training_examples_b200/_lib.py
--- a/simpleaicv_pytorch_training_examples_b200/_lib.py
+++ b/simpleaicv_pytorch_training_examples_b200/_lib.py
@@ -40,11 +40,12 @@
     'saicv_linear_dgrad': [c_void_p, c_void_p, c_void_p, c_void_p, c_void_p, c_int, c_int, c_int, c_int, c_int, c_void_p],
     'saicv_linear_wgrad': [c_void_p, c_void_p, c_void_p, c_int, c_int, c_int, c_int, c_void_p],
     'saicv_wgrad_splits': [c_int, c_int, c_ll],
+    'saicv_wgrad_transposed': [c_int, c_int],
     'saicv_conv_fprop': [c_void_p, c_void_p, c_void_p, c_void_p, ctypes.POINTER(ConvShape), c_int, c_void_p],
     'saicv_conv_dgrad': [c_void_p, c_void_p, c_void_p, c_void_p, c_void_p, ctypes.POINTER(ConvShape), c_void_p],
     'saicv_conv_wgrad': [c_void_p, c_void_p, c_void_p, ctypes.POINTER(ConvShape), c_int, c_void_p],
     'saicv_prep_conv_weight': [c_void_p, c_void_p, c_int, c_int, c_int, c_int, c_int, c_int, c_int, c_int, c_void_p],
-    'saicv_finish_conv_wgrad': [c_void_p, c_void_p, c_int, c_int, c_int, c_int, c_int, c_int, c_int, c_int, c_int, c_int, c_void_p],
+    'saicv_finish_conv_wgrad': [c_void_p, c_void_p, c_int, c_int, c_int, c_int, c_int, c_int, c_int, c_int, c_int, c_int, c_int, c_void_p],
     'saicv_reduce_partials': [c_void_p, c_void_p, c_int, c_ll, c_int, c_void_p],
     'saicv_cast_bf16': [c_void_p, c_void_p, c_ll, c_void_p],
     'saicv_nchw_to_nhwc_bf16': [c_void_p, c_void_p, c_int, c_int, c_int, c_int, c_void_p],
diff --git a/simpleaicv_pytorch_training_examples_b200/csrc/capi_elementwise.cu b/simpleaicv_pytorch_training_examples_b200/csrc/capi_elementwise.cu
--- a/simpleaicv_pytorch_training_examples_b200/csrc/capi_elementwise.cu
+++ b/simpleaicv_pytorch_training_examples_b200/csrc/capi_elementwise.cu
@@ -649,7 +649,7 @@
 
 __global__ void finish_conv_wgrad_kernel(const float* __restrict__ partial, float* __restrict__ grad, int splits,
                                          int K, int C, int R, int S, int kpad, int accumulate, int order, int Kp,
-                                         int Cp) {
+                                         int Cp, int transposed) {
   const long long total = (long long)K * C * R * S;
   for (long long i = (long long)blockIdx.x * blockDim.x + threadIdx.x; i < total;
        i += (long long)gridDim.x * blockDim.x) {
@@ -657,8 +657,8 @@
     const long long kc = i / (R * S);
     const int c = (int)(kc % C), k = (int)(kc / C);
     const int S8 = (S + 7) & ~7;
-    const long long src = order == 1 ? (long long)k * kpad + (long long)(c * R + tap / S) * S8 + tap % S
-                                     : (long long)k * kpad + (long long)tap * Cp + c;
+    const long long col = order == 1 ? (long long)(c * R + tap / S) * S8 + tap % S : (long long)tap * Cp + c;
+    const long long src = transposed ? col * Kp + k : (long long)k * kpad + col;
     float s = accumulate ? grad[i] : 0.f;
     for (int sp = 0; sp < splits; ++sp) s += partial[(long long)sp * Kp * kpad + src];
     grad[i] = s;
@@ -1085,11 +1085,12 @@
 }
 
 int saicv_finish_conv_wgrad(const float* partial, float* grad, int splits, int k, int c, int r, int s, int kpad,
-                            int accumulate, int order, int kp, int cp, void* stream) {
+                            int accumulate, int order, int kp, int cp, int transposed, void* stream) {
   if (kp <= 0) kp = k;
   if (cp <= 0) cp = c;
   finish_conv_wgrad_kernel<<<grid_for((long long)k * c * r * s), kThreads, 0, ST>>>(partial, grad, splits, k, c, r,
-                                                                                     s, kpad, accumulate, order, kp, cp);
+                                                                                     s, kpad, accumulate, order, kp, cp,
+                                                                                     transposed);
   return check_launch("finish_conv_wgrad_kernel");
 }
 
diff --git a/simpleaicv_pytorch_training_examples_b200/csrc/capi_gemm.cu b/simpleaicv_pytorch_training_examples_b200/csrc/capi_gemm.cu
--- a/simpleaicv_pytorch_training_examples_b200/csrc/capi_gemm.cu
+++ b/simpleaicv_pytorch_training_examples_b200/csrc/capi_gemm.cu
@@ -88,6 +88,22 @@
     set_error("cuTensorMapEncodeTiled(out) failed: %d (cols=%llu rows=%llu ldd=%llu splits=%llu)", (int)r,
               (unsigned long long)cols, (unsigned long long)rows, (unsigned long long)ldd,
               (unsigned long long)splits);
+    return false;
+  }
+  return true;
+}
+
+bool encode_out_phases(CUtensorMap* m, void* ptr, uint64_t c, uint64_t np, uint64_t q, uint32_t rows) {
+  cuuint64_t dims[5] = {c, 2, q, 2, np};
+  cuuint64_t strides[4] = {c * 2, 2 * c * 2, 2 * q * c * 2, 4 * q * c * 2};
+  cuuint32_t box[5] = {64u, 1u, (cuuint32_t)q, 1u, rows};
+  cuuint32_t estr[5] = {1, 1, 1, 1, 1};
+  CUresult r = g_encode_tiled(m, CU_TENSOR_MAP_DATA_TYPE_BFLOAT16, 5, ptr, dims, strides, box, estr,
+                              CU_TENSOR_MAP_INTERLEAVE_NONE, CU_TENSOR_MAP_SWIZZLE_128B,
+                              CU_TENSOR_MAP_L2_PROMOTION_L2_256B, CU_TENSOR_MAP_FLOAT_OOB_FILL_NONE);
+  if (r != CUDA_SUCCESS) {
+    set_error("cuTensorMapEncodeTiled(phase out) failed: %d (c=%llu rows=%llu q=%llu box rows=%u)", (int)r,
+              (unsigned long long)c, (unsigned long long)np, (unsigned long long)q, rows);
     return false;
   }
   return true;
@@ -156,8 +172,8 @@
     if (e != cudaSuccess) return set_error("cudaFuncSetAttribute(smem=%d): %s", Cfg::kSmemBytes, cudaGetErrorString(e));
     attr_set = true;
   }
-  const int num_m = (p.M + BM - 1) / BM, num_n = (p.N + BN - 1) / BN;
-  const long long total = (long long)num_m * num_n * p.splits;
+  const int num_m = (p.M + p.tile_rows - 1) / p.tile_rows, num_n = (p.N + BN - 1) / BN;
+  const long long total = (long long)num_m * num_n * p.splits * p.phases;
   const int grid = (int)(total < g_sm_count ? total : g_sm_count);
   const int stat_bytes = (p.epi_flags & EPI_STATS) ? ((8 * p.N + 15) & ~15) : 0;
   int stages = 0, nb = 1;
@@ -188,6 +204,8 @@
              cudaStream_t st, const void* aux = nullptr, bool aux_f32 = false) {
   CUtensorMap r = d;
   p.aux_tma = 0;
+  if (p.tile_rows == 0) p.tile_rows = BM;
+  if (p.phases == 0) p.phases = 1;
   const bool both = (p.epi_flags & EPI_RESID) && (p.epi_flags & (EPI_RESID_BF16 | EPI_MUL_DGELU | EPI_MUL_DRELU));
   if (aux && !both && !(p.epi_flags & EPI_DIRECT) && p.splits == 1 && aux_f32 == (p.out_f32 != 0) && aligned16(aux) &&
       !getenv("SAICV_GEMM_NO_AUX_TMA")) {
@@ -195,7 +213,13 @@
     p.aux_tma = 1;
   }
   int var = VAR_FULL;
-  if (!getenv("SAICV_GEMM_FULL_VARIANT")) {
+  if (p.a_mode == A_IM2COL_MN && (p.epi_flags || !p.out_f32 || getenv("SAICV_GEMM_FULL_VARIANT")))
+    return set_error("the transposed conv weight gradient runs on the plain fp32 epilogue (VAR_PLAIN_F32) only");
+  if (p.phases > 1 || p.tile_rows != BM) {
+    if (p.epi_flags || p.aux_tma || p.out_f32 || p.splits != 1)
+      return set_error("the phase data gradient has a plain bf16 epilogue: no epilogue flags, aux operand or split-K");
+    var = VAR_PHASE_BF16;
+  } else if (!getenv("SAICV_GEMM_FULL_VARIANT")) {
     if (p.aux_tma && !(p.epi_flags & ~GemmVariant<VAR_AUX>::kMask)) var = VAR_AUX;
     else if (!p.aux_tma && !p.out_f32 && !(p.epi_flags & ~GemmVariant<VAR_PLAIN_BF16>::kMask))
       var = ((p.epi_flags & EPI_STATS) && !getenv("SAICV_GEMM_INLINE_STATS")) ? VAR_STATS_BF16 : VAR_PLAIN_BF16;
@@ -209,6 +233,7 @@
     case VAR_STATS_BF16: return launch<BN_, VAR_STATS_BF16>(a, b, d, r, p, st);      \
     case VAR_PLAIN_F32: return launch<BN_, VAR_PLAIN_F32>(a, b, d, r, p, st);        \
     case VAR_AUX: return launch<BN_, VAR_AUX>(a, b, d, r, p, st);                    \
+    case VAR_PHASE_BF16: return launch<BN_, VAR_PHASE_BF16>(a, b, d, r, p, st);      \
     default: return launch<BN_, VAR_FULL>(a, b, d, r, p, st);                        \
   }
   switch (bn) {
@@ -216,6 +241,41 @@
     default: SAICV_LAUNCH_BN(128)
   }
 #undef SAICV_LAUNCH_BN
+}
+
+int conv_dgrad_phases(const void* dy, const void* w, const void* add, const uint32_t* mask_bits, void* dx,
+                      const saicv_conv_shape* cs, cudaStream_t st) {
+  if (cs->r != 3 || cs->s != 3 || cs->pad != 1 || cs->h % 2 || cs->w % 2 || cs->w / 2 > BM)
+    return set_error("saicv_conv_dgrad: stride 2 needs a 3x3 pad-1 conv on even h, w with w <= %d (r=%d s=%d pad=%d "
+                     "h=%d w=%d); zero-upsample dy and pass stride 1 otherwise", 2 * BM, cs->r, cs->s, cs->pad, cs->h, cs->w);
+  if (add || mask_bits) return set_error("saicv_conv_dgrad: stride 2 takes no `add` / `mask_bits`");
+  const int P = cs->h / 2, Q = cs->w / 2;
+  const int rows = BM / Q;
+  CUtensorMap ta, tb, td;
+  if (!encode_im2col(&ta, dy, cs->n, P, Q, cs->k, 0, 0, 0, 0, 1, 128)) return 2;
+  const int Kw = 9 * cs->c;
+  if (!encode_2d(&tb, w, CU_TENSOR_MAP_DATA_TYPE_BFLOAT16, 2, Kw, cs->k, Kw, 64, 64)) return 2;
+  if (!encode_out_phases(&td, dx, cs->c, (uint64_t)cs->n * P, Q, rows)) return 2;
+  GemmParams p{};
+  p.M = cs->n * P * Q; p.N = cs->c; p.num_kb = 4 * (cs->k / 64); p.kb_per_split = p.num_kb; p.splits = 1;
+  p.a_mode = A_IM2COL; p.b_mode = B_MN2D; p.b_cin = cs->c;
+  p.g.P = P; p.g.Q = Q; p.g.stride = 1; p.g.lc_h = 0; p.g.lc_w = 0;
+  p.g.R = 3; p.g.S = 3; p.g.cchunks = cs->k / 64; p.g.n_img = cs->n;
+  p.epi_flags = 0; p.out_f32 = 0; p.out = dx; p.ldd = cs->c;
+  p.tile_rows = rows * Q;
+  p.phases = 4;
+  const int taps1[2][2] = {{1, -1}, {2, 0}};
+  const int order[4] = {3, 1, 2, 0};
+  for (int i = 0; i < 4; ++i) {
+    const int a = order[i] >> 1, b = order[i] & 1;
+    p.ph_out[i] = order[i];
+    p.ph_taps[i] = (1 + a) * (1 + b);
+    int t = 0;
+    for (int dr = 0; dr <= a; ++dr)
+      for (int ds = 0; ds <= b; ++ds)
+        p.ph_tab[i][t++] = (taps1[a][dr] * 3 + taps1[b][ds]) | (dr << 8) | (ds << 9);
+  }
+  return dispatch(pick_bn(cs->c), ta, tb, td, p, st);
 }
 
 }
@@ -229,6 +289,13 @@
   const long long tiles = ((out_rows + BM - 1) / BM) * ((out_cols + bn - 1) / bn);
   const int sms = ensure_init() ? g_sm_count : 132;
   return (int)(tiles < sms ? tiles : sms);
+}
+
+int saicv_wgrad_transposed(int out_rows, int out_cols) {
+  const int bn = pick_bn(out_cols), bnt = pick_bn(out_rows);
+  const long long cost = (long long)((out_rows + BM - 1) / BM) * BM * ((out_cols + bn - 1) / bn) * bn;
+  const long long cost_t = (long long)((out_cols + BM - 1) / BM) * BM * ((out_rows + bnt - 1) / bnt) * bnt;
+  return cost_t < cost ? 1 : 0;
 }
 
 int saicv_wgrad_splits(int out_rows, int out_cols, long long reduce_len) {
@@ -351,7 +418,9 @@
   if (!ensure_init()) return 1;
   if (cs->c % 64 || cs->k % 64 || !aligned16(dy) || !aligned16(w) || !aligned16(dx))
     return set_error("saicv_conv_dgrad: needs c%%64==0 and k%%64==0 (c=%d k=%d)", cs->c, cs->k);
-  if (cs->stride != 1) return set_error("saicv_conv_dgrad: stride must be 1 (zero-upsample dy for strided convs)");
+  if (cs->stride == 2) return conv_dgrad_phases(dy, w, add, mask_bits, dx, cs, (cudaStream_t)stream);
+  if (cs->stride != 1)
+    return set_error("saicv_conv_dgrad: stride %d (1, or 2 for 3x3 pad 1 on even sizes)", cs->stride);
   const long long M = (long long)cs->n * cs->h * cs->w;
   const int Kw = cs->r * cs->s * cs->c;
   const int bn = pick_bn(cs->c);
@@ -380,22 +449,27 @@
   const int P = conv_out(cs->h, cs->pad, cs->r, cs->stride), Q = conv_out(cs->w, cs->pad, cs->s, cs->stride);
   const long long Mpix = (long long)cs->n * P * Q;
   const int Ncols = cs->r * cs->s * cs->c;
-  const int bn = pick_bn(Ncols);
-  CUtensorMap ta, tb, td;
-  if (!encode_2d(&ta, dy, CU_TENSOR_MAP_DATA_TYPE_BFLOAT16, 2, cs->k, Mpix, cs->k, 64, 64)) return 2;
-  if (!encode_im2col(&tb, x, cs->n, cs->h, cs->w, cs->c, -cs->pad, -cs->pad, cs->pad - (cs->r - 1),
+  const bool tr = saicv_wgrad_transposed(cs->k, Ncols) != 0;
+  const int bn = pick_bn(tr ? cs->k : Ncols);
+  CUtensorMap ta, tb, td;
+  CUtensorMap& tdy = tr ? tb : ta;
+  CUtensorMap& tx = tr ? ta : tb;
+  if (!encode_2d(&tdy, dy, CU_TENSOR_MAP_DATA_TYPE_BFLOAT16, 2, cs->k, Mpix, cs->k, 64, 64)) return 2;
+  if (!encode_im2col(&tx, x, cs->n, cs->h, cs->w, cs->c, -cs->pad, -cs->pad, cs->pad - (cs->r - 1),
                      cs->pad - (cs->s - 1), cs->stride, 64))
     return 2;
-  if (!encode_out(&td, dw_partial, true, Ncols, cs->k, Ncols, splits, (uint64_t)cs->k * Ncols)) return 2;
-  GemmParams p{};
-  p.M = cs->k; p.N = Ncols; p.num_kb = (int)((Mpix + BK - 1) / BK);
+  if (tr ? !encode_out(&td, dw_partial, true, cs->k, Ncols, cs->k, splits, (uint64_t)cs->k * Ncols)
+         : !encode_out(&td, dw_partial, true, Ncols, cs->k, Ncols, splits, (uint64_t)cs->k * Ncols))
+    return 2;
+  GemmParams p{};
+  p.M = tr ? Ncols : cs->k; p.N = tr ? cs->k : Ncols; p.num_kb = (int)((Mpix + BK - 1) / BK);
   p.kb_per_split = (p.num_kb + splits - 1) / splits;
   p.splits = (p.num_kb + p.kb_per_split - 1) / p.kb_per_split;
   if (p.splits != splits) return set_error("saicv_conv_wgrad: splits=%d leaves an empty split (use saicv_wgrad_splits)", splits);
-  p.a_mode = A_MN2D; p.b_mode = B_IM2COL;
+  p.a_mode = tr ? A_IM2COL_MN : A_MN2D; p.b_mode = tr ? B_MN2D : B_IM2COL;
   p.g.P = P; p.g.Q = Q; p.g.stride = cs->stride; p.g.lc_h = -cs->pad; p.g.lc_w = -cs->pad;
   p.g.R = cs->r; p.g.S = cs->s; p.g.cchunks = cs->c / 64; p.g.n_img = cs->n;
-  p.epi_flags = 0; p.out_f32 = 1; p.out = dw_partial; p.ldd = Ncols; p.split_stride = (long long)cs->k * Ncols;
+  p.epi_flags = 0; p.out_f32 = 1; p.out = dw_partial; p.ldd = p.N; p.split_stride = (long long)cs->k * Ncols;
   return dispatch(bn, ta, tb, td, p, (cudaStream_t)stream);
 }
 
diff --git a/simpleaicv_pytorch_training_examples_b200/csrc/gemm_sm90.cuh b/simpleaicv_pytorch_training_examples_b200/csrc/gemm_sm90.cuh
--- a/simpleaicv_pytorch_training_examples_b200/csrc/gemm_sm90.cuh
+++ b/simpleaicv_pytorch_training_examples_b200/csrc/gemm_sm90.cuh
@@ -4,7 +4,7 @@
 
 namespace saicv {
 
-enum : int { A_K2D = 0, A_IM2COL = 1, A_MN2D = 2 };
+enum : int { A_K2D = 0, A_IM2COL = 1, A_MN2D = 2, A_IM2COL_MN = 3 };
 enum : int { B_K2D = 0, B_MN2D = 2, B_IM2COL = 3 };
 enum : int { EPI_BIAS = 1, EPI_RELU = 2, EPI_GELU = 4, EPI_DIRECT = 8, EPI_RESID = 16, EPI_RESID_BF16 = 32,
               EPI_MUL_DGELU = 64, EPI_ROW_SCALE = 128, EPI_STATS = 256, EPI_MUL_DRELU = 512, EPI_MASK_BITS = 1024 };
@@ -62,19 +62,26 @@
   int aux_tma;
   float* stats_partial;
   const uint32_t* mask_bits;
+  int tile_rows;
+  int phases;
+  int ph_out[4];
+  int ph_taps[4];
+  int ph_tab[4][4];
 };
 
-enum : int { VAR_FULL = 0, VAR_PLAIN_BF16 = 1, VAR_PLAIN_F32 = 2, VAR_AUX = 3, VAR_STATS_BF16 = 4 };
+enum : int { VAR_FULL = 0, VAR_PLAIN_BF16 = 1, VAR_PLAIN_F32 = 2, VAR_AUX = 3, VAR_STATS_BF16 = 4, VAR_PHASE_BF16 = 5 };
 template <int VAR>
 struct GemmVariant {
   static constexpr int kMask = VAR == VAR_FULL ? (0x7fffffff & ~EPI_MASK_BITS)
                                : (VAR == VAR_PLAIN_BF16 || VAR == VAR_STATS_BF16) ? (EPI_BIAS | EPI_RELU | EPI_STATS)
                                : VAR == VAR_PLAIN_F32 ? EPI_BIAS
+                               : VAR == VAR_PHASE_BF16 ? 0
                                : (EPI_BIAS | EPI_ROW_SCALE | EPI_RESID | EPI_RESID_BF16 | EPI_MUL_DGELU | EPI_MUL_DRELU |
                                   EPI_MASK_BITS);
-  static constexpr int kOut = (VAR == VAR_PLAIN_BF16 || VAR == VAR_STATS_BF16) ? 1 : VAR == VAR_PLAIN_F32 ? 2 : 0;
+  static constexpr int kOut = (VAR == VAR_PLAIN_BF16 || VAR == VAR_STATS_BF16 || VAR == VAR_PHASE_BF16) ? 1 : VAR == VAR_PLAIN_F32 ? 2 : 0;
   static constexpr int kAux = VAR == VAR_FULL ? 0 : VAR == VAR_AUX ? 2 : 1;
   static constexpr bool kStatsWarps = VAR == VAR_STATS_BF16;
+  static constexpr bool kPhases = VAR == VAR_PHASE_BF16;
   static constexpr int kThreads = kStatsWarps ? kGemmThreads + 128 : kGemmThreads;
 };
 
@@ -117,6 +124,29 @@
   if (prev >= 0) {
     __syncwarp();
     if (lane == 0) mbar_arrive(&empty_bar[prev]);
+  }
+}
+
+template <int NCH>
+__device__ __forceinline__ void load_patch_chunks(const CUtensorMap* tm, uint64_t* bar, uint8_t* dst, const ConvGeom& g,
+                                                  int cb0, int kb) {
+  const int pix = kb * BK;
+  const int PQ = g.P * g.Q;
+  const int bn_ = pix / PQ;
+  const int rem = pix - bn_ * PQ;
+  const int pp = rem / g.Q;
+  const int bh = pp * g.stride + g.lc_h;
+  const int bw = (rem - pp * g.Q) * g.stride + g.lc_w;
+#pragma unroll
+  for (int j = 0; j < NCH; ++j) {
+    const int cb = cb0 + j;
+    const int tapj = cb / g.cchunks;
+    const int ccj = cb - tapj * g.cchunks;
+    const int rj = tapj / g.S;
+    const int sj = tapj - rj * g.S;
+    const bool valid = tapj < g.R * g.S;
+    tma_load_im2col_4d(tm, bar, dst + j * 8192, ccj * 64, bw, bh, valid ? bn_ : g.n_img, (uint16_t)(valid ? sj : 0),
+                       (uint16_t)(valid ? rj : 0));
   }
 }
 
@@ -173,9 +203,12 @@
   }
   __syncthreads();
 
-  const int num_m = (p.M + BM - 1) / BM;
+  const int phases = V::kPhases ? p.phases : 1;
+  const int tile_rows = V::kPhases ? p.tile_rows : BM;
+  const int num_m = (p.M + tile_rows - 1) / tile_rows;
   const int num_n = (p.N + BN - 1) / BN;
-  const int total = num_m * num_n * p.splits;
+  const int per_phase = num_m * num_n * p.splits;
+  const int total = per_phase * phases;
 
   if (warp == 0) {
     if (lane == 0) {
@@ -183,13 +216,15 @@
       uint32_t phase = 0;
       const int PQ = p.g.P * p.g.Q;
       for (int w = blockIdx.x; w < total; w += gridDim.x) {
-        const int n_blk = w % num_n;
-        const int t = w / num_n;
+        const int ph = V::kPhases ? w / per_phase : 0;
+        const int wp = w - ph * per_phase;
+        const int n_blk = wp % num_n;
+        const int t = wp / num_n;
         const int m_blk = t % num_m;
         const int split = t / num_m;
-        const int m0 = m_blk * BM, n0 = n_blk * BN;
+        const int m0 = m_blk * tile_rows, n0 = n_blk * BN;
         const int kb0 = split * p.kb_per_split;
-        const int kb1 = min(p.num_kb, kb0 + p.kb_per_split);
+        const int kb1 = min(phases > 1 ? p.ph_taps[ph] * p.g.cchunks : p.num_kb, kb0 + p.kb_per_split);
         int a_n = 0, a_h = 0, a_w = 0;
         if (p.a_mode == A_IM2COL) {
           a_n = m0 / PQ;
@@ -204,17 +239,32 @@
           mbar_expect_tx(bar, kABytes + kBBytes);
           uint8_t* a_dst = sA + stage * kABytes;
           uint8_t* b_dst = sB + stage * kBBytes;
-          int tap = 0, cc = kb, r = 0, s = 0;
+          int tap = 0, cc = kb, r = 0, s = 0, tapb = 0;
           if (p.a_mode == A_IM2COL) {
             tap = kb / p.g.cchunks;
             cc = kb - tap * p.g.cchunks;
-            r = tap / p.g.S;
-            s = tap - r * p.g.S;
+            if (phases > 1) {
+              const int e = p.ph_tab[ph][tap];
+              tapb = e & 0xff;
+              r = (e >> 8) & 1;
+              s = (e >> 9) & 1;
+            } else {
+              r = tap / p.g.S;
+              s = tap - r * p.g.S;
+              tapb = p.flip_taps ? (p.g.R * p.g.S - 1 - tap) : tap;
+            }
           }
           if (p.a_mode == A_K2D) {
             tma_load_2d(&tmA, bar, a_dst, kb * BK, m0);
           } else if (p.a_mode == A_IM2COL) {
             tma_load_im2col_4d(&tmA, bar, a_dst, cc * 64, a_w, a_h, a_n, (uint16_t)s, (uint16_t)r);
+          } else if constexpr (VAR == VAR_PLAIN_F32) {
+            if (p.a_mode == A_IM2COL_MN) {
+              load_patch_chunks<2>(&tmA, bar, a_dst, p.g, m0 / 64, kb);
+            } else {
+              tma_load_2d(&tmA, bar, a_dst, m0, kb * BK);
+              tma_load_2d(&tmA, bar, a_dst + 8192, m0 + 64, kb * BK);
+            }
           } else {
             tma_load_2d(&tmA, bar, a_dst, m0, kb * BK);
             tma_load_2d(&tmA, bar, a_dst + 8192, m0 + 64, kb * BK);
@@ -224,7 +274,6 @@
           } else if (p.b_mode == B_MN2D) {
             int col_base = 0, row = kb * BK;
             if (p.a_mode == A_IM2COL) {
-              const int tapb = p.flip_taps ? (p.g.R * p.g.S - 1 - tap) : tap;
               col_base = tapb * p.b_cin;
               row = cc * 64;
             }
@@ -272,7 +321,8 @@
     constexpr int NCH = BN / 32;
     const int c_begin = half ? 2 : 0;
     const int c_end = half ? NCH : 2;
-    const bool a_mn = (p.a_mode == A_MN2D), b_mn = (p.b_mode != B_K2D);
+    const bool a_mn = VAR == VAR_PLAIN_F32 ? (p.a_mode == A_MN2D || p.a_mode == A_IM2COL_MN) : (p.a_mode == A_MN2D);
+    const bool b_mn = (p.b_mode != B_K2D);
     int stage = 0;
     uint32_t phase = 0;
     const int spt = out_f32 ? (c_end - c_begin) : ((c_end - c_begin) >> 1);
@@ -286,7 +336,7 @@
         const int m_blk2 = (int)((pf_w / num_n) % num_m);
         const int col = n_blk2 * BN + (out_f32 ? (c_begin + pf_j) * 32 : ((c_begin >> 1) + pf_j) * 64);
         mbar_expect_tx(&abar[pf_b], kStoreBufBytes);
-        tma_load_3d(&tmR, &abar[pf_b], sbase + pf_b * kStoreBufBytes, col, m_blk2 * BM, 0);
+        tma_load_3d(&tmR, &abar[pf_b], sbase + pf_b * kStoreBufBytes, col, m_blk2 * tile_rows, 0);
       }
       if (++pf_j == spt) { pf_j = 0; pf_w += gridDim.x; }
       if (++pf_b == NB) pf_b = 0;
@@ -302,17 +352,19 @@
       named_bar_sync(3, kStatBarThreads);
     }
     for (int w = blockIdx.x; w < total; w += gridDim.x) {
-      const int n_blk = w % num_n;
-      const int t = w / num_n;
+      const int ph = V::kPhases ? w / per_phase : 0;
+      const int wp = w - ph * per_phase;
+      const int n_blk = wp % num_n;
+      const int t = wp / num_n;
       const int m_blk = t % num_m;
       const int split = t / num_m;
-      const int m0 = m_blk * BM, n0 = n_blk * BN;
+      const int m0 = m_blk * tile_rows, n0 = n_blk * BN;
       const long long row = m0 + row_in_tile;
       if (c_begin >= c_end) continue;
       float acc[2][32];
       {
         const int kb0 = split * p.kb_per_split;
-        const int kb1 = min(p.num_kb, kb0 + p.kb_per_split);
+        const int kb1 = min(phases > 1 ? p.ph_taps[ph] * p.g.cchunks : p.num_kb, kb0 + p.kb_per_split);
         const uint32_t b_off = half * 8192u;
         if (a_mn) gemm_mainloop<BN, 1, 1>(acc, sA, sB, full_bar, empty_bar, nstages, stage, phase, kb0, kb1, b_off, lane);
         else if (b_mn) gemm_mainloop<BN, 0, 1>(acc, sA, sB, full_bar, empty_bar, nstages, stage, phase, kb0, kb1, b_off, lane);
@@ -474,7 +526,14 @@
             named_bar_sync(bar_id, 128);
             const int scol = out_f32 ? col0 : col0 - 32;
             if (gtid == 0) {
-              if (scol < p.N) {
+              if (scol < p.N && phases > 1) {
+                const int ab = p.ph_out[ph];
+                asm volatile(
+                    "cp.async.bulk.tensor.5d.global.shared::cta.bulk_group [%0, {%2, %3, %4, %5, %6}], [%1];" ::"l"(
+                        reinterpret_cast<uint64_t>(&tmD)),
+                    "r"(smem_u32(sbuf)), "r"(scol), "r"(ab & 1), "r"(0), "r"(ab >> 1), "r"(m0 / p.g.Q)
+                    : "memory");
+              } else if (scol < p.N) {
                 asm volatile(
                     "cp.async.bulk.tensor.3d.global.shared::cta.bulk_group [%0, {%2, %3, %4}], [%1];" ::"l"(
                         reinterpret_cast<uint64_t>(&tmD)),
diff --git a/simpleaicv_pytorch_training_examples_b200/engine/convnet.py b/simpleaicv_pytorch_training_examples_b200/engine/convnet.py
--- a/simpleaicv_pytorch_training_examples_b200/engine/convnet.py
+++ b/simpleaicv_pytorch_training_examples_b200/engine/convnet.py
@@ -218,9 +218,8 @@
         w = self.conv.weight
         wbuf, wacc = sink.begin(w)
         n, P, Q, _ = dy.shape
-        h, wd = tape['in_hw']
         if self.is_stem:
-            part = ops.linear_wgrad(dy.view(-1, self.kp), tape['cols'])
+            part = ops.linear_wgrad(dy.view(-1, self.kp), tape['cols'], transposed=ops.wgrad_transposed(self.kp, self.kpad))
             ops.finish_conv_wgrad(part, wbuf, self.kpad, accumulate=wacc, order=ops.ORDER_CRS, kp=self.kp)
             sink.done(w, wbuf)
             assert not need_dx, 'the stem has no data gradient'
@@ -231,15 +230,10 @@
         sink.done(w, wbuf)
         if not need_dx:
             return None
-        if self.stride == 1:
-            return ops.conv_dgrad(dy, self.op.w, cs, add=add, mask_bits=mask_bits)
-        assert self.stride == 2
-        if self.r == 1:
+        if self.stride == 2 and self.r == 1:
             assert add is None and mask_bits is None
             return 'strided', ops.linear_dgrad(dy.view(-1, self.kp), self.op.w).view(n, P, Q, self.cp)
-        u = ops.zero_upsample2(dy, h, wd)
-        cs1 = ops.make_conv_shape(n, h, wd, self.cp, self.kp, self.r, self.s, 1, self.pad)
-        return ops.conv_dgrad(u, self.op.w, cs1, add=add, mask_bits=mask_bits)
+        return ops.conv_dgrad(dy, self.op.w, cs, add=add, mask_bits=mask_bits)
 
 
 class ResidualBlockRT:
diff --git a/simpleaicv_pytorch_training_examples_b200/ops.py b/simpleaicv_pytorch_training_examples_b200/ops.py
--- a/simpleaicv_pytorch_training_examples_b200/ops.py
+++ b/simpleaicv_pytorch_training_examples_b200/ops.py
@@ -63,13 +63,18 @@
     return _lib.load().saicv_wgrad_splits(out_rows, out_cols, reduce_len)
 
 
-def linear_wgrad(dy, x, partial=None):
+def wgrad_transposed(out_rows, out_cols):
+    return bool(_lib.load().saicv_wgrad_transposed(out_rows, out_cols))
+
+
+def linear_wgrad(dy, x, partial=None, transposed=False):
     M, N = dy.shape
     K = x.shape[1]
     splits = wgrad_splits(N, K, M)
+    a, b, rows, cols = (x, dy, K, N) if transposed else (dy, x, N, K)
     if partial is None:
-        partial = torch.empty(splits, N, K, device=dy.device, dtype=torch.float32)
-    _lib.call('saicv_linear_wgrad', _p(dy), _p(x), _p(partial), M, N, K, splits, _stream())
+        partial = torch.empty(splits, rows, cols, device=dy.device, dtype=torch.float32)
+    _lib.call('saicv_linear_wgrad', _p(a), _p(b), _p(partial), M, rows, cols, splits, _stream())
     return partial
 
 
@@ -89,7 +94,16 @@
     return out
 
 
+def phase_dgrad_ok(cs):
+    return (cs.stride == 2 and cs.r == 3 and cs.s == 3 and cs.pad == 1 and cs.h % 2 == 0 and cs.w % 2 == 0
+            and cs.w <= 256)
+
+
 def conv_dgrad(dy, w, cs, out=None, add=None, mask_bits=None):
+    if cs.stride != 1 and not (phase_dgrad_ok(cs) and add is None and mask_bits is None):
+        assert cs.stride == 2, cs.stride
+        dy = zero_upsample2(dy, cs.h, cs.w)
+        cs = make_conv_shape(cs.n, cs.h, cs.w, cs.c, cs.k, cs.r, cs.s, 1, cs.pad)
     if out is None:
         out = torch.empty(cs.n, cs.h, cs.w, cs.c, device=dy.device, dtype=torch.bfloat16)
     _lib.call('saicv_conv_dgrad', _p(dy), _p(w), _p(add), _p(mask_bits), _p(out), ctypes.byref(cs), _stream())
@@ -102,7 +116,8 @@
     ncols = cs.r * cs.s * cs.c
     splits = wgrad_splits(cs.k, ncols, cs.n * P * Q)
     if partial is None:
-        partial = torch.empty(splits, cs.k, ncols, device=dy.device, dtype=torch.float32)
+        shape = (splits, ncols, cs.k) if wgrad_transposed(cs.k, ncols) else (splits, cs.k, ncols)
+        partial = torch.empty(shape, device=dy.device, dtype=torch.float32)
     _lib.call('saicv_conv_wgrad', _p(dy), _p(x), _p(partial), ctypes.byref(cs), splits, _stream())
     return partial
 
@@ -118,8 +133,10 @@
 
 def finish_conv_wgrad(partial, grad, kpad, accumulate=False, order=ORDER_RSC, kp=0, cp=0):
     k, c, r, s = grad.shape
+    rows = kp or k
+    transposed = tuple(partial.shape[1:]) == (kpad, rows) and wgrad_transposed(rows, kpad)
     _lib.call('saicv_finish_conv_wgrad', _p(partial), _p(grad), partial.shape[0], k, c, r, s, kpad,
-              int(accumulate), order, kp, cp, _stream())
+              int(accumulate), order, kp, cp, int(transposed), _stream())
     return grad
 
 
```

Result: faster. 5733 (median of 6 runs) (+3.1%).
